# YuhuaXu/ImageMosaicing

Measured on AMD Instinct MI355X. Metric: image-pairs/sec (detect+match+H+warp), 4000x3000 UAV frames, higher is better.
Workload: dtype i16 fixed-point pyramid filtered in f32 (as the reference's OpenCV), f32 (RANSAC / warp coordinates), int8 MFMA with int32 accumulation (descriptor distances, exact), u8 (pixels); 1 GPU; C3: ONE 500-frame 4000x3000 UAV survey, pair window 2 (499 pairs), SIFT(2000,3,0.01,20) + exact BF match + 3x3 grid select + Ransac2D + MosaicImagesRefined warp; frames=500, pairs=499, frames_per_gpu=500, pairs_per_gpu=499

## Files before the change

### imagemosaicing_amd/capi.py

```python
import ctypes as C
import os
import numpy as np

_HERE = os.path.dirname(os.path.abspath(__file__))
_LIB = None

SFPOINT = np.dtype([("x", "<f4"), ("y", "<f4"), ("id", "<i4")])
KEYPOINT = np.dtype([("x", "<f4"), ("y", "<f4"), ("size", "<f4"), ("angle", "<f4"), ("response", "<f4"),
                     ("octave", "<i4"), ("class_id", "<i4")])
DMATCH = np.dtype([("queryIdx", "<i4"), ("trainIdx", "<i4"), ("imgIdx", "<i4"), ("distance", "<f4")])
MATCHPAIR = np.dtype([("ax", "<f4"), ("ay", "<f4"), ("aid", "<i4"), ("ai", "<i4"), ("af", "<i4"),
                      ("bx", "<f4"), ("by", "<f4"), ("bid", "<i4"), ("bi", "<i4"), ("bf", "<i4")])
PAIR_RESULT = np.dtype([("i", "<i4"), ("j", "<i4"), ("n_in", "<i4"), ("n_selected", "<i4"), ("ok", "<i4"),
                        ("accepted", "<i4"), ("H", "<f4", (9,)), ("_pad", "<i4"),
                        ("a", SFPOINT, (400,)), ("b", SFPOINT, (400,))])
CHIPINFO = np.dtype([("x0", "<i4"), ("y0", "<i4"), ("w", "<i4"), ("h", "<i4"), ("img", "<i4"),
                     ("sx", "<f4"), ("sy", "<f4"), ("quad", "<f4", (8,))])
IMAGE_TRANSFORM = np.dtype([("m", "<f4", (9,)), ("fixed", "<i4")])
PAIR_MOMENTS = np.dtype([("i", "<i4"), ("j", "<i4"), ("n_in", "<i4"), ("_pad", "<i4"), ("aa", "<f8", (6,)), ("ab", "<f8", (9,)), ("bb", "<f8", (6,))])
FEATURE_HEADER = np.dtype([("img_id", "<i4"), ("n_kp", "<i4"), ("w", "<i4"), ("h", "<i4")])
FEATURE_RECORD_BYTES = 319488
FEATURE_CHUNK_HEADER = np.dtype([("img_id", "<i4"), ("n_kp", "<i4"), ("w", "<i4"), ("h", "<i4"), ("chunk", "<i4"), ("n_chunks", "<i4"),
                                 ("row0", "<i4"), ("rows", "<i4")])
FEATURE_CHUNK_ROWS = 2048
assert FEATURE_CHUNK_HEADER.itemsize == 32
assert SFPOINT.itemsize == 12 and KEYPOINT.itemsize == 28 and MATCHPAIR.itemsize == 40 and PAIR_RESULT.itemsize == 9664 and PAIR_MOMENTS.itemsize == 184


class Params(C.Structure):
    _fields_ = [("nfeatures", C.c_int32), ("n_octave_layers", C.c_int32), ("contrast_threshold", C.c_float),
                ("edge_threshold", C.c_float), ("sigma", C.c_float), ("max_selected", C.c_int32),
                ("select_fraction", C.c_double), ("grid_x", C.c_int32), ("grid_y", C.c_int32), ("min_inliers", C.c_int32),
                ("ransac_dist", C.c_float), ("sample_times", C.c_int32), ("pair_window", C.c_int32), ("ratio", C.c_float)]


class ScreenParams(C.Structure):
    _fields_ = [("top_k", C.c_int32), ("partners", C.c_int32), ("min_score", C.c_int32), ("ratio_pct", C.c_int32), ("window", C.c_int32)]


class GainParams(C.Structure):
    _fields_ = [("sigma_n", C.c_float), ("sigma_g", C.c_float), ("channels", C.c_int32), ("step", C.c_int32)]


class BlockGainParams(C.Structure):
    _fields_ = [("sigma_n", C.c_float), ("sigma_g", C.c_float), ("channels", C.c_int32), ("step", C.c_int32), ("grid_x", C.c_int32),
                ("grid_y", C.c_int32), ("smooth", C.c_int32), ("reserved", C.c_int32)]


class SharpParams(C.Structure):
    _fields_ = [("prior", C.c_float), ("blur_ratio", C.c_float), ("step", C.c_int32), ("reserved", C.c_int32)]


class CoverParams(C.Structure):
    _fields_ = [("step", C.c_int32), ("min_depth", C.c_int32), ("max_loss", C.c_int64)]


class FeatherParams(C.Structure):
    _fields_ = [("ramp", C.c_int32), ("reserved", C.c_int32 * 3)]


class SeamlineParams(C.Structure):
    _fields_ = [("ramp", C.c_int32), ("reserved", C.c_int32 * 3)]


class MedianParams(C.Structure):
    _fields_ = [("ramp", C.c_int32), ("depth", C.c_int32), ("reserved", C.c_int32 * 2)]


class SeamCutParams(C.Structure):
    _fields_ = [("ramp", C.c_int32), ("level", C.c_int32), ("depth", C.c_int32), ("data_weight", C.c_int32), ("diff_weight", C.c_int32),
                ("seam_penalty", C.c_int32), ("miss_cost", C.c_int32), ("reserved", C.c_int32)]


class SeamReport(C.Structure):
    _fields_ = [("energy_before", C.c_int64), ("energy_after", C.c_int64), ("changed", C.c_int32), ("fallback", C.c_int32)]


SEAM_CELL = np.dtype([("frame", "<u2", 8), ("omega", "u1", 8), ("gray", "u1", 8)])


class Camera(C.Structure):
    _fields_ = [(n, C.c_double) for n in ("fx", "fy", "cx", "cy", "k1", "k2", "p1", "p2", "k3")]


class UndistortParams(C.Structure):
    _fields_ = [("out_fx", C.c_double), ("out_fy", C.c_double), ("out_cx", C.c_double), ("out_cy", C.c_double), ("fill", C.c_int32),
                ("reserved", C.c_int32 * 3)]


class PreviewParams(C.Structure):
    _fields_ = [("render", C.c_int32), ("ramp", C.c_int32), ("level", C.c_int32), ("nodata", C.c_int32), ("reserved", C.c_int32 * 4)]


class LocalWarpParams(C.Structure):
    _fields_ = [("grid_x", C.c_int32), ("grid_y", C.c_int32), ("min_ties", C.c_int32), ("reserved", C.c_int32), ("max_residual", C.c_double),
                ("max_shift", C.c_double), ("smooth", C.c_double), ("prior", C.c_double)]


LOCAL_WARP_REPORT = np.dtype([("n_ties", "<i8"), ("rej_den", "<i8"), ("rej_residual", "<i8"), ("rej_side", "<i8"), ("rms_before", "<f8"),
                              ("rms_after", "<f8"), ("max_shift", "<f8"), ("solved", "<i4"), ("_pad", "<i4")])
assert C.sizeof(LocalWarpParams) == 48 and LOCAL_WARP_REPORT.itemsize == 64

NODATA_NONE, NODATA_ZERO, NODATA_MAP = 0, 1, 2


GAIN_PAIR_STATS = np.dtype([("a", "<i4"), ("b", "<i4"), ("n", "<i8"), ("sum_a", "<i8", (3,)), ("sum_b", "<i8", (3,))])
assert GAIN_PAIR_STATS.itemsize == 64
BLOCK_GAIN_STATS = np.dtype([("pair", "<i4"), ("cell_a", "<i4"), ("cell_b", "<i4"), ("reserved", "<i4"), ("n", "<i8"), ("sum_a", "<i8", (3,)),
                             ("sum_b", "<i8", (3,))])
SHARP_PAIR_STATS = np.dtype([("a", "<i4"), ("b", "<i4"), ("n", "<i8"), ("e_a", "<i8"), ("e_b", "<i8"), ("s_a", "<i8"), ("s_b", "<i8")])
SHARP_FRAME_STATS = np.dtype([("n", "<i8"), ("e", "<i8"), ("s", "<i8")])
SHARP_KEPT, SHARP_DROPPED, SHARP_CUT_VERTEX, SHARP_NO_PAIR = 0, 1, 2, 3
assert SHARP_PAIR_STATS.itemsize == 48 and SHARP_FRAME_STATS.itemsize == 24 and C.sizeof(SharpParams) == 16
COVER_FRAME_STATS = np.dtype([("at_depth", "<i8", (8,))])
COVER_BINS = 9
COVER_NOT_CANDIDATE, COVER_DROPPED, COVER_KEPT_COVERAGE, COVER_CUT_VERTEX, COVER_NOT_EXAMINED = 0, 1, 2, 3, 4
COVER_STATS_FN = C.CFUNCTYPE(C.c_int, C.c_void_p, C.c_void_p, C.c_void_p)
assert COVER_FRAME_STATS.itemsize == 64 and C.sizeof(CoverParams) == 16
PAIR_NORMAL_BLOCK = np.dtype([("i", "<i4"), ("j", "<i4"), ("n_in", "<i4"), ("_pad", "<i4"), ("cost", "<f8"), ("g", "<f8", (16,)), ("N", "<f8", (136,))])


class ProjectiveParams(C.Structure):
    _fields_ = [("max_iters", C.c_int32), ("reserved", C.c_int32), ("prior", C.c_double), ("lambda0", C.c_double), ("lambda_up", C.c_double),
                ("lambda_down", C.c_double), ("min_rel_decrease", C.c_double)]


class ProjectiveReport(C.Structure):
    _fields_ = [("trials", C.c_int32), ("accepted", C.c_int32), ("n_free", C.c_int32), ("n_pairs_used", C.c_int32), ("n_points", C.c_int64),
                ("cost0", C.c_double), ("cost_data", C.c_double), ("cost_prior", C.c_double), ("lambda_", C.c_double)]

    def as_dict(self):
        return {n.rstrip("_"): getattr(self, n) for n, _ in self._fields_}


PAIR_CALIB_BLOCK = np.dtype([("i", "<i4"), ("j", "<i4"), ("n_in", "<i4"), ("n_bad", "<i4"), ("cost", "<f8"), ("g", "<f8", (13,)), ("N", "<f8", (91,))])
CALIB_K1, CALIB_K2, CALIB_P1, CALIB_P2, CALIB_K3 = 1, 2, 4, 8, 16


class CalibParams(C.Structure):
    _fields_ = [("max_iters", C.c_int32), ("mask", C.c_int32), ("min_ties", C.c_int32), ("reserved", C.c_int32), ("lambda0", C.c_double),
                ("lambda_up", C.c_double), ("lambda_down", C.c_double), ("min_rel_decrease", C.c_double)]


class CalibReport(C.Structure):
    _fields_ = [("trials", C.c_int32), ("accepted", C.c_int32), ("n_pairs_used", C.c_int32), ("n_unused_records", C.c_int32), ("n_points", C.c_int64),
                ("cost0", C.c_double), ("cost", C.c_double), ("lambda_", C.c_double)]

    def as_dict(self):
        return {n.rstrip("_"): getattr(self, n) for n, _ in self._fields_}


assert PAIR_CALIB_BLOCK.itemsize == 856 and C.sizeof(CalibParams) == 48 and C.sizeof(CalibReport) == 48


class TieParams(C.Structure):
    _fields_ = [("radius", C.c_int32), ("search", C.c_int32), ("drop_mask", C.c_int32), ("reserved", C.c_int32), ("min_ncc", C.c_float)]


TIE_REPORT = np.dtype([("i", "<i4"), ("j", "<i4"), ("n_in", "<i4"), ("n_out", "<i4"), ("flags", "<i4"), ("count", "<i4", (8,)), ("_pad", "<i4"),
                       ("ncc_q_sum", "<i8")])
TIE_NONE, TIE_REFINED, TIE_EDGE, TIE_FLAT, TIE_LOW, TIE_BORDER = 0, 1, 2, 3, 4, 5
TIE_FLAG_NOT_ACCEPTED, TIE_FLAG_NO_FRAME, TIE_FLAG_BAD_RECORD, TIE_FLAG_DEMOTED = 1, 2, 4, 8
assert TIE_REPORT.itemsize == 64 and C.sizeof(TieParams) == 20
assert PAIR_NORMAL_BLOCK.itemsize == 1240 and C.sizeof(ProjectiveParams) == 48 and C.sizeof(ProjectiveReport) == 56
assert BLOCK_GAIN_STATS.itemsize == 72 and C.sizeof(BlockGainParams) == 32
assert C.sizeof(Camera) == 72 and C.sizeof(UndistortParams) == 48


class VerifyParams(C.Structure):
    _fields_ = [("cycle_tol", C.c_double), ("gate_abs", C.c_double), ("gate_k", C.c_double), ("max_rounds", C.c_int32), ("bridges", C.c_int32)]


PAIR_EDGE = np.dtype([("i", "<i4"), ("j", "<i4"), ("n_in", "<i4"), ("flags", "<i4"), ("box", "<f4", (4,)), ("F", "<f8", (9,)), ("B", "<f8", (9,))])
PAIR_CYCLE = np.dtype([("n_ok", "<i4"), ("n_bad", "<i4"), ("min_e2", "<f8")])
PAIR_RESIDUAL = np.dtype([("i", "<i4"), ("j", "<i4"), ("n_used", "<i4"), ("n_den", "<i4"), ("sum_r2", "<f8"), ("max_r2", "<f8")])
VERIFY_REPORT = np.dtype([("i", "<i4"), ("j", "<i4"), ("n_in", "<i4"), ("verdict", "<i4"), ("n_ok", "<i4"), ("n_bad", "<i4"), ("round", "<i4"),
                          ("flags", "<i4"), ("min_e2", "<f8"), ("rms", "<f8"), ("max_r2", "<f8"), ("reserved", "<f8")])
VERIFY_SUMMARY = np.dtype([("count", "<i4", (8,)), ("rounds", "<i4"), ("n_labelled", "<i4"), ("reserved", "<i4", (2,)), ("s", "<f8"), ("gate", "<f8")])
EDGE_USABLE, EDGE_TESTABLE = 1, 2
VERDICT_NOT_USED, VERDICT_VERIFIED, VERDICT_ADMITTED, VERDICT_BRIDGE, VERDICT_REJECTED, VERDICT_UNDECIDED = 0, 1, 2, 3, 4, 5
VERIFY_SUSPECT = 1
assert PAIR_EDGE.itemsize == 176 and PAIR_CYCLE.itemsize == 16 and PAIR_RESIDUAL.itemsize == 32
assert C.sizeof(VerifyParams) == 32 and VERIFY_REPORT.itemsize == 64 and VERIFY_SUMMARY.itemsize == 64


class GuidedParams(C.Structure):
    _fields_ = [("radius", C.c_float), ("max_dist2", C.c_int32), ("ratio", C.c_float), ("reserved", C.c_int32)]


assert C.sizeof(GuidedParams) == 16


class Mi355Error(RuntimeError):
    def __init__(self, code, msg):
        super().__init__("mi355 error %d: %s" % (code, msg))
        self.code = code


def lib_path():
    return os.environ.get("MI355_LIB") or os.path.join(_HERE, "libmi355mosaic.so")


def load_library():
    global _LIB
    if _LIB is None:
        p = lib_path()
        if not os.path.exists(p):
            raise ImportError("libmi355mosaic.so is not built: run `python -m imagemosaicing_amd.build` "
                              "(there is no CPU fallback for the HIP path)")
        try:
            import torch
        except ImportError:
            pass
        L = C.CDLL(p)
        L.mi355_last_error.restype = C.c_char_p
        L.mi355_last_error.argtypes = [C.c_void_p]
        L.mi355_create.argtypes = [C.POINTER(C.c_void_p), C.c_void_p, C.c_int]
        L.mi355_destroy.argtypes = [C.c_void_p]
        L.mi355_free.argtypes = [C.c_void_p]
        _LIB = L
    return _LIB


def default_params():
    p = Params()
    load_library().mi355_default_params(C.byref(p))
    return p


def _p(a):
    return a.ctypes.data_as(C.c_void_p) if a is not None else None


def _img_geom(img):
    img = np.ascontiguousarray(img, np.uint8)
    h, w = img.shape[:2]
    ch = img.shape[2] if img.ndim == 3 else 1
    return img, w, h, img.strides[0], ch


def _copy_out(ptr, nbytes, dtype):
    if nbytes == 0:
        return np.zeros(0, dtype)
    raw = np.ctypeslib.as_array(C.cast(ptr, C.POINTER(C.c_uint8)), shape=(nbytes,)).copy()
    return raw.view(dtype)


def _view_out(ptr, nbytes, dtype, copy):
    raw = np.ctypeslib.as_array(C.cast(ptr, C.POINTER(C.c_uint8)), shape=(nbytes,))
    return (raw.copy() if copy else raw).view(dtype)


class Context:

    def __init__(self, device=0, params=None):
        self.L = load_library()
        self._h = C.c_void_p()
        rc = self.L.mi355_create(C.byref(self._h), C.byref(params) if params is not None else None, int(device))
        if rc != 0:
            raise Mi355Error(rc, (self.L.mi355_last_error(None) or b"").decode())
        self.params = params if params is not None else default_params()
        self.device = int(device)

    def close(self):
        if self._h:
            self.L.mi355_destroy(self._h)
            self._h = C.c_void_p()

    def __del__(self):
        try:
            self.close()
        except Exception:
            pass

    def _chk(self, rc):
        if rc < 0:
            raise Mi355Error(rc, (self.L.mi355_last_error(self._h) or b"").decode())
        return rc

    def set_stream(self, hip_stream):
        self._chk(self.L.mi355_set_stream(self._h, C.c_void_p(hip_stream or 0)))

    def synchronize(self):
        self._chk(self.L.mi355_synchronize(self._h))

    def set_option(self, name, value):
        self._chk(self.L.mi355_set_option(self._h, name.encode(), int(value)))

    def profile_enable(self, on=True):
        self._chk(self.L.mi355_profile_enable(self._h, int(bool(on))))

    def profile_only(self, cls=None):
        self._chk(self.L.mi355_profile_only(self._h, (cls or "").encode()))

    def profile_reset(self):
        self._chk(self.L.mi355_profile_reset(self._h))

    def profile_get(self, cls):
        ms, n, b = C.c_double(), C.c_int64(), C.c_double()
        self._chk(self.L.mi355_profile_get(self._h, cls.encode(), C.byref(ms), C.byref(n), C.byref(b)))
        return ms.value, n.value, b.value

    def SiftExtract(self, img_id, bgr, max_kp=None):
        img, w, h, ws, ch = _img_geom(bgr)
        assert ch == 3
        max_kp = max_kp or max(int(self.params.nfeatures), 2048)
        kp = np.zeros(max_kp, KEYPOINT)
        desc = np.zeros((max_kp, 128), np.float32)
        n = C.c_int(0)
        self._chk(self.L.mi355_sift_extract(self._h, int(img_id), _p(img), w, h, ws, _p(kp), _p(desc), max_kp, C.byref(n)))
        k = min(n.value, max_kp)
        return kp[:k].copy(), desc[:k].copy()

    def SiftExtractHost(self, img_id, bgr):
        img, w, h, ws, ch = _img_geom(bgr)
        assert ch == 3
        self._chk(self.L.mi355_sift_extract(self._h, int(img_id), _p(img), w, h, ws, None, None, 0, None))

    def SiftExtractDev(self, img_id, d_bgr, w, h, ws, want_count=False):
        if not want_count:
            self._chk(self.L.mi355_sift_extract_dev(self._h, int(img_id), C.c_void_p(int(d_bgr)), int(w), int(h), int(ws), None))
            return None
        n = C.c_int(0)
        self._chk(self.L.mi355_sift_extract_dev(self._h, int(img_id), C.c_void_p(int(d_bgr)), int(w), int(h), int(ws), C.byref(n)))
        return n.value

    def GetFeatures(self, img_id, max_kp=4096):
        kp = np.zeros(max_kp, KEYPOINT)
        desc = np.zeros((max_kp, 128), np.float32)
        n = C.c_int(0)
        self._chk(self.L.mi355_get_features(self._h, int(img_id), _p(kp), _p(desc), max_kp, C.byref(n)))
        return kp[:n.value].copy(), desc[:n.value].copy()

    def SetFeatures(self, img_id, kp, desc, w, h):
        kp = np.ascontiguousarray(kp, KEYPOINT)
        desc = np.ascontiguousarray(desc, np.float32)
        self._chk(self.L.mi355_set_features(self._h, int(img_id), _p(kp), _p(desc), len(kp), int(w), int(h)))

    def DropFeatures(self, img_id=-1):
        self._chk(self.L.mi355_drop_features(self._h, int(img_id)))

    def MatchPairs(self, pairs, ransac_dist=2.5, seed=1):
        pairs = np.ascontiguousarray(pairs, np.int32).reshape(-1, 2)
        out = np.zeros(len(pairs), PAIR_RESULT)
        self._chk(self.L.mi355_match_pairs(self._h, _p(pairs), len(pairs), C.c_float(ransac_dist), C.c_uint32(seed), _p(out)))
        return out

    def MatchPairsDev(self, pairs, d_out, ransac_dist=2.5, seed=1):
        pairs = np.ascontiguousarray(pairs, np.int32).reshape(-1, 2)
        self._chk(self.L.mi355_match_pairs_dev(self._h, _p(pairs), len(pairs), C.c_float(ransac_dist), C.c_uint32(seed), C.c_void_p(int(d_out))))

    def ScreenPairs(self, img_ids, window=0, top_k=256, partners=None, min_score=None, ratio_pct=80, rank=0, world=1, return_scores=False):
        ids = np.ascontiguousarray(img_ids, np.int32).reshape(-1)
        p = screen_params(window=window, top_k=top_k, partners=partners, min_score=min_score, ratio_pct=ratio_pct)
        cap = len(ids) * p.partners if p.partners > 0 else 0
        n = C.c_int(0)
        while True:
            out = np.zeros((max(cap, 1), 2), np.int32)
            sc = np.zeros(max(cap, 1), np.int32)
            rc = self.L.mi355_screen_pairs(self._h, _p(ids), len(ids), C.byref(p), int(rank), int(world), _p(out), _p(sc), cap, C.byref(n))
            if rc == -1 and n.value > cap:
                cap = n.value
                continue
            self._chk(rc)
            break
        pairs = out[:n.value].copy()
        return (pairs, sc[:n.value].copy()) if return_scores else pairs

    def ScreenScoresDev(self, img_ids, d_scores, **params):
        ids = np.ascontiguousarray(img_ids, np.int32).reshape(-1)
        p = screen_params(**params)
        self._chk(self.L.mi355_screen_scores_dev(self._h, _p(ids), len(ids), C.byref(p), C.c_void_p(int(d_scores))))

    def BFMatch(self, img_i, img_j, sorted_=True, max_matches=2048):
        m = np.zeros(max_matches, DMATCH)
        d2 = np.zeros(max_matches, np.int32)
        s2 = np.zeros(max_matches, np.int32)
        n = C.c_int(0)
        self._chk(self.L.mi355_bf_match(self._h, int(img_i), int(img_j), int(bool(sorted_)), _p(m), _p(d2), _p(s2), max_matches, C.byref(n)))
        k = min(n.value, max_matches)
        return m[:k].copy(), d2[:k].copy(), s2[:k].copy()

    def SelectMatchPairs(self, matches, kp1_xy, kp2_xy, nMatch, width, height, gridX=3, gridY=3):
        matches = np.asarray(matches)
        if matches.dtype != DMATCH:
            mm = np.zeros(len(matches), DMATCH)
            mm["queryIdx"] = matches[:, 0]
            mm["trainIdx"] = matches[:, 1]
            matches = mm
        matches = np.ascontiguousarray(matches)
        kp1 = np.ascontiguousarray(kp1_xy, np.float32)
        kp2 = np.ascontiguousarray(kp2_xy, np.float32)
        v1 = np.zeros(400, SFPOINT)
        v2 = np.zeros(400, SFPOINT)
        n = C.c_int(0)
        self._chk(self.L.mi355_select_grid(self._h, _p(matches), len(matches), _p(kp1), len(kp1), _p(kp2), len(kp2), int(nMatch),
                                           int(width), int(height), int(gridX), int(gridY), _p(v1), _p(v2), C.byref(n)))
        return v1[:n.value].copy(), v2[:n.value].copy()

    def Ransac2D(self, p1, p2, fRansacDist=1.0, sampleTimes=1000, seed=1):
        p1 = np.ascontiguousarray(p1, SFPOINT)
        p2 = np.ascontiguousarray(p2, SFPOINT)
        n = len(p1)
        i1 = np.zeros(max(400, n), SFPOINT)
        i2 = np.zeros(max(400, n), SFPOINT)
        nin = C.c_int(0)
        H = np.zeros(9, np.float32)
        ok = self._chk(self.L.mi355_ransac2d(self._h, _p(p1), _p(p2), n, C.c_float(fRansacDist), int(sampleTimes), C.c_uint32(seed),
                                             _p(i1), _p(i2), C.byref(nin), _p(H)))
        return ok, i1[:nin.value].copy(), i2[:nin.value].copy(), H

    def ImageProjectionTransform(self, img, h9):
        img, w, h, ws, ch = _img_geom(img)
        h9 = np.ascontiguousarray(h9, np.float32)
        dst = C.c_void_p()
        dw, dh, dws = C.c_int(), C.c_int(), C.c_int()
        self._chk(self.L.mi355_warp_image(self._h, _p(img), w, h, ws, ch, _p(h9), C.byref(dst), C.byref(dw), C.byref(dh), C.byref(dws)))
        buf = _copy_out(dst, dh.value * dws.value, np.uint8).reshape(dh.value, dws.value)
        self.L.mi355_free(dst)
        return buf, dw.value, dh.value, dws.value

    def MosaicImagesRefined(self, imgs, h9s, want_pixels=True):
        n, imgs, ptrs, w, h, ws = self._host_args(imgs)
        h9s = np.ascontiguousarray(h9s, np.float32)
        canvas = C.c_void_p()
        cw, ch, cws = C.c_int(), C.c_int(), C.c_int()
        self._chk(self.L.mi355_mosaic_refined(self._h, ptrs, _p(w), _p(h), _p(ws), n, _p(h9s), C.byref(canvas), C.byref(cw), C.byref(ch), C.byref(cws)))
        buf = _copy_out(canvas, ch.value * cws.value, np.uint8).reshape(ch.value, cws.value) if want_pixels else None
        self.L.mi355_free(canvas)
        return buf, cw.value, ch.value, cws.value

    def MosaicImagesRefinedDev(self, d_imgs, w, h, ws, h9s, d_canvas, cw, ch, cws, row0=0, rows=-1):
        n = len(d_imgs)
        ptrs = (C.c_void_p * n)(*[int(p) for p in d_imgs])
        w = np.ascontiguousarray(w, np.int32)
        h = np.ascontiguousarray(h, np.int32)
        ws = np.ascontiguousarray(ws, np.int32)
        h9s = np.ascontiguousarray(h9s, np.float32)
        self._chk(self.L.mi355_mosaic_refined_dev(self._h, ptrs, _p(w), _p(h), _p(ws), n, _p(h9s), C.c_void_p(int(d_canvas)),
                                                  int(cw), int(ch), int(cws), int(row0), int(rows if rows >= 0 else ch)))

    def SurfExtract(self, img_id, bgr, hessian=50.0, max_kp=4096):
        img, w, h, ws, ch = _img_geom(bgr)
        assert ch == 3
        kp = np.zeros(max_kp, KEYPOINT)
        desc = np.zeros((max_kp, 128), np.float32)
        n = C.c_int(0)
        self._chk(self.L.mi355_surf_extract(self._h, int(img_id), _p(img), w, h, ws, C.c_float(hessian), int(max_kp), _p(kp), _p(desc), C.byref(n)))
        return kp[:n.value].copy(), desc[:n.value].copy()

    def SurfMatchPairs(self, pairs, ransac_dist=2.5, seed=1, match_dist=0.5, max_features=200, min_inliers=18):
        pairs = np.ascontiguousarray(pairs, np.int32).reshape(-1, 2)
        out = np.zeros(len(pairs), PAIR_RESULT)
        self._chk(self.L.mi355_surf_match_pairs(self._h, _p(pairs), len(pairs), C.c_float(ransac_dist), C.c_uint32(seed), C.c_float(match_dist),
                                                int(max_features), int(min_inliers), _p(out)))
        return out

    def PackFeaturesDev(self, img_ids, d_payload):
        ids = np.ascontiguousarray(img_ids, np.int32)
        hdr = np.zeros(len(ids), FEATURE_HEADER)
        self._chk(self.L.mi355_pack_features_dev(self._h, _p(ids), len(ids), _p(hdr), C.c_void_p(int(d_payload))))
        return hdr

    def InstallFeaturesDev(self, hdr, d_payload):
        hdr = np.ascontiguousarray(hdr, FEATURE_HEADER)
        self._chk(self.L.mi355_install_features_dev(self._h, _p(hdr), C.c_void_p(int(d_payload)), len(hdr)))

    def FeatureChunkCount(self, img_ids):
        ids = np.ascontiguousarray(img_ids, np.int32)
        n = C.c_int(0)
        self._chk(self.L.mi355_feature_chunk_count(self._h, _p(ids), len(ids), C.byref(n)))
        return n.value

    def PackFeatureChunksDev(self, img_ids, d_payload, max_records):
        ids = np.ascontiguousarray(img_ids, np.int32)
        hdr = np.zeros(max(int(max_records), 1), FEATURE_CHUNK_HEADER)
        n = C.c_int(0)
        self._chk(self.L.mi355_pack_feature_chunks_dev(self._h, _p(ids), len(ids), _p(hdr), C.c_void_p(int(d_payload) or None), int(max_records), C.byref(n)))
        return hdr[:n.value].copy()

    def InstallFeatureChunksDev(self, hdr, d_payload):
        hdr = np.ascontiguousarray(hdr, FEATURE_CHUNK_HEADER)
        self._chk(self.L.mi355_install_feature_chunks_dev(self._h, _p(hdr), C.c_void_p(int(d_payload) or None), len(hdr)))

    def CompactAcceptedDev(self, d_in, n, d_out):
        k = C.c_int(0)
        self._chk(self.L.mi355_compact_accepted_dev(self._h, C.c_void_p(int(d_in)), int(n), C.c_void_p(int(d_out)), C.byref(k)))
        return k.value

    def last_sift_counters(self):
        out = (C.c_int32 * 8)()
        self._chk(self.L.mi355_last_sift_counters(self._h, out))
        return list(out)

    def CommInit(self, id128, rank, world):
        buf = (C.c_uint8 * 128).from_buffer_copy(bytes(id128))
        self._chk(self.L.mi355_comm_init(self._h, buf, int(rank), int(world)))

    def CommDestroy(self):
        self._chk(self.L.mi355_comm_destroy(self._h))

    def CommInfo(self):
        r, n = C.c_int(0), C.c_int(0)
        self._chk(self.L.mi355_comm_info(self._h, C.byref(r), C.byref(n)))
        return r.value, n.value

    def AllGatherFeatures(self, img_ids, n_max_per_rank):
        ids = np.ascontiguousarray(img_ids, np.int32)
        self._chk(self.L.mi355_allgather_features(self._h, _p(ids), len(ids), int(n_max_per_rank)))

    def AllGatherFeatureChunks(self, img_ids, install_own=False):
        ids = np.ascontiguousarray(img_ids, np.int32)
        self._chk(self.L.mi355_allgather_feature_chunks(self._h, _p(ids), len(ids), 1 if install_own else 0))

    def AllGatherResults(self, d_local, n_local, accepted_only=True, root=-1, copy=True, wait=True):
        assert wait or (root >= 0 and not copy)
        ptr, n = C.c_void_p(), C.c_int(0)
        flags = (1 if accepted_only else 0) | (0 if wait else 2)
        self._chk(self.L.mi355_allgather_results(self._h, C.c_void_p(int(d_local)), int(n_local), flags, int(root), C.byref(ptr), C.byref(n)))
        if not ptr.value or n.value == 0:
            return np.zeros(0, PAIR_RESULT)
        return _view_out(ptr, n.value * PAIR_RESULT.itemsize, PAIR_RESULT, copy)

    def PairMomentsDev(self, d_results, n, d_out):
        self._chk(self.L.mi355_pair_moments_dev(self._h, C.c_void_p(int(d_results)), int(n), C.c_void_p(int(d_out))))

    def PairNormalBlocksDev(self, d_results, n, h8, part, d_out):
        h8 = np.ascontiguousarray(h8, np.float64).reshape(-1, 8)
        part = np.ascontiguousarray(part, np.uint8)
        assert len(h8) == len(part)
        self._chk(self.L.mi355_pair_normal_blocks_dev(self._h, C.c_void_p(int(d_results)), int(n), _p(h8), _p(part), len(part), C.c_void_p(int(d_out))))

    def GlobalProjectiveRefineDev(self, d_results, n_pairs, w, h, start, fixed=None, label=None, params=None):
        a = _projective_args(w, h, start, fixed, label)
        out, rep = np.zeros(len(a[2]), IMAGE_TRANSFORM), ProjectiveReport()
        self._chk(self.L.mi355_global_projective_refine_dev(self._h, C.c_void_p(int(d_results) or None), int(n_pairs), len(a[2]), _p(a[0]), _p(a[1]), _p(a[3]), _p(a[4]), _p(a[2]),
                                                            C.byref(params) if params is not None else None, _p(out), C.byref(rep)))
        return out, rep.as_dict()

    def PairCalibBlocksDev(self, d_results, n, h8, cam, d_out, min_ties=16):
        h8 = None if h8 is None else np.ascontiguousarray(h8, np.float64).reshape(-1, 8)
        assert h8 is None or len(h8) >= int(n)
        self._chk(self.L.mi355_pair_calib_blocks_dev(self._h, C.c_void_p(int(d_results or 0) or None), int(n), _p(h8), C.byref(cam) if cam is not None else None,
                                                     int(min_ties), C.c_void_p(int(d_out or 0) or None)))

    def CalibrateLensDev(self, d_results, n_pairs, start, params=None, **kw):
        p = params if params is not None else calib_params(**kw)
        out, rep = Camera(), CalibReport()
        self._chk(self.L.mi355_calibrate_lens_dev(self._h, C.c_void_p(int(d_results or 0) or None), int(n_pairs), C.byref(start) if start is not None else None, C.byref(p),
                                                  C.byref(out), C.byref(rep)))
        return out, rep.as_dict()

    def RefineTiesDev(self, d_in, n, d_imgs, w, h, ws, d_out, d_status=0, d_ncc2=0, d_report=0, params=None, **kw):
        n_img, ptrs, w, h, ws = self._frame_args(d_imgs, w, h, ws)
        p = params if params is not None else tie_params(**kw)
        self._chk(self.L.mi355_refine_ties_dev(self._h, C.c_void_p(int(d_in or 0) or None), int(n), ptrs, _p(w), _p(h), _p(ws), n_img, C.byref(p),
                                               C.c_void_p(int(d_out or 0) or None), C.c_void_p(int(d_status or 0) or None),
                                               C.c_void_p(int(d_ncc2 or 0) or None), C.c_void_p(int(d_report or 0) or None)))

    def RefineTies(self, results, imgs, img_ids=None, geom=None, params=None, **kw):
        res = np.ascontiguousarray(results, PAIR_RESULT)
        n = len(res)
        ptrs, ids, w, h, ws, _keep = self._into_args(imgs, img_ids, geom)
        p = params if params is not None else tie_params(**kw)
        out = np.zeros(n, PAIR_RESULT)
        status, ncc2, report = np.zeros((n, 400), np.uint8), np.zeros((n, 400), np.float32), np.zeros(n, TIE_REPORT)
        self._chk(self.L.mi355_refine_ties(self._h, _p(res), n, ptrs, _p(ids), _p(w), _p(h), _p(ws), len(ids), C.byref(p), _p(out), _p(status), _p(ncc2),
                                           _p(report)))
        return out, status, ncc2, report

    def AllGatherMoments(self, d_local, n_local, copy=True):
        ptr, n = C.c_void_p(), C.c_int(0)
        self._chk(self.L.mi355_allgather_moments(self._h, C.c_void_p(int(d_local)), int(n_local), C.byref(ptr), C.byref(n)))
        if not ptr.value or n.value == 0:
            return np.zeros(0, PAIR_MOMENTS)
        return _view_out(ptr, n.value * PAIR_MOMENTS.itemsize, PAIR_MOMENTS, copy)

    def StripeCover(self, w, h, h9s, row0, rows, blended=False, keep=None, band=5, exact=False):
        n = len(w)
        w = np.ascontiguousarray(w, np.int32); h = np.ascontiguousarray(h, np.int32)
        h9s = np.ascontiguousarray(h9s, np.float32)
        keep_a = None if keep is None else np.ascontiguousarray(keep, np.uint8)
        need = np.zeros(n, np.uint8)
        mode = 1 if blended else (2 if exact else 0)
        self._chk(self.L.mi355_mosaic_stripe_cover(self._h, mode, _p(w), _p(h), n, _p(h9s), _p(keep_a), int(band), int(row0), int(rows), _p(need)))
        return need

    def ExchangeFrames(self, d_frames, h, ws, need, owner=None, own_through_rccl=False):
        n = len(d_frames)
        ptrs = (C.c_void_p * max(n, 1))(*[int(p) if p else None for p in d_frames])
# ... 1470 lines not shown
```

### imagemosaicing_amd/csrc/api.hip

```cpp
#include "common.h"
#include "mosaic_frame.h"
#include <memory>
#include <new>

static thread_local std::string g_create_error;

void mi_set_host_error(const std::string& s) { g_create_error = s; }

extern "C" void mi355_default_params(mi355_params* p) {
    if (!p) return;
    p->nfeatures = 2000; p->n_octave_layers = 3; p->contrast_threshold = 0.01f; p->edge_threshold = 20.0f; p->sigma = 1.6f;
    p->max_selected = 400; p->select_fraction = 0.3; p->grid_x = 3; p->grid_y = 3; p->min_inliers = 30;
    p->ransac_dist = 2.5f; p->sample_times = 1000; p->pair_window = 182; p->ratio = 0.0f;
}

void mi355_ctx::prof_begin(const char* cls, double alg_bytes, hipStream_t st) {
    ProfClass& pc = prof[cls];
    if (pc.used == pc.ev.size()) {
        hipEvent_t a, b;
        if (hipEventCreate(&a) != hipSuccess || hipEventCreate(&b) != hipSuccess) return;
        pc.ev.emplace_back(a, b);
    }
    pc.bytes += alg_bytes;
    (void)hipEventRecord(pc.ev[pc.used].first, st);
// ... 67 lines not shown
    if (ctx->heavy_ev) (void)hipEventDestroy(ctx->heavy_ev);
    for (hipEvent_t e : ctx->batch_events) if (e) (void)hipEventDestroy(e);
    if (ctx->own_stream) (void)hipStreamDestroy(ctx->own_stream);
    delete ctx;
}

extern "C" const char* mi355_last_error(mi355_ctx* ctx) { return ctx ? ctx->err.c_str() : g_create_error.c_str(); }

extern "C" int mi355_set_stream(mi355_ctx* ctx, void* hip_stream) {
    LOCKED_PROLOGUE
    { int rc = mi_resolve_features(ctx); if (rc != MI355_OK) return rc; }
    (void)hipStreamSynchronize(ctx->stream);
    if (hip_stream) {
        if (ctx->own_stream) { (void)hipStreamDestroy(ctx->own_stream); ctx->own_stream = nullptr; }
        ctx->stream = (hipStream_t)hip_stream;
    } else {
        if (!ctx->own_stream) MI_HIP(hipStreamCreateWithFlags(&ctx->own_stream, hipStreamNonBlocking));
        ctx->stream = ctx->own_stream;
    }
    return MI355_OK;
}

extern "C" int mi355_synchronize(mi355_ctx* ctx) {
    LOCKED_PROLOGUE
    int rc = mi_resolve_features(ctx);
    if (rc != MI355_OK) return rc;
    MI_HIP(hipStreamSynchronize(ctx->stream));
    return MI355_OK;
}

extern "C" void mi355_free(void* p) { free(p); }

extern "C" int mi355_sift_extract_dev(mi355_ctx* ctx, int img_id, const uint8_t* d_bgr, int w, int h, int width_step, int* n_kp) {
    LOCKED_PROLOGUE
    if (!d_bgr || w < 16 || h < 16 || width_step < 3 * w) { ctx->set_error("sift_extract: bad image geometry"); return MI355_ERR_ARG; }
    return mi_sift_extract_dev(ctx, img_id, d_bgr, w, h, width_step, n_kp);
}

extern "C" int mi355_sift_extract(mi355_ctx* ctx, int img_id, const uint8_t* bgr, int w, int h, int width_step,
                                  mi355_keypoint* kp, float* desc128, int max_kp, int* n_kp) {
    int n = 0;
    const bool deferred = !kp && !desc128 && !n_kp;
    {
        LOCKED_PROLOGUE
        if (!bgr || w < 16 || h < 16 || width_step < 3 * w) { ctx->set_error("sift_extract: bad image geometry"); return MI355_ERR_ARG; }
        const size_t bytes = (size_t)width_step * h;
        if (ctx->keep_frames) {
            uint8_t* dkeep = nullptr;
            int rc = mi_kept_frame_slot(ctx, img_id, w, h, width_step, "sift_extract", &dkeep);
            if (rc != MI355_OK) return rc;
            MI_HIP(hipMemcpyAsync(dkeep, bgr, bytes, hipMemcpyHostToDevice, ctx->stream));
            ctx->pend_event = ctx->kept_frames[img_id].ev;
            rc = mi_sift_extract_dev(ctx, img_id, dkeep, w, h, width_step, deferred ? nullptr : &n);
            ctx->pend_event = nullptr;
            if (rc != MI355_OK || deferred) return rc;
        } else if (deferred) {
            const size_t ring = (size_t)(ctx->sift_nslots + 1) * (size_t)(ctx->sift_batch < 1 ? 1 : ctx->sift_batch);
            if (ctx->host_frames.size() != ring) {
                int rc = mi_resolve_features(ctx);
                if (rc != MI355_OK) return rc;
                for (auto& b : ctx->host_frames) b.release();
                for (hipEvent_t e : ctx->host_frame_ev) if (e) (void)hipEventDestroy(e);
                ctx->host_frames.assign(ring, DevBuf());
                ctx->host_frame_ev.assign(ring, nullptr);
                ctx->host_frame_used.assign(ring, 0);
                ctx->host_frame_next = 0;
            }
            const size_t slot = ctx->host_frame_next;
            ctx->host_frame_next = (ctx->host_frame_next + 1) % ring;
            DevBuf& dimg = ctx->host_frames[slot];
            if (!ctx->host_frame_ev[slot]) MI_HIP(hipEventCreateWithFlags(&ctx->host_frame_ev[slot], hipEventDisableTiming));
            if (ctx->host_frame_used[slot]) {
                int rc = mi_sift_flush_if_parked(ctx, ctx->host_frame_ev[slot]);
                if (rc != MI355_OK) return rc;
                MI_HIP(hipStreamWaitEvent(ctx->stream, ctx->host_frame_ev[slot], 0));
            }
            ctx->host_frame_used[slot] = 1;
            MI_HIP(dimg.reserve(bytes + 16));
            MI_HIP(hipMemcpyAsync(dimg.p, bgr, bytes, hipMemcpyHostToDevice, ctx->stream));
            ctx->pend_event = ctx->host_frame_ev[slot];
            const int rc = mi_sift_extract_dev(ctx, img_id, dimg.as<uint8_t>(), w, h, width_step, nullptr);
            ctx->pend_event = nullptr;
            return rc;
        } else {
            DevBuf& dimg = ctx->buf("sift_host_img");
            MI_HIP(dimg.reserve(bytes + 16));
            MI_HIP(hipMemcpyAsync(dimg.p, bgr, bytes, hipMemcpyHostToDevice, ctx->stream));
            int rc = mi_sift_extract_dev(ctx, img_id, dimg.as<uint8_t>(), w, h, width_step, &n);
            if (rc != MI355_OK) return rc;
        }
    }
    if (n_kp) *n_kp = n;
    if (kp || desc128) return mi355_get_features(ctx, img_id, kp, desc128, max_kp, nullptr);
    return MI355_OK;
}

extern "C" int mi355_set_features(mi355_ctx* ctx, int img_id, const mi355_keypoint* kp, const float* desc128, int n_kp, int w, int h) {
    LOCKED_PROLOGUE
    return mi_set_features(ctx, img_id, kp, desc128, n_kp, w, h);
}

extern "C" int mi355_drop_features(mi355_ctx* ctx, int img_id) {
    LOCKED_PROLOGUE
    (void)mi_resolve_features(ctx);
    MI_HIP(hipStreamSynchronize(ctx->stream));
    if (img_id < 0) { for (auto& kv : ctx->feats) kv.second.release(); ctx->feats.clear(); }
    else { auto it = ctx->feats.find(img_id); if (it != ctx->feats.end()) { it->second.release(); ctx->feats.erase(it); } }
    return MI355_OK;
}

extern "C" int mi355_match_pairs_dev(mi355_ctx* ctx, const int32_t* pairs_ij, int n_pairs, float ransac_dist, uint32_t seed, mi355_pair_result* d_out) {
    LOCKED_PROLOGUE
    if (n_pairs < 0 || (n_pairs > 0 && (!pairs_ij || !d_out))) return MI355_ERR_ARG;
    return mi_match_pairs_dev(ctx, pairs_ij, n_pairs, ransac_dist, seed, d_out);
}

extern "C" int mi355_match_pairs(mi355_ctx* ctx, const int32_t* pairs_ij, int n_pairs, float ransac_dist, uint32_t seed, mi355_pair_result* out) {
    LOCKED_PROLOGUE
    if (n_pairs < 0 || (n_pairs > 0 && (!pairs_ij || !out))) return MI355_ERR_ARG;
    if (n_pairs == 0) return MI355_OK;
    DevBuf& dres = ctx->buf("pair_results");
    MI_HIP(dres.reserve(sizeof(mi355_pair_result) * (size_t)n_pairs));
    int rc = mi_match_pairs_dev(ctx, pairs_ij, n_pairs, ransac_dist, seed, dres.as<mi355_pair_result>());
    if (rc != MI355_OK) return rc;
    MI_HIP(hipMemcpyAsync(out, dres.p, sizeof(mi355_pair_result) * (size_t)n_pairs, hipMemcpyDeviceToHost, ctx->stream));
    MI_HIP(hipStreamSynchronize(ctx->stream));
    return MI355_OK;
}

extern "C" int mi355_bf_match(mi355_ctx* ctx, int img_i, int img_j, int sorted, mi355_dmatch* matches, int32_t* d2, int32_t* second_d2,
                              int max_matches, int* n_matches) {
    LOCKED_PROLOGUE
    return mi_bf_match(ctx, img_i, img_j, sorted, matches, d2, second_d2, max_matches, n_matches);
}

extern "C" int mi355_select_grid(mi355_ctx* ctx, const mi355_dmatch* sorted, int n, const float* kp1_xy, int n_kp1,
                                 const float* kp2_xy, int n_kp2, int nMatch, int width, int height, int gridX, int gridY,
                                 mi355_sfpoint* v1, mi355_sfpoint* v2, int* n_out) {
    LOCKED_PROLOGUE
    if (nMatch < 0 || nMatch > MI355_MAX_SELECTED) { ctx->set_error("select_grid: nMatch must be in [0,400]"); return MI355_ERR_ARG; }
    return mi_select_grid(ctx, sorted, n, kp1_xy, n_kp1, kp2_xy, n_kp2, nMatch, width, height, gridX, gridY, v1, v2, n_out);
}

extern "C" int mi355_ransac2d(mi355_ctx* ctx, const mi355_sfpoint* p1, const mi355_sfpoint* p2, int n, float dist, int sample_times,
                              uint32_t seed, mi355_sfpoint* in1, mi355_sfpoint* in2, int* n_in, float H[9]) {
    LOCKED_PROLOGUE
    if (!n_in || !H) return MI355_ERR_ARG;
    *n_in = 0;
    for (int i = 0; i < 9; i++) H[i] = 0.0f;
    if (n <= 0 || !p1 || !p2) return 0;
    if (n > MI355_RANSAC_BIG_MAX) { ctx->set_error("ransac2d: at most 65535 correspondences"); return MI355_ERR_ARG; }
    if (n > MI355_MAX_SELECTED) {
        int ok = 0;
        const int rc = mi_ransac_big(ctx, p1, p2, n, dist, sample_times, seed, in1, in2, n_in, H, &ok);
        return rc != MI355_OK ? rc : ok;
    }
    DevBuf& d1 = ctx->buf("r1_p1"); DevBuf& d2 = ctx->buf("r1_p2"); DevBuf& dn = ctx->buf("r1_n"); DevBuf& dres = ctx->buf("pair_results");
    MI_HIP(d1.reserve(sizeof(mi355_sfpoint) * MI355_MAX_SELECTED)); MI_HIP(d2.reserve(sizeof(mi355_sfpoint) * MI355_MAX_SELECTED));
    MI_HIP(dn.reserve(sizeof(int))); MI_HIP(dres.reserve(sizeof(mi355_pair_result)));
    MI_HIP(hipMemcpyAsync(d1.p, p1, sizeof(mi355_sfpoint) * n, hipMemcpyHostToDevice, ctx->stream));
    MI_HIP(hipMemcpyAsync(d2.p, p2, sizeof(mi355_sfpoint) * n, hipMemcpyHostToDevice, ctx->stream));
    MI_HIP(hipMemcpyAsync(dn.p, &n, sizeof(int), hipMemcpyHostToDevice, ctx->stream));
    int rc = mi_ransac_batch(ctx, d1.as<mi355_sfpoint>(), d2.as<mi355_sfpoint>(), dn.as<int>(), &n, 1, MI355_MAX_SELECTED, dist, sample_times, seed,
                             dres.as<mi355_pair_result>());
    if (rc != MI355_OK) return rc;
    const std::unique_ptr<mi355_pair_result> r(new (std::nothrow) mi355_pair_result);
    if (!r) return MI355_ERR_NOMEM;
    hipError_t e = hipMemcpyAsync(r.get(), dres.p, sizeof(mi355_pair_result), hipMemcpyDeviceToHost, ctx->stream);
    if (e == hipSuccess) e = hipStreamSynchronize(ctx->stream);
    if (e != hipSuccess) { ctx->set_error(hipGetErrorString(e)); return MI355_ERR_DEVICE; }
    *n_in = r->n_in;
    if (in1) memcpy(in1, r->a, sizeof(mi355_sfpoint) * r->n_in);
    if (in2) memcpy(in2, r->b, sizeof(mi355_sfpoint) * r->n_in);
    memcpy(H, r->H, sizeof(float) * 9);
    return r->ok;
}

extern "C" int mi355_warp_image(mi355_ctx* ctx, const uint8_t* src, int w, int h, int ws, int ch, const float h9[9],
                                uint8_t** dst, int* dw, int* dh, int* dws) {
    LOCKED_PROLOGUE
    if (!dst || !dw || !dh || !dws) return MI355_ERR_ARG;
    return mi_warp_image(ctx, src, w, h, ws, ch, h9, dst, dw, dh, dws);
}

extern "C" int mi355_mosaic_refined_dev(mi355_ctx* ctx, const uint8_t* const* d_imgs, const int* w, const int* h, const int* ws, int n,
                                        const float* h9s, uint8_t* d_canvas, int cw, int ch, int cws, int row0, int rows) {
    LOCKED_PROLOGUE
    if (!d_imgs || !w || !h || !ws || !h9s || !d_canvas || n <= 0) return MI355_ERR_ARG;
    return mi_mosaic_refined_dev(ctx, d_imgs, w, h, ws, n, h9s, d_canvas, cw, ch, cws, row0, rows);
}

extern "C" int mi355_mosaic_refined(mi355_ctx* ctx, const uint8_t* const* imgs, const int* w, const int* h, const int* ws, int n,
                                    const float* h9s, uint8_t** canvas, int* cw, int* ch, int* cws) {
    LOCKED_PROLOGUE
    if (!imgs || !w || !h || !ws || !h9s || !canvas || !cw || !ch || !cws) return MI355_ERR_ARG;
    int lw, lh, lws;
    std::vector<const uint8_t*> d_imgs;
    uint8_t* d_canvas;
    int rc = mi_render_host_begin(ctx, "mosaic_refined", imgs, w, h, ws, n, h9s, &lw, &lh, &lws, d_imgs, &d_canvas);
    if (rc == MI355_OK) rc = mi_mosaic_refined_dev(ctx, d_imgs.data(), w, h, ws, n, h9s, d_canvas, lw, lh, lws, 0, lh);
    if (rc != MI355_OK) return rc;
    return mi_render_host_end(ctx, lw, lh, lws, canvas, cw, ch, cws);
}

extern "C" int mi355_chips_and_masks(mi355_ctx* ctx, const uint8_t* const* imgs, const int* w, const int* h, const int* ws, int n,
                                     const float* h9s, const uint8_t* keep, int find_masks,
                                     int* n_chips, mi355_chip_info** chips, uint8_t*** chip_imgs, uint8_t*** masks, int* canvas_w, int* canvas_h) {
    LOCKED_PROLOGUE
    return mi_chips_and_masks(ctx, imgs, w, h, ws, n, h9s, keep, find_masks, n_chips, chips, chip_imgs, masks, canvas_w, canvas_h);
}

extern "C" int mi355_multiband_blend(mi355_ctx* ctx, const uint8_t* const* chips, const uint8_t* const* masks, const mi355_chip_info* info, int n,
                                     int canvas_w, int canvas_h, int band, uint8_t** out, int* out_w, int* out_h, int* out_ws) {
    LOCKED_PROLOGUE
    return mi_multiband_blend(ctx, chips, masks, info, n, canvas_w, canvas_h, band, out, out_w, out_h, out_ws);
}

extern "C" int mi355_mosaic_blended(mi355_ctx* ctx, const uint8_t* const* imgs, const int* w, const int* h, const int* ws, int n, const float* h9s,
                                    const uint8_t* keep, int band, uint8_t** out, int* out_w, int* out_h, int* out_ws) {
    LOCKED_PROLOGUE
    return mi_mosaic_blended(ctx, imgs, w, h, ws, n, h9s, keep, band, out, out_w, out_h, out_ws);
}

extern "C" int mi355_mosaic_blended_dev(mi355_ctx* ctx, const uint8_t* const* d_imgs, const int* w, const int* h, const int* ws, int n, const float* h9s,
                                        const uint8_t* keep, int band, uint8_t* d_canvas, int cw, int ch, int cws) {
    LOCKED_PROLOGUE
    return mi_mosaic_blended_dev(ctx, d_imgs, w, h, ws, n, h9s, keep, band, d_canvas, cw, ch, cws);
}

extern "C" int mi355_mosaic_blended_rows_dev(mi355_ctx* ctx, const uint8_t* const* d_imgs, const int* w, const int* h, const int* ws, int n, const float* h9s,
                                             const uint8_t* keep, int band, uint8_t* d_rows, int cw, int ch, int cws, int row0, int rows) {
    LOCKED_PROLOGUE
    if (rows < 1) { ctx->set_error("mosaic_blended_rows_dev: bad stripe"); return MI355_ERR_ARG; }
    return mi_mosaic_blended_dev(ctx, d_imgs, w, h, ws, n, h9s, keep, band, d_rows, cw, ch, cws, row0, rows);
}

extern "C" int mi355_mosaic_stripe_cover(mi355_ctx* ctx, int mode, const int* w, const int* h, int n, const float* h9s, const uint8_t* keep, int band,
                                         int row0, int rows, uint8_t* need) {
    LOCKED_PROLOGUE
    if (!w || !h || !h9s || !need || n <= 0 || mode < 0 || mode > 2) { ctx->set_error("mosaic_stripe_cover: bad arguments"); return MI355_ERR_ARG; }
    memset(need, 0, (size_t)n);
    std::vector<const uint8_t*> none((size_t)n, nullptr);
    std::vector<int> ws((size_t)n);
    for (int k = 0; k < n; k++) ws[k] = (3 * w[k] + 3) & ~3;
    if (mode != MI355_COVER_BLENDED) {
        int cw = 0, ch = 0, cws = 0;
        const int rc = mi355_mosaic_layout(w, h, n, h9s, &cw, &ch, &cws, nullptr);
        if (rc != MI355_OK) { ctx->set_error("mosaic_stripe_cover: no image with h[8] != 0 / empty canvas"); return rc; }
        return mi_mosaic_refined_dev(ctx, none.data(), w, h, ws.data(), n, h9s, nullptr, cw, ch, cws, row0, rows, need, mode == MI355_COVER_REFINED_EXACT ? 1 : 0);
    }
    int cw = 0, ch = 0;
    { const int rc = mi_blend_layout(w, h, n, h9s, keep, &cw, &ch); if (rc != MI355_OK) return rc; }
    return mi_mosaic_blended_dev(ctx, none.data(), w, h, ws.data(), n, h9s, keep, band, nullptr, cw, ch, (cw * 3 + 3) & ~3, row0, rows, need);
}

extern "C" int mi355_blend_layout(const int* w, const int* h, int n, const float* h9s, const uint8_t* keep, int* cw, int* ch, int* cws) {
    if (!cw || !ch) return MI355_ERR_ARG;
    const int rc = mi_blend_layout(w, h, n, h9s, keep, cw, ch);
    if (rc == MI355_OK && cws) *cws = (*cw * 3 + 3) & ~3;
    return rc;
}

extern "C" int mi355_profile_enable(mi355_ctx* ctx, int on) {
    LOCKED_PROLOGUE
    ctx->profiling = on != 0;
    return MI355_OK;
}
extern "C" int mi355_last_sift_counters(mi355_ctx* ctx, int32_t out8[8]) {
    LOCKED_PROLOGUE
    if (!out8) return MI355_ERR_ARG;
    for (int i = 0; i < 8; i++) out8[i] = ctx->last_counts[i];
    return MI355_OK;
}
extern "C" int mi355_set_option(mi355_ctx* ctx, const char* name, int value) {
    LOCKED_PROLOGUE
    if (!name) return MI355_ERR_ARG;
    if (std::string(name) == "sift_slots") {
        int rc = mi_resolve_features(ctx);
        if (rc != MI355_OK) return rc;
        ctx->sift_nslots = value < 1 ? 1 : (value > 4 ? 4 : value);
        return MI355_OK;
    }
    if (std::string(name) == "sift_batch") {
        int rc = mi_resolve_features(ctx);
        if (rc != MI355_OK) return rc;
        ctx->sift_batch = value < 1 ? 1 : (value > 32 ? 32 : value);
        return MI355_OK;
    }
    if (std::string(name) == "keepall_max") {
        if (value < MI355_SIFT_KEEPALL_MAX || value > MI355_SIFT_KEEPALL_LIMIT || value % 2048 != 0) {
            ctx->set_error("set_option: keepall_max must be a multiple of 2048 in [" + std::to_string(MI355_SIFT_KEEPALL_MAX) + ", " + std::to_string(MI355_SIFT_KEEPALL_LIMIT) + "]");
            return MI355_ERR_ARG;
        }
        int rc = mi_resolve_features(ctx);
        if (rc != MI355_OK) return rc;
        for (const auto& kv : ctx->feats)
            if (kv.second.n > value) {
                ctx->set_error("set_option: keepall_max=" + std::to_string(value) + " is below the " + std::to_string(kv.second.n) + " keypoints of image " + std::to_string(kv.first));
                return MI355_ERR_ARG;
            }
        ctx->keepall_max = value;
        return MI355_OK;
    }
    if (std::string(name) == "big_subpairs_max") { ctx->big_sub_max = value < 1 ? 1 : value; return MI355_OK; }
    {
        struct { const char* n; int* p; } knobs[] = {{"ransac_split", &ctx->ransac_split}, {"strict_frames", &ctx->strict_frames}};
        for (auto& k : knobs) if (std::string(name) == k.n) { *k.p = value; return MI355_OK; }
    }
    if (std::string(name) == "keep_frames") { ctx->keep_frames = value ? 1 : 0; return MI355_OK; }
    if (std::string(name) == "download_chunk_mb") {
        if (value < 1) { ctx->set_error("set_option: download_chunk_mb must be >= 1"); return MI355_ERR_ARG; }
        ctx->download_chunk = (size_t)value << 20;
        return MI355_OK;
    }
    if (std::string(name) == "download_threads") { ctx->download_threads = value < 1 ? 1 : (value > 16 ? 16 : value); return MI355_OK; }
    if (std::string(name) == "preview_stripe_rows") {
        if (value < 0) { ctx->set_error("set_option: preview_stripe_rows must be >= 0"); return MI355_ERR_ARG; }
        ctx->preview_stripe_rows = value;
        return MI355_OK;
    }
    if (std::string(name) == "download_mode") { ctx->download_mode = value < 0 || value > 2 ? 0 : value; return MI355_OK; }
    if (std::string(name) == "sift_flush") return mi_sift_flush(ctx);
    if (std::string(name) == "blur_stream") { ctx->blur_stream = value ? 1 : 0; return MI355_OK; }
    if (std::string(name) == "sift_cascade" || std::string(name) == "keepall_order") return MI355_OK;
    if (std::string(name) == "serial_heavy") {
        int rc = mi_resolve_features(ctx);
        if (rc != MI355_OK) return rc;
        ctx->serial_heavy = value ? 1 : 0; ctx->heavy_ev_valid = false;
        return MI355_OK;
    }
    if (std::string(name).rfind("profile_every:", 0) == 0) { ctx->prof[std::string(name).substr(14)].every = value < 1 ? 1 : value; return MI355_OK; }
    if (std::string(name) == "xstream_min_w") { ctx->xstream_min_w = value < 256 ? 256 : value; return MI355_OK; }
    if (std::string(name) == "xstream_min_frames") { ctx->xstream_min_frames = value < 1 ? 1 : value; return MI355_OK; }
    ctx->set_error(std::string("set_option: unknown option ") + name);
    return MI355_ERR_ARG;
}
extern "C" int mi355_profile_only(mi355_ctx* ctx, const char* kernel_class) {
    LOCKED_PROLOGUE
    ctx->prof_only = kernel_class ? kernel_class : "";
    return MI355_OK;
}
extern "C" int mi355_profile_reset(mi355_ctx* ctx) {
    LOCKED_PROLOGUE
    (void)mi_resolve_features(ctx);
    MI_HIP(hipStreamSynchronize(ctx->stream));
    for (auto& kv : ctx->prof) { kv.second.used = 0; kv.second.bytes = 0.0; kv.second.seen = 0; }
    return MI355_OK;
}
extern "C" int mi355_profile_get(mi355_ctx* ctx, const char* kernel_class, double* total_ms, int64_t* launches, double* alg_bytes) {
    LOCKED_PROLOGUE
    if (!kernel_class) return MI355_ERR_ARG;
    (void)mi_resolve_features(ctx);
    MI_HIP(hipStreamSynchronize(ctx->stream));
    double ms = 0.0; int64_t cnt = 0; double bytes = 0.0;
    auto it = ctx->prof.find(kernel_class);
    if (it != ctx->prof.end()) {
        for (size_t i = 0; i < it->second.used; i++) {
            float t = 0.0f;
            if (hipEventElapsedTime(&t, it->second.ev[i].first, it->second.ev[i].second) == hipSuccess) ms += t;
        }
        cnt = (int64_t)it->second.used; bytes = it->second.bytes;
    }
    if (total_ms) *total_ms = ms;
    if (launches) *launches = cnt;
    if (alg_bytes) *alg_bytes = bytes;
    return MI355_OK;
}

extern "C" int mi355_pair_schedule(int n_images, int window, int rank, int world, int32_t* pairs_ij, int max_pairs, int* n_pairs) {
    if (n_images < 0 || window < 2 || world < 1 || rank < 0 || rank >= world || !n_pairs) return MI355_ERR_ARG;
    int cnt = 0;
    for (int i = rank; i < n_images; i += world) {
        const int jEnd = n_images < i + window ? n_images : i + window;
        for (int j = i + 1; j < jEnd; j++) {
            if (pairs_ij && cnt < max_pairs) { pairs_ij[2 * cnt] = i; pairs_ij[2 * cnt + 1] = j; }
            cnt++;
        }
    }
    *n_pairs = cnt;
    return (pairs_ij && cnt > max_pairs) ? MI355_ERR_ARG : MI355_OK;
}
```

### imagemosaicing_amd/csrc/common.h

```cpp
#pragma once
#include <hip/hip_runtime.h>
#include <cstdint>
#include <cstdio>
#include <cstring>
#include <cstdlib>
#include <map>
#include <mutex>
#include <string>
#include <unordered_map>
#include <vector>
#include "../../include/mi355_mosaic.h"

#define MI_HIP(call)                                                                       \
    do {                                                                                   \
        hipError_t e_ = (call);                                                            \
        if (e_ != hipSuccess) {                                                            \
            ctx->set_error(std::string(#call) + ": " + hipGetErrorString(e_));             \
            return MI355_ERR_DEVICE;                                                       \
        }                                                                                  \
    } while (0)

#define LOCKED_PROLOGUE                                  \
    if (!ctx) return MI355_ERR_ARG;                      \
    std::lock_guard<std::mutex> lk(ctx->mu);             \
    if (hipSetDevice(ctx->device) != hipSuccess) { ctx->set_error("hipSetDevice failed"); return MI355_ERR_DEVICE; }

constexpr int MI355_SIFT_BATCH_MAX = 32;
constexpr int MI355_SIFT_KEEPALL_MAX = 32768;

constexpr int MI355_SIFT_KEEPALL_LIMIT = 262144;

struct DevBuf {
    void*  p = nullptr;
    size_t cap = 0;
    hipError_t reserve(size_t bytes) {
        if (bytes <= cap) return hipSuccess;
        if (p) { hipError_t e = hipFree(p); if (e != hipSuccess) return e; p = nullptr; cap = 0; }
        size_t slack = bytes / 4;
        if (slack > ((size_t)256 << 20)) slack = (size_t)256 << 20;
        size_t want = bytes + slack + 256;
        hipError_t e = hipMalloc(&p, want);
        if (e == hipSuccess) cap = want;
        return e;
    }
    void release() { if (p) (void)hipFree(p); p = nullptr; cap = 0; }
    template <class T> T* as() const { return reinterpret_cast<T*>(p); }
};

struct HostBuf {
    void*  p = nullptr;
    size_t cap = 0;
    hipError_t reserve(size_t bytes) {
        if (bytes <= cap) return hipSuccess;
        if (p) { hipError_t e = hipHostFree(p); if (e != hipSuccess) return e; p = nullptr; cap = 0; }
        const size_t want = bytes + bytes / 8 + 4096;
        hipError_t e = hipHostMalloc(&p, want, hipHostMallocDefault);
        if (e == hipSuccess) cap = want;
        return e;
    }
    void release() { if (p) (void)hipHostFree(p); p = nullptr; cap = 0; }
    template <class T> T* as() const { return reinterpret_cast<T*>(p); }
};

struct Features {
    int n = 0;
    int npad = 0;
    int w = 0, h = 0;
    DevBuf kp;
    DevBuf xy;
    DevBuf d8;
    DevBuf s8;
    DevBuf n8;
    bool pending = false;
    volatile int* h_cnt = nullptr;
    hipEvent_t ready = nullptr;
    unsigned caps[3] = {0, 0, 0};
    int kp_limit = 0;
    void release() { kp.release(); xy.release(); d8.release(); s8.release(); n8.release(); }
};

struct KeptFrame {
    void*  p = nullptr;
    size_t cap = 0;
    int w = 0, h = 0, ws = 0;
    hipEvent_t ev = nullptr;
};

struct ProfClass {
    std::vector<std::pair<hipEvent_t, hipEvent_t>> ev;
    size_t used = 0;
    double bytes = 0.0;
    size_t seen = 0;
    int every = 1;
};

struct SiftWork;
struct mi355_comm;
struct SurfState;

struct mi355_ctx {
    int device = 0;
    hipStream_t stream = nullptr;
    hipStream_t own_stream = nullptr;
    std::mutex mu;
    mi355_params p;
    std::string err;
    std::unordered_map<int, Features> feats;
    std::map<std::string, DevBuf> ws;
    std::map<std::string, HostBuf> hws;
    struct DrawTables { uint32_t seed = 0; bool valid = false; DevBuf buf, raw; hipEvent_t ready = nullptr; unsigned long long used = 0; };
    DrawTables draw_tables[4];
    unsigned long long draw_clock = 0;
    hipStream_t aux_stream = nullptr;
    hipEvent_t aux_ev = nullptr;
    int* draw_flags = nullptr;
    bool profiling = false;
    std::string prof_only;
    std::map<std::string, ProfClass> prof;
    std::vector<SiftWork*> sift_slots;
    int sift_next = 0;
    std::vector<hipEvent_t> batch_events; size_t batch_events_used = 0;
    hipEvent_t heavy_ev = nullptr; bool heavy_ev_valid = false;
    int serial_heavy = 0;
    std::vector<DevBuf> host_frames;
    std::vector<hipEvent_t> host_frame_ev;
    std::vector<char> host_frame_used;
    size_t host_frame_next = 0;
    hipEvent_t pend_event = nullptr;
    int keep_frames = 0;
    std::unordered_map<int, KeptFrame> kept_frames;
    size_t download_chunk = (size_t)64 << 20;
    int download_threads = 4;
    int preview_stripe_rows = 1024;
    int download_mode = 0;
    hipStream_t dl_stream = nullptr;
    hipEvent_t dl_ev[3] = {nullptr, nullptr, nullptr};
    int blur_stream = 1;
    int sift_nslots = 3;
    int xstream_min_w = 1500, xstream_min_frames = 4;
    int sift_batch = 16;
    int strict_frames = 0;
    int ransac_split = -1;
    hipEvent_t sift_in_ev = nullptr;
    std::vector<int*> pinned_chunks;
    size_t pinned_used = 0;
    int num_cu = 256;
    mi355_comm* comm = nullptr;
    SurfState* surf = nullptr;
    int keepall_max = MI355_SIFT_KEEPALL_MAX;
    int big_sub_max = 65536;
    int last_counts[8] = {0};

    void set_error(const std::string& s) { err = s; }
    DevBuf& buf(const std::string& name) { return ws[name]; }
    HostBuf& hbuf(const std::string& name) { return hws[name]; }
    void prof_begin(const char* cls, double alg_bytes, hipStream_t st);
    void prof_end(const char* cls, hipStream_t st);
};

struct ProfScope {
    mi355_ctx* c; const char* cls; hipStream_t st;
    bool on;
    ProfScope(mi355_ctx* c_, const char* cls_, double bytes, hipStream_t st_ = nullptr) : c(c_), cls(cls_), st(st_ ? st_ : c_->stream) {
        on = c->profiling && (c->prof_only.empty() || ("," + c->prof_only + ",").find(std::string(",") + cls + ",") != std::string::npos);
        if (on) { ProfClass& pc = c->prof[cls]; if (pc.every > 1) on = (pc.seen++ % (size_t)pc.every) == 0; }
        if (on) c->prof_begin(cls, bytes, st);
    }
    ~ProfScope() { if (on) c->prof_end(cls, st); }
};

int mi_warp_image(mi355_ctx*, const uint8_t* src, int w, int h, int ws, int ch, const float* h9,
                  uint8_t** dst, int* dw, int* dh, int* dws);
int mi_mosaic_refined_dev(mi355_ctx*, const uint8_t* const* d_imgs, const int* w, const int* h, const int* ws, int n,
                          const float* h9s, uint8_t* d_canvas, int cw, int ch, int cws, int row0, int rows, uint8_t* cover_only = nullptr, int cover_exact = 0);
int mi_mosaic_feathered_dev(mi355_ctx*, const uint8_t* const* d_imgs, const int* w, const int* h, const int* ws, int n, const float* h9s,
                            const mi355_feather_params* params, uint8_t* d_canvas, int cw, int ch, int cws, int row0, int rows);
int mi_mosaic_seamline_dev(mi355_ctx*, const uint8_t* const* d_imgs, const int* w, const int* h, const int* ws, int n, const float* h9s,
                           const mi355_seamline_params* params, uint8_t* d_canvas, int cw, int ch, int cws, uint16_t* d_owner, uint16_t* d_count,
                           int row0, int rows, uint8_t* cover_only);
int mi_mosaic_median_dev(mi355_ctx*, const uint8_t* const* d_imgs, const int* w, const int* h, const int* ws, int n, const float* h9s,
                         const mi355_median_params* params, uint8_t* d_canvas, int cw, int ch, int cws, uint8_t* d_spread, uint16_t* d_count,
                         int row0, int rows, uint8_t* cover_only);
int mi_mosaic_seamcut_dev(mi355_ctx*, const uint8_t* const* d_imgs, const int* w, const int* h, const int* ws, int n, const float* h9s,
                          const mi355_seamcut_params* params, const uint16_t* d_cells, uint8_t* d_canvas, int cw, int ch, int cws, uint16_t* d_owner,
                          uint16_t* d_count, int row0, int rows, uint8_t* cover_only);
int mi_seam_labels_dev(mi355_ctx*, const mi355_seam_cell* d_cand, int gw, int gh, const mi355_seamcut_params* params, uint16_t* d_cells,
                       mi355_seam_report* report);
int mi_seamcut_params_check(mi355_ctx*, const char* who, const mi355_seamcut_params* params);
int mi_mosaic_blended_seam_dev(mi355_ctx*, const uint8_t* const* d_imgs, const int* w, const int* h, const int* ws, int n, const float* h9s,
                               const uint8_t* keep, int band, const mi355_seamcut_params* params, const uint16_t* d_cells, int gw, int gh,
                               uint8_t* d_canvas, int cw, int ch, int cws);
int mi_mosaic_overview_dev(mi355_ctx*, const uint8_t* d_rows, int cw, int ch, int cws, const uint16_t* d_valid_rows, int nodata, int levels,
                           uint8_t* const* d_levels, uint16_t* const* d_covers, int row0, int rows, int only_level = 0);
int mi_sift_flush(mi355_ctx*);
int mi_sift_flush_if_parked(mi355_ctx*, hipEvent_t ev);
int mi_mosaic_blended(mi355_ctx*, const uint8_t* const* imgs, const int* w, const int* h, const int* ws, int n, const float* h9s,
                      const uint8_t* keep, int band, uint8_t** out, int* ow, int* oh, int* ows);
int mi_mosaic_blended_dev(mi355_ctx*, const uint8_t* const* d_imgs, const int* w, const int* h, const int* ws, int n, const float* h9s,
                          const uint8_t* keep, int band, uint8_t* d_canvas, int cw, int ch, int cws, int row0 = 0, int rows = -1, uint8_t* cover_only = nullptr);
int mi_blend_layout(const int* w, const int* h, int n, const float* h9s, const uint8_t* keep, int* cw, int* ch);
int mi_multiband_blend(mi355_ctx*, const uint8_t* const* chips, const uint8_t* const* masks, const mi355_chip_info* info, int n,
                       int W, int H, int band, uint8_t** out, int* ow, int* oh, int* ows);
int mi_chips_and_masks(mi355_ctx*, const uint8_t* const* imgs, const int* w, const int* h, const int* ws, int n,
                       const float* h9s, const uint8_t* keep, int find_masks, int* n_chips, mi355_chip_info** chips,
                       uint8_t*** chip_imgs, uint8_t*** masks, int* cw, int* ch);
int mi_ransac_tables(mi355_ctx*, uint32_t seed, const uint16_t** d_tables);
int mi_ransac_batch(mi355_ctx*, const mi355_sfpoint* d_p1, const mi355_sfpoint* d_p2, const int* d_n, const int* h_n,
                    int n_pairs, int stride, float dist, int sample_times, uint32_t seed, mi355_pair_result* d_out, int min_keep = -1);
int mi_ransac_big(mi355_ctx*, const mi355_sfpoint* p1, const mi355_sfpoint* p2, int n, float dist, int sample_times, uint32_t seed,
                  mi355_sfpoint* in1, mi355_sfpoint* in2, int* n_in, float* H, int* ok);
int mi_match_pairs_dev(mi355_ctx*, const int32_t* pairs, int n_pairs, float dist, uint32_t seed, mi355_pair_result* d_out);
int mi_finalize_pairs(mi355_ctx*, const int32_t* pairs_ij , int n_pairs, const int* d_nsel, mi355_pair_result* d_out);
int mi_bf_match(mi355_ctx*, int img_i, int img_j, int sorted, mi355_dmatch* matches, int32_t* d2, int32_t* second, int maxm, int* nm);
int mi_select_grid(mi355_ctx*, const mi355_dmatch* sorted, int n, const float* kp1, int nk1, const float* kp2, int nk2,
                   int nMatch, int width, int height, int gx, int gy, mi355_sfpoint* v1, mi355_sfpoint* v2, int* n_out);
int mi_set_features(mi355_ctx*, int img_id, const mi355_keypoint* kp, const float* desc, int n, int w, int h);
int mi_finish_features(mi355_ctx*, Features& f);
int mi_finish_features_batch(mi355_ctx*, Features* const* fs, int nf, const int* d_n, int n_stride, hipStream_t st, int max_rows = 2048);
int mi_resolve_features(mi355_ctx*);
int mi_resolve_features_of(mi355_ctx*, const int* ids, int n);
int mi_sift_extract_dev(mi355_ctx*, int img_id, const uint8_t* d_bgr, int w, int h, int ws, int* n_kp);
void mi_sift_release(mi355_ctx*);
void mi_comm_release(mi355_ctx*);
void mi_surf_release(mi355_ctx*);
int  mi_kept_frame_slot(mi355_ctx*, int img_id, int w, int h, int ws, const char* who, uint8_t** d_frame);
void mi_frames_release(mi355_ctx*);
int mi_compact_accepted(mi355_ctx* ctx, const mi355_pair_result* d_in, int n, mi355_pair_result* d_out, int* d_n_out);
int mi_pair_moments(mi355_ctx* ctx, const mi355_pair_result* d_results, int n, mi355_pair_moments* d_out);

#include "host_error.h"
int  mi_inverse_matrix_host(const float* src, int order, float* dst, float eps);
void mi_glibc_draw_table(uint32_t seed, int n, int max_draws, uint16_t* out4);
```

### imagemosaicing_amd/csrc/sift.hip

```cpp
#include "common.h"
#include "sift_plan.h"
#include <memory>
#include "detmath.h"
#include <cmath>
#include <type_traits>

namespace {

using namespace sift_plan;
constexpr int MAX_INTERP = 5, ORI_BINS = 36;
constexpr int FIXPT_SCALE = 48;
constexpr float DOG_THRESHOLD_P1 = 21.0f;
constexpr float HIST_Q = 1024.0f;
constexpr int SIFT_BATCH_MAX = MI355_SIFT_BATCH_MAX;
static_assert(SIFT_BATCH_MAX == BATCH_MAX, "sift_plan.h: BATCH_MAX");
typedef int16_t lvl_t;

__host__ __device__ __forceinline__ int reflect101(int p, int n) {
    if (n == 1) return 0;
    while (p < 0 || p >= n) { if (p < 0) p = -p; else p = 2 * n - 2 - p; }
    return p;
}

typedef float v2f __attribute__((ext_vector_type(2)));
struct __attribute__((aligned(4))) uint2_a4 { unsigned x, y; };
typedef float v4f __attribute__((ext_vector_type(4)));

__device__ __forceinline__ v4f ld4(const lvl_t* p) {
    const uint2 q = *reinterpret_cast<const uint2*>(p);
    v4f o;
    o.x = (float)(int)(short)(q.x & 0xffffu); o.y = (float)((int)q.x >> 16);
    o.z = (float)(int)(short)(q.y & 0xffffu); o.w = (float)((int)q.y >> 16);
    return o;
}
__device__ __forceinline__ float ld1(const lvl_t* p) { return (float)(int)*p; }
__device__ __forceinline__ int sat16(float v) {
    int q = (int)rintf(v);
    q = q < -32768 ? -32768 : (q > 32767 ? 32767 : q);
    return q;
}
__device__ __forceinline__ float gray48(const uint8_t* p) {
    return (float)(((1868 * (int)p[0] + 9617 * (int)p[1] + 4899 * (int)p[2] + 8192) >> 14) * FIXPT_SCALE);
}

__device__ __forceinline__ int xcd_remap(int bid, int nb) {
    const int q = nb >> 3, r = nb & 7, xcd = bid & 7, local = bid >> 3;
    const int base = xcd < r ? xcd * (q + 1) : r * (q + 1) + (xcd - r) * q;
    return base + local;
}

template <int J, int NPP, class F> __device__ __forceinline__ bool static_rows(F& f) {
    if constexpr (J < NPP) { if (!f(std::integral_constant<int, J>{})) return false; return static_rows<J + 1, NPP>(f); }
    else return true;
}

struct Blur16Args {
    const lvl_t* src;
    const uint8_t* bgr[SIFT_BATCH_MAX];
    int bgr_ws[SIFT_BATCH_MAX];
    lvl_t* dst;
    lvl_t* ds;
    int w, h;
    int tiles_x, tiles_y;
    float k[2 * MAX_R + 1];
    float kp[2 * (MAX_R + 1)];
    size_t fstride;
    int nb;
};

template <int R, bool BGR>
__global__ __launch_bounds__(256) void blur16_tile(Blur16Args a) {
    constexpr int ROWS = T16H + 2 * R, COLS = T16W + 2 * R, PIN = COLS | 1, PMID = T16W + 4;
    __shared__ float s_in[ROWS * PIN];
    __shared__ __attribute__((aligned(16))) float s_mid[ROWS * PMID];
    const int tid = threadIdx.x, fr = blockIdx.y;
    const int tile = xcd_remap(blockIdx.x, a.tiles_x * a.tiles_y);
    const int ty = tile / a.tiles_x, tx = tile - ty * a.tiles_x;
    const int x0 = tx * T16W, y0 = ty * T16H;
    const lvl_t* src = BGR ? nullptr : a.src + (size_t)fr * a.fstride;
    const uint8_t* bgr = a.bgr[0]; int bws = a.bgr_ws[0];
    if (BGR) {
#pragma unroll
        for (int q = 1; q < SIFT_BATCH_MAX; q++) if (fr == q) { bgr = a.bgr[q]; bws = a.bgr_ws[q]; }
    }
    lvl_t* dst = a.dst + (size_t)fr * a.fstride;
    for (int idx = tid; idx < ROWS * COLS; idx += 256) {
        const int ry = idx / COLS, rx = idx - ry * COLS;
        const int gy = reflect101(y0 - R + ry, a.h), gx = reflect101(x0 - R + rx, a.w);
        s_in[ry * PIN + rx] = BGR ? gray48(bgr + (size_t)gy * bws + 3 * gx) : ld1(src + (size_t)gy * a.w + gx);
    }
    __syncthreads();
    for (int item = tid; item < ROWS * (T16W / 4); item += 256) {
        const int xg = item / ROWS, row = item - xg * ROWS;
        const float* in = s_in + row * PIN + 4 * xg;
        float e[2 * R + 4];
#pragma unroll
        for (int m = 0; m < 2 * R + 4; m++) e[m] = in[m];
        float acc[4];
#pragma unroll
        for (int q = 0; q < 4; q++) acc[q] = a.k[0] * e[q];
#pragma unroll
        for (int i = 1; i <= 2 * R; i++) {
#pragma unroll
            for (int q = 0; q < 4; q++) { const float p = a.k[i] * e[q + i]; acc[q] = acc[q] + p; }
        }
        *reinterpret_cast<v4f*>(s_mid + row * PMID + 4 * xg) = (v4f){acc[0], acc[1], acc[2], acc[3]};
    }
    __syncthreads();
    for (int item = tid; item < T16H * (T16W / 4); item += 256) {
        const int yy = item / (T16W / 4), xg = item - yy * (T16W / 4);
        const float* mid = s_mid + (yy + R) * PMID + 4 * xg;
        v4f acc = *reinterpret_cast<const v4f*>(mid) * a.k[R];
#pragma unroll
        for (int j = 1; j <= R; j++) {
            const v4f sm = *reinterpret_cast<const v4f*>(mid + j * PMID) + *reinterpret_cast<const v4f*>(mid - j * PMID);
            const v4f p = sm * a.k[R + j];
            acc = acc + p;
        }
        const int gx = x0 + 4 * xg, gy = y0 + yy;
        if (gy >= a.h) continue;
        const int o0 = sat16(acc.x), o1 = sat16(acc.y), o2 = sat16(acc.z), o3 = sat16(acc.w);
        lvl_t* d = dst + (size_t)gy * a.w + gx;
        if (gx + 3 < a.w && (a.w & 3) == 0) {
            *reinterpret_cast<uint2*>(d) = make_uint2((unsigned)(o0 & 0xffff) | ((unsigned)o1 << 16), (unsigned)(o2 & 0xffff) | ((unsigned)o3 << 16));
        } else {
            if (gx < a.w) d[0] = (lvl_t)o0;
            if (gx + 1 < a.w) d[1] = (lvl_t)o1;
            if (gx + 2 < a.w) d[2] = (lvl_t)o2;
            if (gx + 3 < a.w) d[3] = (lvl_t)o3;
        }
        if (a.ds && !(gy & 1) && (gy >> 1) < (a.h >> 1)) {
            lvl_t* q = a.ds + (size_t)fr * a.fstride + (size_t)(gy >> 1) * (a.w >> 1);
            if ((gx >> 1) < (a.w >> 1)) q[gx >> 1] = (lvl_t)o0;
            if (((gx + 2) >> 1) < (a.w >> 1)) q[(gx + 2) >> 1] = (lvl_t)o2;
        }
    }
}

#include "build/blur16_asm.inc"
template <int R, bool BGR, bool DS>
__device__ __forceinline__ void blur16_stream_body(const Blur16Args& a, int L, int nstrip, int nseg) {
    constexpr int RA = (R + 3) / 4 * 4, SW = 256, BW = SW + 2 * RA;
    constexpr int BUF = (BW + 8 + 63) & ~63;
    static_assert(2 * RA + R <= 64, "halo lanes");
    __shared__ __attribute__((aligned(16))) float s_buf[4][2][BUF];
    const int lane = threadIdx.x & 63, wave = threadIdx.x >> 6;
    int unit = __builtin_amdgcn_readfirstlane(xcd_remap(blockIdx.x, gridDim.x) * 4 + wave);
    const int per = nstrip * nseg, fr = unit / per;
    if (fr >= a.nb) return;
    unit -= fr * per;
    const int seg = unit / nstrip, strip = unit - seg * nstrip;
    if (seg >= nseg) return;
    const int x0 = strip * SW, y0 = seg * L;
    const int lact = (a.h - y0 < L) ? a.h - y0 : L;
    const int wv = a.w - x0;
    const int xm = x0 + 4 * lane;
    const int xl = xm < a.w - 4 ? xm : a.w - 4;
    int hcol, hpos;
    if (lane < RA) { hcol = x0 - RA + lane; hpos = lane; }
    else if (lane < 2 * RA) { hcol = x0 + SW + (lane - RA); hpos = SW + lane; }
    else if (wv < SW && lane < 2 * RA + R) { hcol = x0 + wv + (lane - 2 * RA); hpos = RA + wv + (lane - 2 * RA); }
    else { hcol = x0; hpos = BW + (lane & 7); }
    hcol = reflect101(hcol, a.w);
    const size_t fro = (size_t)fr * a.fstride;
    const uint8_t* bgr = a.bgr[0]; int bws = a.bgr_ws[0];
    if (BGR) {
#pragma unroll
        for (int q = 1; q < SIFT_BATCH_MAX; q++) if (fr == q) { bgr = a.bgr[q]; bws = a.bgr_ws[q]; }
    }
    const int rowb = BGR ? bws : 2 * a.w;
    int gy = y0 - R, dir = 1;
    if (gy < 0) { gy = -gy; dir = -1; }
    const unsigned long long rp = (unsigned long long)(BGR ? reinterpret_cast<uintptr_t>(bgr) : reinterpret_cast<uintptr_t>(a.src + fro)) + (unsigned long long)gy * (unsigned)rowb;
    const unsigned moff = BGR ? 3u * xl : 2u * xl;
    unsigned hoff, hsh = 0;
    if (BGR) {
        const int b0 = 3 * hcol; int st = b0 & ~3; if (st + 8 > bws) st = bws - 8;
        hoff = (unsigned)st; hsh = 8u * (unsigned)(b0 - st);
    } else hoff = 2u * hcol;
    const unsigned lds0 = (unsigned)reinterpret_cast<uintptr_t>(&s_buf[wave][0][0]);
    const unsigned lds_win = lds0 + 16u * lane, lds_main = lds0 + 4u * (RA + 4 * lane), lds_halo = lds0 + 4u * hpos;
    const unsigned long long dp = (unsigned long long)reinterpret_cast<uintptr_t>(a.dst + fro) + 2ull * (unsigned long long)y0 * a.w;
    const unsigned long long dsp = DS ? (unsigned long long)reinterpret_cast<uintptr_t>(a.ds + fro) + 2ull * (unsigned long long)(y0 >> 1) * (a.w >> 1) : 0ull;
    const unsigned doff = 2u * xm, dsoff = 2u * (xm >> 1);
    const unsigned long long smask = __ballot(xm < a.w);
    const unsigned long long kp = (unsigned long long)reinterpret_cast<uintptr_t>(__builtin_amdgcn_kernarg_segment_ptr()) + offsetof(Blur16Args, kp);
    const int n = lact + 2 * R + 1;
    const int hm1 = a.h - 1, dstr = 2 * a.w;
    (void)hsh;
#define BLUR_ASM_CALL(NAME) NAME(lds_win, lds_main, lds_halo, moff, hoff, doff, dsoff, rp, dp, dsp, kp, smask, rowb, gy, dir, hm1, dstr, n)
    if constexpr (BGR) { static_assert(R == 6, "base level"); blur16_asm_r6_bgr(lds_win, lds_main, lds_halo, moff, hoff, doff, dsoff, hsh, rp, dp, dsp, kp, smask, rowb, gy, dir, hm1, dstr, n); }
    else if constexpr (R == 5) BLUR_ASM_CALL(blur16_asm_r5);
    else if constexpr (R == 6) BLUR_ASM_CALL(blur16_asm_r6);
    else if constexpr (R == 8 && DS) BLUR_ASM_CALL(blur16_asm_r8_ds);
    else if constexpr (R == 8) BLUR_ASM_CALL(blur16_asm_r8);
    else if constexpr (R == 10) BLUR_ASM_CALL(blur16_asm_r10);
    else if constexpr (R == 13) BLUR_ASM_CALL(blur16_asm_r13);
#undef BLUR_ASM_CALL
}
template <int R, bool BGR, bool DS, int W>
__global__ __launch_bounds__(256) __attribute__((amdgpu_waves_per_eu(W, W))) void blur16_stream(Blur16Args a, int L, int nstrip, int nseg) {
    blur16_stream_body<R, BGR, DS>(a, L, nstrip, nseg);
}

__global__ __launch_bounds__(256) void downsample16(const lvl_t* src, int sw, lvl_t* dst, int dw, int dh, size_t fstride) {
    src += (size_t)blockIdx.z * fstride; dst += (size_t)blockIdx.z * fstride;
    const int x = blockIdx.x * 64 + (threadIdx.x & 63), y = blockIdx.y * 4 + (threadIdx.x >> 6);
    if (x < dw && y < dh) dst[(size_t)y * dw + x] = src[(size_t)(2 * y) * sw + 2 * x];
}

struct OctaveDev { lvl_t* lv[N_LEVELS]; int w, h; };

constexpr int ECAP = 128;
constexpr int REG_STRIDE = 32;
struct BatchStride { size_t pyr, claimed, cand, refined, kps, cube, sel, mins; };
struct FrameOuts { mi355_keypoint* kp[SIFT_BATCH_MAX]; uint8_t* d8[SIFT_BATCH_MAX]; };

struct Refined { int o, layer, r, c; float xi, xr, xc, contr, scl; unsigned start; };

struct PyrDev { OctaveDev oc[MAX_OCT]; unsigned* claimed[MAX_OCT]; unsigned* mins[MAX_OCT]; int n_oct; };

__device__ __forceinline__ float dogv(const OctaveDev& oc, size_t foff, int lvl, int r, int c) {
    const size_t o = foff + (size_t)r * oc.w + c;
    return (float)((int)oc.lv[lvl + 1][o] - (int)oc.lv[lvl][o]);
}

__device__ __forceinline__ void solve3(const float a[3][3], const float b[3], float x[3]) {
    const float det = (a[0][0] * (a[1][1] * a[2][2] - a[2][1] * a[1][2]) - a[0][1] * (a[1][0] * a[2][2] - a[2][0] * a[1][2])) + a[0][2] * (a[1][0] * a[2][1] - a[2][0] * a[1][1]);
    if (det == 0.0f) { x[0] = x[1] = x[2] = 0.0f; return; }
    const float d = 1.0f / det;
    x[0] = d * ((b[0] * (a[1][1] * a[2][2] - a[1][2] * a[2][1]) - a[0][1] * (b[1] * a[2][2] - a[1][2] * b[2])) + a[0][2] * (b[1] * a[2][1] - a[1][1] * b[2]));
    x[1] = d * ((a[0][0] * (b[1] * a[2][2] - a[1][2] * b[2]) - b[0] * (a[1][0] * a[2][2] - a[1][2] * a[2][0])) + a[0][2] * (a[1][0] * b[2] - b[1] * a[2][0]));
    x[2] = d * ((a[0][0] * (a[1][1] * b[2] - b[1] * a[2][1]) - a[0][1] * (a[1][0] * b[2] - b[1] * a[2][0])) + b[0] * (a[1][0] * a[2][1] - a[1][1] * a[2][0]));
}

struct FitOff { float xi, xr, xc; };
template <class DV>
__device__ __forceinline__ FitOff fit_step(DV dv, int L, int R, int C) {
    const float img_scale = 1.0f / (float)(255 * FIXPT_SCALE);
    const float deriv_scale = img_scale * 0.5f, second_scale = img_scale, cross_scale = img_scale * 0.25f;
    float dD[3];
    dD[0] = (dv(L, R, C + 1) - dv(L, R, C - 1)) * deriv_scale;
    dD[1] = (dv(L, R + 1, C) - dv(L, R - 1, C)) * deriv_scale;
    dD[2] = (dv(L + 1, R, C) - dv(L - 1, R, C)) * deriv_scale;
    const float v2 = dv(L, R, C) * 2.0f;
    const float dxx = (dv(L, R, C + 1) + dv(L, R, C - 1) - v2) * second_scale;
    const float dyy = (dv(L, R + 1, C) + dv(L, R - 1, C) - v2) * second_scale;
    const float dss = (dv(L + 1, R, C) + dv(L - 1, R, C) - v2) * second_scale;
    const float dxy = (dv(L, R + 1, C + 1) - dv(L, R + 1, C - 1) - dv(L, R - 1, C + 1) + dv(L, R - 1, C - 1)) * cross_scale;
    const float dxs = (dv(L + 1, R, C + 1) - dv(L + 1, R, C - 1) - dv(L - 1, R, C + 1) + dv(L - 1, R, C - 1)) * cross_scale;
    const float dys = (dv(L + 1, R + 1, C) - dv(L + 1, R - 1, C) - dv(L - 1, R + 1, C) + dv(L - 1, R - 1, C)) * cross_scale;
    const float A[3][3] = {{dxx, dxy, dxs}, {dxy, dyy, dys}, {dxs, dys, dss}};
    float X[3];
    solve3(A, dD, X);
    FitOff f; f.xi = -X[2]; f.xr = -X[1]; f.xc = -X[0];
    return f;
}
template <class DV>
__device__ __forceinline__ bool fit_accept(DV dv, int L, int R, int C, FitOff f, float contrast_thr, float edge_thr, float& contr) {
    const float img_scale = 1.0f / (float)(255 * FIXPT_SCALE);
    const float deriv_scale = img_scale * 0.5f, second_scale = img_scale, cross_scale = img_scale * 0.25f;
    float dD0 = (dv(L, R, C + 1) - dv(L, R, C - 1)) * deriv_scale;
    float dD1 = (dv(L, R + 1, C) - dv(L, R - 1, C)) * deriv_scale;
    float dD2 = (dv(L + 1, R, C) - dv(L - 1, R, C)) * deriv_scale;
    const float t = ((0.0f + dD0 * f.xc) + dD1 * f.xr) + dD2 * f.xi;
    contr = dv(L, R, C) * img_scale + t * 0.5f;
    if (fabsf(contr) * (float)N_LAYERS < contrast_thr) return false;
    const float v2 = dv(L, R, C) * 2.0f;
    const float dxx = (dv(L, R, C + 1) + dv(L, R, C - 1) - v2) * second_scale;
    const float dyy = (dv(L, R + 1, C) + dv(L, R - 1, C) - v2) * second_scale;
    const float dxy = (dv(L, R + 1, C + 1) - dv(L, R + 1, C - 1) - dv(L, R - 1, C + 1) + dv(L, R - 1, C - 1)) * cross_scale;
    const float tr = dxx + dyy, det = dxx * dyy - dxy * dxy;
    if (det <= 0.0f || (tr * tr) * edge_thr >= ((edge_thr + 1.0f) * (edge_thr + 1.0f)) * det) return false;
    return true;
}
__device__ __forceinline__ int fit_state(FitOff f) {
    if (fabsf(f.xi) < 0.5f && fabsf(f.xr) < 0.5f && fabsf(f.xc) < 0.5f) return 0;
    if (fabsf(f.xi) > 7.0e8f || fabsf(f.xr) > 7.0e8f || fabsf(f.xc) > 7.0e8f) return 1;
    if (!(f.xi == f.xi) || !(f.xr == f.xr) || !(f.xc == f.xc)) return 1;
    return 2;
}

__global__ __launch_bounds__(256) void extrema_kernel(OctaveDev oc, int octave, unsigned long long* cand, unsigned* count, unsigned cap, unsigned* overflow, BatchStride bs,
                                                      float* cube, unsigned cube_cap) {
    {
        const size_t f = blockIdx.y;
#pragma unroll
        for (int l = 0; l < N_LEVELS; l++) oc.lv[l] += f * bs.pyr;
        cand += f * bs.cand; count += f * CCNT_STRIDE; overflow += f * CNT_STRIDE; cube += f * bs.cube;
    }
    constexpr int PC = EW + 8;
    constexpr int P4 = PC / 4;
    constexpr int RW = EH + 2;
    __shared__ v4f s_d4[5][RW * P4];
    __shared__ unsigned long long s_list[ECAP];
    __shared__ unsigned s_n, s_base;
    const int tid = threadIdx.x;
    const int tiles_x = (oc.w + EW - 1) / EW, tiles_y = (oc.h + EH - 1) / EH;
    const int tile = xcd_remap(blockIdx.x, tiles_x * tiles_y);
    const int tyy = tile / tiles_x, txx = tile - tyy * tiles_x;
    const int x0 = txx * EW, y0 = tyy * EH;
    if (tid == 0) s_n = 0;
    const bool vec = ((oc.w & 3) == 0) && (x0 - 4 >= 0) && (x0 + EW + 4 <= oc.w) && ((reinterpret_cast<uintptr_t>(oc.lv[0]) & 7) == 0);
    if (vec) {
        for (int idx = tid; idx < RW * (EW / 4); idx += 256) {
            const int ry = idx / (EW / 4), c4 = idx - ry * (EW / 4);
            int gy = y0 - 1 + ry;
            gy = gy < 0 ? 0 : (gy > oc.h - 1 ? oc.h - 1 : gy);
            const size_t o = (size_t)gy * oc.w + (x0 + 4 * c4);
            v4f g[N_LEVELS];
#pragma unroll
            for (int l = 0; l < N_LEVELS; l++) g[l] = ld4(oc.lv[l] + o);
#pragma unroll
            for (int l = 0; l < 5; l++) s_d4[l][ry * P4 + 1 + c4] = g[l + 1] - g[l];
        }
        if (tid < 2 * RW) {
            const int ry = tid >> 1, side = tid & 1;
            int gy = y0 - 1 + ry;
            gy = gy < 0 ? 0 : (gy > oc.h - 1 ? oc.h - 1 : gy);
            const size_t o = (size_t)gy * oc.w + (side ? x0 + EW : x0 - 1);
            float g[N_LEVELS];
#pragma unroll
            for (int l = 0; l < N_LEVELS; l++) g[l] = ld1(oc.lv[l] + o);
#pragma unroll
            for (int l = 0; l < 5; l++) reinterpret_cast<float*>(s_d4[l])[ry * PC + (side ? 4 + EW : 3)] = g[l + 1] - g[l];
        }
    } else {
        for (int idx = tid; idx < RW * PC; idx += 256) {
            const int ry = idx / PC, rx = idx - ry * PC;
            int gy = y0 - 1 + ry, gx = x0 - 4 + rx;
            gy = gy < 0 ? 0 : (gy > oc.h - 1 ? oc.h - 1 : gy);
            gx = gx < 0 ? 0 : (gx > oc.w - 1 ? oc.w - 1 : gx);
            const size_t o = (size_t)gy * oc.w + gx;
            float g[N_LEVELS];
#pragma unroll
            for (int l = 0; l < N_LEVELS; l++) g[l] = ld1(oc.lv[l] + o);
#pragma unroll
            for (int l = 0; l < 5; l++) reinterpret_cast<float*>(s_d4[l])[idx] = g[l + 1] - g[l];
        }
    }
    __syncthreads();
    for (int item = tid; item < EH * (EW / 4); item += 256) {
        const int ly = item / (EW / 4), xg = item - ly * (EW / 4);
        const int r = y0 + ly;
        float cm[5][6], cn[5][6], mid[5][6], top[5][6], bot[5][6];
#pragma unroll
        for (int pl = 0; pl < 5; pl++) {
            const float* base = reinterpret_cast<const float*>(s_d4[pl]) + (ly + 1) * PC + 4 * xg + 4;
#pragma unroll
            for (int rr = -1; rr <= 1; rr++) {
                const float* q = base + rr * PC;
                const v4f c4 = *reinterpret_cast<const v4f*>(q);
                float v[6] = {q[-1], c4.x, c4.y, c4.z, c4.w, q[4]};
#pragma unroll
                for (int j = 0; j < 6; j++) { if (rr == -1) top[pl][j] = v[j]; else if (rr == 0) mid[pl][j] = v[j]; else bot[pl][j] = v[j]; }
            }
#pragma unroll
            for (int j = 0; j < 6; j++) {
                cm[pl][j] = fmaxf(fmaxf(top[pl][j], mid[pl][j]), bot[pl][j]);
                cn[pl][j] = fminf(fminf(top[pl][j], mid[pl][j]), bot[pl][j]);
            }
        }
        unsigned hit = 0;
#pragma unroll
        for (int k = 0; k < 4; k++) {
            const int j = k + 1;
#pragma unroll
            for (int layer = 1; layer <= N_LAYERS; layer++) {
                const float val = mid[layer][j];
                float mx = fmaxf(fmaxf(cm[layer - 1][j - 1], cm[layer - 1][j]), cm[layer - 1][j + 1]);
                mx = fmaxf(mx, fmaxf(fmaxf(cm[layer + 1][j - 1], cm[layer + 1][j]), cm[layer + 1][j + 1]));
                mx = fmaxf(mx, fmaxf(fmaxf(cm[layer][j - 1], cm[layer][j + 1]), fmaxf(top[layer][j], bot[layer][j])));
                float mn = fminf(fminf(cn[layer - 1][j - 1], cn[layer - 1][j]), cn[layer - 1][j + 1]);
                mn = fminf(mn, fminf(fminf(cn[layer + 1][j - 1], cn[layer + 1][j]), cn[layer + 1][j + 1]));
                mn = fminf(mn, fminf(fminf(cn[layer][j - 1], cn[layer][j + 1]), fminf(top[layer][j], bot[layer][j])));
                const float q = val > 0.0f ? mx : -mn;
                hit |= fabsf(val) >= fmaxf(q, DOG_THRESHOLD_P1) ? (1u << ((layer - 1) * 4 + k)) : 0u;
            }
        }
        unsigned cmask = 0;
#pragma unroll
        for (int k = 0; k < 4; k++) { const int c = x0 + 4 * xg + k; cmask |= (c >= IMG_BORDER && c < oc.w - IMG_BORDER) ? (0x111u << k) : 0u; }
        hit = (r >= IMG_BORDER && r < oc.h - IMG_BORDER) ? (hit & cmask) : 0u;
        while (hit) {
            const int bb = __builtin_ctz(hit); hit &= hit - 1;
            const int layer = bb / 4 + 1, c = x0 + 4 * xg + (bb & 3);
            const unsigned long long rec = ((unsigned long long)octave << 48) | ((unsigned long long)layer << 40) | ((unsigned long long)r << 20) | (unsigned long long)c;
            const unsigned slot = atomicAdd(&s_n, 1u);
            if (slot < ECAP) s_list[slot] = rec;
            else {
                const unsigned reg = ((unsigned)tile >> REG_SHIFT) & (NREG - 1);
                const unsigned g = atomicAdd(&count[reg * REG_STRIDE], 1u);
                if (g < cap) cand[(size_t)reg * cap + g] = rec; else *overflow = 1;
            }
        }
    }
    __syncthreads();
    const unsigned nloc = s_n < ECAP ? s_n : ECAP;
    const unsigned reg = ((unsigned)tile >> REG_SHIFT) & (NREG - 1);
    if (tid == 0 && nloc) s_base = atomicAdd(&count[reg * REG_STRIDE], nloc);
    __syncthreads();
    for (unsigned i = tid; i < nloc; i += 256) {
        const unsigned g = s_base + i;
        if (g < cap) cand[(size_t)reg * cap + g] = s_list[i] | (g < cube_cap ? (1ull << 63) : 0ull); else *overflow = 1;
    }
    for (unsigned idx = tid; idx < nloc * 27; idx += 256) {
        const unsigned ci = idx / 27, e = idx - ci * 27;
        const unsigned g = s_base + ci;
        if (g >= cube_cap) continue;
        const unsigned long long rec = s_list[ci];
        const int L0 = (int)((rec >> 40) & 0xff), R0 = (int)((rec >> 20) & 0xfffff), C0 = (int)(rec & 0xfffff);
        const int dl = (int)(e / 9) - 1, dr = (int)((e / 3) % 3) - 1, dc = (int)(e % 3) - 1;
        cube[((size_t)reg * 32 + e) * cube_cap + g] = reinterpret_cast<const float*>(s_d4[L0 + dl])[(R0 + dr - y0 + 1) * PC + (C0 + dc - x0) + 4];
    }
}

constexpr int XCAP = 144;
constexpr int XNB_CAP = 64;
constexpr int XRING_DW = 5 * 3 * 128;
constexpr int XNB_DW = 18;
constexpr int XLDS_BYTES = 4 * (XRING_DW * 4 + XCAP * 8 + XNB_CAP * XNB_DW * 4);
static_assert(XWAVES * XLDS_BYTES <= 160 * 1024 && XLDS_BYTES <= 53 * 1024, "extrema_stream: ring + list must leave room for XWAVES workgroups per CU");
typedef short s2 __attribute__((ext_vector_type(2)));
struct XRow { uint2 m[N_LEVELS]; };
struct XDog { s2 m[5][2]; };
__device__ __forceinline__ s2 as_s2(unsigned v) { return __builtin_bit_cast(s2, v); }
__device__ __forceinline__ unsigned as_u(s2 v) { return __builtin_bit_cast(unsigned, v); }
__device__ __forceinline__ s2 pmax(s2 a, s2 b) { return __builtin_elementwise_max(a, b); }
__device__ __forceinline__ s2 pmin(s2 a, s2 b) { return __builtin_elementwise_min(a, b); }
__device__ __forceinline__ unsigned dpp_lower(unsigned v) { return (unsigned)__builtin_amdgcn_update_dpp(0, (int)v, 0x138 , 0xf, 0xf, true); }
__device__ __forceinline__ unsigned dpp_upper(unsigned v) { return (unsigned)__builtin_amdgcn_update_dpp(0, (int)v, 0x130 , 0xf, 0xf, true); }

__device__ __forceinline__ unsigned xtest_row(const XDog& A, const XDog& B, const XDog& C, int xm, int clo, int chi, bool row_ok) {
    s2 hx[5][2], hn[5][2];
#pragma unroll
    for (int p = 0; p < 5; p++) {
        auto h3 = [](s2 c01, s2 c23, bool mx, s2& o01, s2& o23) {
            const unsigned u01 = as_u(c01), u23 = as_u(c23);
            const unsigned l23 = dpp_lower(u23), r01 = dpp_upper(u01);
            const s2 s_m0 = as_s2(__builtin_amdgcn_alignbit(u01, l23, 16));
            const s2 s_12 = as_s2(__builtin_amdgcn_alignbit(u23, u01, 16));
            const s2 s_34 = as_s2(__builtin_amdgcn_alignbit(r01, u23, 16));
            if (mx) { o01 = pmax(pmax(s_m0, c01), s_12); o23 = pmax(pmax(s_12, c23), s_34); }
            else    { o01 = pmin(pmin(s_m0, c01), s_12); o23 = pmin(pmin(s_12, c23), s_34); }
        };
        h3(pmax(pmax(A.m[p][0], B.m[p][0]), C.m[p][0]), pmax(pmax(A.m[p][1], B.m[p][1]), C.m[p][1]), true, hx[p][0], hx[p][1]);
        h3(pmin(pmin(A.m[p][0], B.m[p][0]), C.m[p][0]), pmin(pmin(A.m[p][1], B.m[p][1]), C.m[p][1]), false, hn[p][0], hn[p][1]);
    }
    unsigned hit = 0;
    const s2 t21 = {21, 21}, tm21 = {-21, -21};
#pragma unroll
    for (int layer = 1; layer <= N_LAYERS; layer++) {
#pragma unroll
        for (int r = 0; r < 2; r++) {
            const s2 val = B.m[layer][r];
            const s2 mx = pmax(pmax(pmax(hx[layer - 1][r], hx[layer][r]), hx[layer + 1][r]), t21);
            const s2 mn = pmin(pmin(pmin(hn[layer - 1][r], hn[layer][r]), hn[layer + 1][r]), tm21);
            const bool h0 = (val.x == mx.x) | (val.x == mn.x), h1 = (val.y == mx.y) | (val.y == mn.y);
            hit = (hit << 2) | (h0 ? 2u : 0u) | (h1 ? 1u : 0u);
        }
    }
    if (!row_ok || hit == 0) return 0u;
    unsigned out = 0;
#pragma unroll
    for (int b = 0; b < 12; b++) out |= ((hit >> (11 - b)) & 1u) << b;
    unsigned cmask = 0;
#pragma unroll
    for (int k = 0; k < 4; k++) cmask |= (xm + k >= clo && xm + k < chi) ? (0x111u << k) : 0u;
    return out & cmask;
}

struct XH { s2 hx[5][2], hn[5][2]; };
struct XCen { s2 v[3][2]; };
__device__ __forceinline__ void xrow_extremes(const XDog& d, XH& h, XCen& c) {
#pragma unroll
    for (int p = 0; p < 5; p++) {
        const unsigned u01 = as_u(d.m[p][0]), u23 = as_u(d.m[p][1]);
        const unsigned l23 = dpp_lower(u23), r01 = dpp_upper(u01);
        const s2 s_m0 = as_s2(__builtin_amdgcn_alignbit(u01, l23, 16));
        const s2 s_12 = as_s2(__builtin_amdgcn_alignbit(u23, u01, 16));
        const s2 s_34 = as_s2(__builtin_amdgcn_alignbit(r01, u23, 16));
        h.hx[p][0] = pmax(pmax(s_m0, d.m[p][0]), s_12); h.hx[p][1] = pmax(pmax(s_12, d.m[p][1]), s_34);
        h.hn[p][0] = pmin(pmin(s_m0, d.m[p][0]), s_12); h.hn[p][1] = pmin(pmin(s_12, d.m[p][1]), s_34);
    }
#pragma unroll
    for (int l = 0; l < 3; l++) { c.v[l][0] = d.m[l + 1][0]; c.v[l][1] = d.m[l + 1][1]; }
}
__device__ __forceinline__ unsigned xtest_rows(const XH& A, const XH& B, const XH& C, const XCen& cen, int xm, int clo, int chi, bool row_ok) {
    s2 hx[5][2], hn[5][2];
#pragma unroll
    for (int p = 0; p < 5; p++)
#pragma unroll
        for (int r = 0; r < 2; r++) { hx[p][r] = pmax(pmax(A.hx[p][r], B.hx[p][r]), C.hx[p][r]); hn[p][r] = pmin(pmin(A.hn[p][r], B.hn[p][r]), C.hn[p][r]); }
    unsigned hit = 0;
    const s2 t21 = {21, 21}, tm21 = {-21, -21};
#pragma unroll
    for (int layer = 1; layer <= N_LAYERS; layer++) {
#pragma unroll
        for (int r = 0; r < 2; r++) {
            const s2 val = cen.v[layer - 1][r];
            const s2 mx = pmax(pmax(pmax(hx[layer - 1][r], hx[layer][r]), hx[layer + 1][r]), t21);
            const s2 mn = pmin(pmin(pmin(hn[layer - 1][r], hn[layer][r]), hn[layer + 1][r]), tm21);
            const bool h0 = (val.x == mx.x) | (val.x == mn.x), h1 = (val.y == mx.y) | (val.y == mn.y);
            hit = (hit << 2) | (h0 ? 2u : 0u) | (h1 ? 1u : 0u);
        }
    }
    if (!row_ok || hit == 0) return 0u;
    unsigned out = 0;
#pragma unroll
    for (int b = 0; b < 12; b++) out |= ((hit >> (11 - b)) & 1u) << b;
    unsigned cmask = 0;
#pragma unroll
    for (int k = 0; k < 4; k++) cmask |= (xm + k >= clo && xm + k < chi) ? (0x111u << k) : 0u;
    return out & cmask;
}

__global__ __launch_bounds__(256) __attribute__((amdgpu_waves_per_eu(XWAVES, XWAVES)))
void extrema_stream(OctaveDev oc, int octave, unsigned long long* cand, unsigned* count, unsigned cap, unsigned* overflow, BatchStride bs,
                    float* cube, unsigned cube_cap, int L, int nstrip, int nseg, int nb, int xsw ) {
    const int lane = threadIdx.x & 63, wave = threadIdx.x >> 6;
    int unit = __builtin_amdgcn_readfirstlane(xcd_remap(blockIdx.x, gridDim.x) * 4 + wave);
    const int per = nstrip * nseg, fr = unit / per;
    if (fr >= nb) return;
    unit -= fr * per;
    {
        const size_t f = (size_t)fr;
#pragma unroll
        for (int l = 0; l < N_LEVELS; l++) oc.lv[l] += f * bs.pyr;
        cand += f * bs.cand; count += f * CCNT_STRIDE; overflow += f * CNT_STRIDE; cube += f * bs.cube;
    }
    const int seg = unit / nstrip, strip = unit - seg * nstrip;
    const int xs = strip * xsw, y0 = seg * L;
    const int lact = (oc.h - y0 < L) ? oc.h - y0 : L;
    const unsigned reg = (unsigned)unit & (NREG - 1);
    const int xm = xs - 4 + 4 * lane;
    const int xl = xm < 0 ? 0 : (xm < oc.w - 4 ? xm : oc.w - 4);
    int clo = xs > IMG_BORDER ? xs : IMG_BORDER, chi = xs + xsw < oc.w - IMG_BORDER ? xs + xsw : oc.w - IMG_BORDER;
    if (lane == 0 || lane == 63) { clo = 0; chi = 0; }
    const int hm1 = oc.h - 1;
    auto load_row = [&](int r, XRow& q) {
        r = r < 0 ? 0 : (r > hm1 ? hm1 : r);
        const size_t o = (size_t)r * oc.w + xl;
#pragma unroll
        for (int l = 0; l < N_LEVELS; l++) q.m[l] = *reinterpret_cast<const uint2*>(oc.lv[l] + o);
    };
    auto to_dog = [&](const XRow& q, XDog& d) {
#pragma unroll
        for (int p = 0; p < 5; p++) { d.m[p][0] = as_s2(q.m[p + 1].x) - as_s2(q.m[p].x); d.m[p][1] = as_s2(q.m[p + 1].y) - as_s2(q.m[p].y); }
    };
    __shared__ unsigned s_ring[4][XRING_DW];
    __shared__ unsigned long long s_rec[4][XCAP];
    __shared__ uint2 s_nb[4][XNB_CAP][XNB_DW / 2];
    static_assert(sizeof(s_ring) + sizeof(s_rec) + sizeof(s_nb) == XLDS_BYTES, "XLDS_BYTES");
    auto ring_put = [&](const XDog& d, int slot) {
        unsigned* q = &s_ring[wave][lane * 30 + slot];
#pragma unroll
        for (int p = 0; p < 5; p++) { q[p * 3] = as_u(d.m[p][0]); q[p * 3 + 15] = as_u(d.m[p][1]); }
    };
    int nq = 0;
    auto wave_sync = [&]() { __builtin_amdgcn_fence(__ATOMIC_ACQ_REL, "wavefront"); __builtin_amdgcn_wave_barrier(); };
    auto flush = [&](auto cubes) {
        constexpr bool CUBES = decltype(cubes)::value;
        if (nq == 0) return;
        wave_sync();
        unsigned base = 0;
        if (lane == 0) base = atomicAdd(&count[reg * REG_STRIDE], (unsigned)nq);
        base = __shfl(base, 0);
        for (int idx = lane; idx < nq; idx += 64) {
            const unsigned g = base + (unsigned)idx;
            if (g >= cap) { *overflow = 1; continue; }
            const unsigned long long rec = s_rec[wave][idx];
            const bool has = CUBES && idx < XNB_CAP && g < cube_cap;
            cand[(size_t)reg * cap + g] = rec | (has ? (1ull << 63) : 0ull);
            if (has) {
                const int sh = (rec & 1ull) ? 0 : 16;
                float* cb = cube + (size_t)reg * 32 * cube_cap + g;
#pragma nounroll
                for (int i = 0; i < XNB_DW / 2; i++, cb += (size_t)3 * cube_cap) {
                    const uint2 wv = s_nb[wave][idx][i];
                    const unsigned long long ww = (((unsigned long long)wv.y << 32) | wv.x) >> sh;
                    cb[0] = (float)(int)(short)(ww & 0xffffu);
                    cb[cube_cap] = (float)(int)(short)((ww >> 16) & 0xffffu);
                    cb[(size_t)2 * cube_cap] = (float)(int)(short)((ww >> 32) & 0xffffu);
                }
            }
        }
        wave_sync();
        nq = 0;
    };
    auto emit = [&](unsigned hit, int rc, auto sbc) -> bool {
        constexpr int SB = decltype(sbc)::value;
        constexpr bool IN_LOOP = SB >= 0;
        const int nq0 = nq;
        while (__builtin_amdgcn_ballot_w64(hit != 0)) {
            const bool mine = hit != 0;
            const int bb = mine ? __builtin_ctz(hit) : 0;
            hit &= hit - 1;
            const unsigned long long m = __builtin_amdgcn_ballot_w64(mine);
            const int add = __builtin_popcountll(m);
            if (nq + add > XCAP) {
                if constexpr (IN_LOOP) { nq = nq0; return false; }
                else flush(std::false_type{});
            }
            if constexpr (IN_LOOP) wave_sync();
            if (mine) {
                const int layer = bb / 4 + 1, k = bb & 3, c = xm + k;
                const int slot = nq + __builtin_popcountll(m & ((1ull << lane) - 1ull));
                s_rec[wave][slot] = ((unsigned long long)octave << 48) | ((unsigned long long)layer << 40) | ((unsigned long long)rc << 20) | (unsigned long long)c;
                if (IN_LOOP && slot < XNB_CAP) {
                    const unsigned* q = &s_ring[wave][(2 * lane + ((k + 1) >> 1) - 1) * 15 + (layer - 1) * 3];
                    uint2* nbp = s_nb[wave][slot];
                    uint2 v[XNB_DW / 2];
#pragma unroll
                    for (int pl = 0; pl < 3; pl++)
#pragma unroll
                        for (int dr = 0; dr < 3; dr++) {
                            const int o = pl * 3 + (SB + dr + 2) % 3;
                            v[pl * 3 + dr] = make_uint2(q[o], q[o + 15]);
                        }
#pragma unroll
                    for (int i = 0; i < XNB_DW / 2; i++) nbp[i] = v[i];
                }
            }
            nq += add;
        }
        return true;
    };
    XH win[3];
    XCen cen[3];
    XRow nxt[XD];
    auto prime = [&](int t) {
        XRow q; XDog dq;
        load_row(y0 + t - 1, q); to_dog(q, dq); ring_put(dq, 0); xrow_extremes(dq, win[0], cen[0]);
        load_row(y0 + t, q); to_dog(q, dq); ring_put(dq, 1); xrow_extremes(dq, win[1], cen[1]);
#pragma unroll
        for (int d = 0; d < XD; d++) load_row(y0 + t + 1 + d, nxt[d]);
    };
    prime(0);
    int tb = 0, t_slow = -1;
    for (bool done = false; !done;) {
        for (;;) {
            if (tb >= lact) { done = true; break; }
            if (nq > XNB_CAP / 2) break;
            auto step = [&](auto jc) -> bool {
                constexpr int j = decltype(jc)::value;
                const int tt = tb + j;
                if (tt >= lact) return false;
                const int rc = y0 + tt;
                XH& A = win[j % 3]; XH& B = win[(j + 1) % 3]; XH& Cc = win[(j + 2) % 3];
                { XDog dq; to_dog(nxt[j % XD], dq); ring_put(dq, (j + 2) % 3); xrow_extremes(dq, Cc, cen[(j + 2) % 3]); }
                load_row(rc + 1 + XD, nxt[j % XD]);
                const unsigned hit = xtest_rows(A, B, Cc, cen[(j + 1) % 3], xm, clo, chi, rc >= IMG_BORDER && rc < oc.h - IMG_BORDER);
                if (!emit(hit, rc, std::integral_constant<int, (j + 1) % 3>{})) { t_slow = tt; return false; }
                return true;
            };
            if (!static_rows<0, 3 * XD>(step)) { done = true; break; }
            tb += 3 * XD;
        }
        flush(std::true_type{});
    }
    if (t_slow >= 0) {
        for (int tt = t_slow; tt < lact; tt++) {
            const int rc = y0 + tt;
            XRow q; XDog A, B, Cc;
            load_row(rc - 1, q); to_dog(q, A);
            load_row(rc, q); to_dog(q, B);
            load_row(rc + 1, q); to_dog(q, Cc);
            emit(xtest_row(A, B, Cc, xm, clo, chi, rc >= IMG_BORDER && rc < oc.h - IMG_BORDER), rc, std::integral_constant<int, -1>{});
        }
        flush(std::false_type{});
    }
}

__global__ __launch_bounds__(256) void refine_kernel(PyrDev P, const unsigned long long* cand_all, const unsigned* cand_counts, unsigned cand_cap, unsigned* cand_total,
                                                     float contrast_thr, float edge_thr, float sigma,
                                                     Refined* out, unsigned* out_count, unsigned out_cap, unsigned* out_resp, BatchStride bs,
                                                     const float* cube_all, unsigned cube_cap) {
    const size_t fr = blockIdx.z, foff = fr * bs.pyr;
    cube_all += fr * bs.cube;
    cand_all += fr * bs.cand; cand_counts += fr * CCNT_STRIDE; cand_total += fr * CNT_STRIDE;
    out += fr * bs.refined; out_count += fr * CNT_STRIDE; out_resp += fr * bs.refined;
    const unsigned reg = blockIdx.y;
    unsigned n = cand_counts[reg * REG_STRIDE];
    if (n > cand_cap) n = cand_cap;
    const unsigned long long* cand = cand_all + (size_t)reg * cand_cap;
    if (blockIdx.x == 0 && blockIdx.y == 0 && threadIdx.x < 64) {
        unsigned tot = cand_counts[threadIdx.x * REG_STRIDE];
        for (int off = 32; off > 0; off >>= 1) tot += __shfl_xor(tot, off);
        if (threadIdx.x == 0) cand_total[0] = tot;
    }
    for (unsigned i = blockIdx.x * blockDim.x + threadIdx.x; i < n; i += gridDim.x * blockDim.x) {
        const unsigned long long pk = cand[i];
        const int o = (int)((pk >> 48) & 0xff);
        int L = (int)((pk >> 40) & 0xff), R = (int)((pk >> 20) & 0xfffff), C = (int)(pk & 0xfffff);
        const unsigned start = ((unsigned)L << 28) | ((unsigned)R << 14) | (unsigned)C;
        const OctaveDev& oc = P.oc[o];
        auto dv = [&](int l, int r, int c) { return dogv(oc, foff, l, r, c); };
        FitOff f = {0.0f, 0.0f, 0.0f};
        int it = 0;
        bool alive = true, accepted = false;
        float contr = 0.0f;
        const bool from_cube = (pk >> 63) != 0;
        const bool can_gather = (oc.w & 1) == 0 && (foff & 1) == 0;
        float cv[27];
        auto gather = [&](int l, int r, int c) {
            const int a0 = (c - 1) & ~1, sh = ((c - 1) & 1) * 16;
            int v[4][9];
#pragma unroll
            for (int q = 0; q < 4; q++) {
                const lvl_t* lp = oc.lv[l - 1 + q] + foff;
#pragma unroll
                for (int dr = 0; dr < 3; dr++) {
                    const uint2_a4 wv = *reinterpret_cast<const uint2_a4*>(lp + (size_t)(r - 1 + dr) * oc.w + a0);
                    const unsigned long long ww = (((unsigned long long)wv.y << 32) | wv.x) >> sh;
                    v[q][dr * 3 + 0] = (int)(short)(ww & 0xffffu); v[q][dr * 3 + 1] = (int)(short)((ww >> 16) & 0xffffu); v[q][dr * 3 + 2] = (int)(short)((ww >> 32) & 0xffffu);
                }
            }
#pragma unroll
            for (int dl = 0; dl < 3; dl++)
#pragma unroll
                for (int e = 0; e < 9; e++) cv[dl * 9 + e] = (float)(v[dl + 1][e] - v[dl][e]);
        };
        if (from_cube || can_gather) {
            for (; it < MAX_INTERP; it++) {
                if (it == 0 && from_cube) {
                    const float* cb = cube_all + (size_t)reg * 32 * cube_cap + i;
#pragma unroll
                    for (int e = 0; e < 27; e++) cv[e] = cb[(size_t)e * cube_cap];
                } else if (can_gather) gather(L, R, C);
                else break;
                const int L0 = L, R0 = R, C0 = C;
                auto dvc = [&](int l, int r, int c) { return cv[(l - L0 + 1) * 9 + (r - R0 + 1) * 3 + (c - C0 + 1)]; };
                f = fit_step(dvc, L, R, C);
                const int stt = fit_state(f);
                if (stt == 1) { alive = false; break; }
                if (stt == 0) { accepted = fit_accept(dvc, L, R, C, f, contrast_thr, edge_thr, contr); alive = accepted; break; }
                C += (int)rintf(f.xc); R += (int)rintf(f.xr); L += (int)rintf(f.xi);
                if (L < 1 || L > N_LAYERS || C < IMG_BORDER || C >= oc.w - IMG_BORDER || R < IMG_BORDER || R >= oc.h - IMG_BORDER) { alive = false; break; }
            }
            if (!alive || (can_gather && !accepted)) continue;
        }
        if (!accepted) {
            for (; it < MAX_INTERP; it++) {
                f = fit_step(dv, L, R, C);
                const int stt = fit_state(f);
                if (stt == 0) break;
                if (stt == 1) { alive = false; break; }
                C += (int)rintf(f.xc); R += (int)rintf(f.xr); L += (int)rintf(f.xi);
                if (L < 1 || L > N_LAYERS || C < IMG_BORDER || C >= oc.w - IMG_BORDER || R < IMG_BORDER || R >= oc.h - IMG_BORDER) { alive = false; break; }
            }
            if (!alive || it >= MAX_INTERP) continue;
            if (!fit_accept(dv, L, R, C, f, contrast_thr, edge_thr, contr)) continue;
        }
        const size_t bit = ((size_t)R * oc.w + C) * 4 + (size_t)L;
        const unsigned mask = 1u << (bit & 31);
        if (!P.mins[o]) {
            const unsigned old = atomicOr(&P.claimed[o][fr * bs.claimed + (bit >> 5)], mask);
            if (old & mask) continue;
        }
        const unsigned long long act = __ballot(1);
        const int leader = __builtin_ctzll(act), lane_id = (int)(threadIdx.x & 63);
        unsigned slot = 0;
        if (lane_id == leader) slot = atomicAdd(out_count, (unsigned)__builtin_popcountll(act));
        slot = __shfl(slot, leader) + (unsigned)__builtin_popcountll(act & ((1ull << lane_id) - 1ull));
        if (slot < out_cap) {
            Refined rr;
            rr.o = o; rr.layer = L; rr.r = R; rr.c = C; rr.xi = f.xi; rr.xr = f.xr; rr.xc = f.xc; rr.contr = contr;
            rr.scl = sigma * det_exp2f(((float)L + f.xi) / (float)N_LAYERS);
            rr.start = start;
            out[slot] = rr;
            out_resp[slot] = __float_as_uint(fabsf(contr));
            if (P.mins[o]) atomicMin(&P.mins[o][fr * bs.mins + bit], start);
        } else if (!P.mins[o]) atomicAnd(&P.claimed[o][fr * bs.claimed + (bit >> 5)], ~mask);
    }
}

__device__ __forceinline__ void unclaim_body(const PyrDev& P, const Refined* ref, const unsigned* ref_count, unsigned ref_cap, const BatchStride& bs, size_t fr, unsigned first, unsigned step) {
    ref += fr * bs.refined; ref_count += fr * CNT_STRIDE;
    unsigned n = *ref_count;
    if (n > ref_cap) n = ref_cap;
    for (unsigned i = first; i < n; i += step) {
        const Refined rr = ref[i];
        const size_t bit = ((size_t)rr.r * P.oc[rr.o].w + rr.c) * 4 + (size_t)rr.layer;
        atomicAnd(&P.claimed[rr.o][fr * bs.claimed + (bit >> 5)], ~(1u << (bit & 31)));
    }
}

__global__ __launch_bounds__(256) void keepall_live_kernel(PyrDev P, const Refined* ref, const unsigned* ref_count, unsigned ref_cap, unsigned* ctrl, unsigned* list, BatchStride bs) {
    const size_t fr = blockIdx.y;
    ref += fr * bs.refined; ref_count += fr * CNT_STRIDE; ctrl += fr * CNT_STRIDE; list += fr * bs.refined;
    unsigned n = *ref_count;
    if (n > ref_cap) n = ref_cap;
    const int lane = threadIdx.x & 63;
    for (unsigned i0 = blockIdx.x * blockDim.x; i0 < n; i0 += gridDim.x * blockDim.x) {
        const unsigned i = i0 + threadIdx.x;
        bool take = false;
        if (i < n) {
            const Refined rr = ref[i];
            const size_t bit = ((size_t)rr.r * P.oc[rr.o].w + rr.c) * 4 + (size_t)rr.layer;
            take = P.mins[rr.o][fr * bs.mins + bit] == rr.start;
        }
        const unsigned long long m = __builtin_amdgcn_ballot_w64(take);
        if (m) {
            const int first = __builtin_ctzll(m);
            unsigned base = 0;
            if (lane == first) base = atomicAdd(&ctrl[2], (unsigned)__builtin_popcountll(m));
            base = __shfl(base, first);
            if (take) list[base + (unsigned)__builtin_popcountll(m & ((1ull << lane) - 1ull))] = i;
        }
    }
}
__global__ __launch_bounds__(256) void keepall_reset_kernel(PyrDev P, const Refined* ref, const unsigned* ref_count, unsigned ref_cap, BatchStride bs) {
    const size_t fr = blockIdx.y;
    ref += fr * bs.refined; ref_count += fr * CNT_STRIDE;
    unsigned n = *ref_count;
    if (n > ref_cap) n = ref_cap;
    for (unsigned i = blockIdx.x * blockDim.x + threadIdx.x; i < n; i += gridDim.x * blockDim.x) {
        const Refined rr = ref[i];
        P.mins[rr.o][fr * bs.mins + ((size_t)rr.r * P.oc[rr.o].w + rr.c) * 4 + (size_t)rr.layer] = 0xffffffffu;
    }
}

struct KpRec {
    unsigned resp_bits; int o, layer, r, c, bin;
    float ptx, pty, scl, angle, xi;
    unsigned start;
};

constexpr int UNCLAIM_WGS = 32;
__global__ __launch_bounds__(1024) void select_unclaim_kernel(PyrDev P, const Refined* ref, BatchStride bs,
                                                              const unsigned* resp , const unsigned* ref_count, unsigned ref_cap,
                                                              unsigned want, unsigned* ctrl , size_t resp_stride,
                                                              unsigned* list ) {
    if (blockIdx.x > 0) { unclaim_body(P, ref, ref_count, ref_cap, bs, blockIdx.y, (blockIdx.x - 1) * 1024 + threadIdx.x, (gridDim.x - 1) * 1024); return; }
    resp += (size_t)blockIdx.y * resp_stride; ref_count += (size_t)blockIdx.y * CNT_STRIDE; ctrl += (size_t)blockIdx.y * CNT_STRIDE;
    list += (size_t)blockIdx.y * resp_stride;
    __shared__ unsigned s_h[16][256];
    __shared__ unsigned s_sel[2], s_cnt;
    const int tid = threadIdx.x, wv = tid >> 6;
    unsigned n = *ref_count;
    if (n > ref_cap) n = ref_cap;
    if (n <= want) {
        if (tid == 0) { ctrl[0] = 0; ctrl[1] = 0; ctrl[2] = n; }
        for (unsigned i = tid; i < n; i += 1024) list[i] = i;
        return;
    }
    const unsigned nr = (n + 1023u) & ~1023u;
    unsigned above = 0, hi_sel = 0;
    for (int pass = 0; pass < 2; pass++) {
        for (int i = tid; i < 16 * 256; i += 1024) (&s_h[0][0])[i] = 0;
        __syncthreads();
        for (unsigned i0 = tid; i0 < nr; i0 += 8 * 1024) {
            unsigned vv[8];
#pragma unroll
            for (int u = 0; u < 8; u++) { const unsigned i = i0 + 1024u * u; vv[u] = i < n ? resp[i] : 0u; }
#pragma unroll
            for (int u = 0; u < 8; u++) {
                if (i0 + 1024u * u >= n) continue;
                const unsigned key = (vv[u] >> 15) & 0xffffu;
                if (pass == 0) atomicAdd(&s_h[wv][key >> 8], 1u);
                else if ((key >> 8) == hi_sel) atomicAdd(&s_h[wv][key & 255u], 1u);
            }
        }
        __syncthreads();
        if (tid < 256) { unsigned t = 0; for (int w = 0; w < 16; w++) t += s_h[w][tid]; s_h[0][tid] = t; }
        __syncthreads();
        if (tid == 0) {
            unsigned cum = above; int b = 255;
            for (; b >= 0; b--) { if (cum + s_h[0][b] >= want) break; cum += s_h[0][b]; }
            if (b < 0) b = 0;
            s_sel[0] = (unsigned)b; s_sel[1] = cum;
        }
        __syncthreads();
        if (pass == 0) { hi_sel = s_sel[0]; above = s_sel[1]; }
        else if (tid == 0) { ctrl[0] = ((hi_sel << 8) | s_sel[0]) << 15; ctrl[1] = 0; s_cnt = 0; }
        __syncthreads();
    }
    const unsigned T = ((hi_sel << 8) | s_sel[0]) << 15;
    const int lane = tid & 63;
    for (unsigned i0 = tid; i0 < nr; i0 += 8 * 1024) {
        unsigned vv[8];
#pragma unroll
        for (int u = 0; u < 8; u++) { const unsigned i = i0 + 1024u * u; vv[u] = i < n ? resp[i] : 0u; }
#pragma unroll
        for (int u = 0; u < 8; u++) {
            const unsigned i = i0 + 1024u * u;
            const bool take = i < n && vv[u] >= T;
            const unsigned long long m = __builtin_amdgcn_ballot_w64(take);
            if (m) {
                const int first = __builtin_ctzll(m);
                unsigned base = 0;
                if (lane == first) base = atomicAdd(&s_cnt, (unsigned)__builtin_popcountll(m));
                base = __shfl(base, first);
                if (take) list[base + (unsigned)__builtin_popcountll(m & ((1ull << lane) - 1ull))] = i;
            }
        }
    }
    __syncthreads();
    if (tid == 0) ctrl[2] = s_cnt;
}

static_assert(sizeof(lvl_t) == 2, "level_taps forms byte offsets of 2-byte samples in 32 bits");
struct LevelTaps { lvl_t e, w, n, s; };
__device__ __forceinline__ LevelTaps level_taps(const lvl_t* lvl, int cols, int r, int c) {
    const char* b = (const char*)lvl;
    const unsigned row = 2u * (unsigned)cols, o = 2u * ((unsigned)r * (unsigned)cols + (unsigned)c);
    LevelTaps t;
    t.e = *(const lvl_t*)(b + o + 2); t.w = *(const lvl_t*)(b + o - 2);
    t.n = *(const lvl_t*)(b + (o - row)); t.s = *(const lvl_t*)(b + (o + row));
    return t;
}
__device__ __forceinline__ void level_grad(const LevelTaps& t, float& dx, float& dy) {
    dx = (float)((int)t.e - (int)t.w); dy = (float)((int)t.n - (int)t.s);
}

constexpr int OCAP = 256;
__global__ __launch_bounds__(256) void orient_kernel(PyrDev P, const Refined* ref, const unsigned* ref_count, unsigned ref_cap,
                                                     KpRec* out, unsigned* out_resp, unsigned* out_count, unsigned out_cap,
                                                     const unsigned* ctrl, int pass, BatchStride bs, const unsigned* list) {
    const size_t fr = blockIdx.y, foff = fr * bs.pyr;
    ref += fr * bs.refined; ref_count += fr * CNT_STRIDE; out += fr * bs.kps; out_resp += fr * bs.kps; out_count += fr * CNT_STRIDE; ctrl += fr * CNT_STRIDE;
    list += fr * bs.refined;
    __shared__ unsigned long long s_hq[4][ORI_BINS];
    const unsigned Tbits = ctrl[0];
    if (pass == 1 && (ctrl[1] == 0 || Tbits == 0)) return;
    __shared__ float s_hist[4][ORI_BINS + 4];
    __shared__ KpRec s_out[OCAP];
    __shared__ unsigned s_on, s_obase;
    const int tid = threadIdx.x, lane = tid & 63, wv = tid >> 6;
    unsigned n = *ref_count;
    if (n > ref_cap) n = ref_cap;
    if (pass == 0) n = ctrl[2] < n ? ctrl[2] : n;
    if (tid == 0) s_on = 0;
    __syncthreads();
    for (unsigned base = blockIdx.x * 4; base < n; base += gridDim.x * 4) {
        unsigned k = base + wv;
        bool take = false;
        if (k < n) {
            if (pass == 0) { k = list[k]; take = true; }
            else take = __float_as_uint(fabsf(ref[k].contr)) < Tbits;
        }
        if (take) {
            const Refined rr = ref[k];
            const OctaveDev& oc = P.oc[__builtin_amdgcn_readfirstlane(rr.o)];
            const lvl_t* img = oc.lv[__builtin_amdgcn_readfirstlane(rr.layer)] + foff;
            const int radius = (int)rintf(4.5f * rr.scl);
            const float osig = 1.5f * rr.scl;
            const float expf_scale = -1.0f / (2.0f * osig * osig);
            const int side = 2 * radius + 1, S = side * side;
            if (lane < ORI_BINS) s_hq[wv][lane] = 0ull;
            __builtin_amdgcn_fence(__ATOMIC_ACQ_REL, "workgroup");
            __builtin_amdgcn_wave_barrier();
            const int per = (S + 63) / 64;
            int sc = lane * per, ic = sc / side, jc = sc - ic * side;
            for (int k0 = 0; k0 < per; k0 += 4) {
                LevelTaps tv[4]; int d2v[4]; bool okv[4];
#pragma unroll
                for (int u = 0; u < 4; u++) {
                    const int s = k0 + u < per ? sc : S;
                    const int i = ic - radius, j = jc - radius;
                    sc++; jc++;
                    if (jc == side) { jc = 0; ic++; }
                    const int y = rr.r + i, x = rr.c + j;
                    okv[u] = (s < S) && !(y <= 0 || y >= oc.h - 1 || x <= 0 || x >= oc.w - 1);
                    d2v[u] = i * i + j * j;
                    tv[u] = LevelTaps{0, 0, 0, 0};
                    if (okv[u]) tv[u] = level_taps(img, oc.w, y, x);
                }
#pragma unroll
                for (int u = 0; u < 4; u++) {
                    if (!okv[u]) continue;
                    float dx, dy;
                    level_grad(tv[u], dx, dy);
                    const float wgt = det_expf((float)d2v[u] * expf_scale);
                    const float ang = det_atan2deg(dy, dx);
                    const float mag = sqrtf(dx * dx + dy * dy);
                    int b = (int)rintf(((float)ORI_BINS / 360.0f) * ang);
                    if (b >= ORI_BINS) b -= ORI_BINS;
                    if (b < 0) b += ORI_BINS;
                    const float t = wgt * mag;
                    atomicAdd(&s_hq[wv][b], (unsigned long long)(unsigned)(int)rintf(t * HIST_Q));
                }
            }
            __builtin_amdgcn_fence(__ATOMIC_ACQ_REL, "workgroup");
            __builtin_amdgcn_wave_barrier();
            if (lane < ORI_BINS) s_hist[wv][lane] = (float)(long long)s_hq[wv][lane] * (1.0f / HIST_Q);
            __builtin_amdgcn_fence(__ATOMIC_ACQ_REL, "workgroup");
            __builtin_amdgcn_wave_barrier();
            float hs = 0.0f;
            if (lane < ORI_BINS) {
                const float m2 = s_hist[wv][(lane + ORI_BINS - 2) % ORI_BINS], m1 = s_hist[wv][(lane + ORI_BINS - 1) % ORI_BINS];
                const float p1 = s_hist[wv][(lane + 1) % ORI_BINS], p2 = s_hist[wv][(lane + 2) % ORI_BINS];
                hs = ((m2 + p2) * (1.0f / 16.0f) + (m1 + p1) * (4.0f / 16.0f)) + s_hist[wv][lane] * (6.0f / 16.0f);
            }
            float omax = hs;
            for (int off = 32; off > 0; off >>= 1) { const float o2 = __shfl_xor(omax, off); omax = o2 > omax ? o2 : omax; }
            const float hl = __shfl(hs, lane > 0 ? lane - 1 : ORI_BINS - 1);
            const float hr = __shfl(hs, lane < ORI_BINS - 1 ? lane + 1 : 0);
            const float mag_thr = omax * 0.8f;
            if (lane < ORI_BINS && hs > hl && hs > hr && hs >= mag_thr) {
                float bf = (float)lane + (0.5f * (hl - hr)) / ((hl - 2.0f * hs) + hr);
                bf = bf < 0.0f ? (float)ORI_BINS + bf : (bf >= (float)ORI_BINS ? bf - (float)ORI_BINS : bf);
                KpRec kr;
                kr.resp_bits = __float_as_uint(fabsf(rr.contr));
                kr.o = rr.o; kr.layer = rr.layer; kr.r = rr.r; kr.c = rr.c; kr.bin = lane;
                kr.ptx = (float)rr.c + rr.xc; kr.pty = (float)rr.r + rr.xr; kr.scl = rr.scl; kr.xi = rr.xi; kr.start = rr.start;
                kr.angle = (360.0f / (float)ORI_BINS) * bf;
                const unsigned slot = atomicAdd(&s_on, 1u);
                if (slot < OCAP) s_out[slot] = kr;
            }
        }
        __syncthreads();
        const bool last = base + gridDim.x * 4 >= n;
        if (s_on > OCAP - 72 || last) {
            const unsigned cntl = s_on < OCAP ? s_on : OCAP;
            if (tid == 0 && cntl) s_obase = atomicAdd(out_count, cntl);
            __syncthreads();
            for (unsigned i = tid; i < cntl; i += 256) {
                const unsigned g = s_obase + i;
                if (g < out_cap) { out[g] = s_out[i]; out_resp[g] = s_out[i].resp_bits; }
            }
            __syncthreads();
            if (tid == 0) s_on = 0;
            __syncthreads();
        }
    }
}

constexpr int TOPK_CAP = 4096;

struct SelRec { float ptx, pty, scl, angle; int o, layer; };

__device__ __forceinline__ unsigned long long tie_key(const KpRec& k) {
    return ((unsigned long long)k.o << 52) | ((unsigned long long)k.layer << 48) | ((unsigned long long)k.r << 28) | ((unsigned long long)k.c << 8) | (unsigned long long)k.bin;
}

__global__ __launch_bounds__(1024) void topk_kernel(const KpRec* kps, const unsigned* resp, const unsigned* kp_count, unsigned kp_cap, int nfeatures,
                                                    FrameOuts outs, SelRec* out_sel, int* out_n, int* overflow, unsigned* ctrl, int pass, BatchStride bs) {
    const size_t fr = blockIdx.x;
    kps += fr * bs.kps; resp += fr * bs.kps; kp_count += fr * CNT_STRIDE; out_sel += fr * bs.sel; out_n += fr * CNT_STRIDE; overflow += fr * CNT_STRIDE; ctrl += fr * CNT_STRIDE;
    mi355_keypoint* out_kp = outs.kp[0];
#pragma unroll
    for (int q = 1; q < SIFT_BATCH_MAX; q++) if ((int)fr == q) out_kp = outs.kp[q];
    __shared__ unsigned s_hist[256];
    if (pass == 1 && (ctrl[1] == 0 || ctrl[0] == 0)) return;
    __shared__ unsigned s_misc[8];
    __shared__ unsigned long long s_k0[TOPK_CAP];
    __shared__ unsigned long long s_k1[TOPK_CAP];
    __shared__ unsigned s_idx[TOPK_CAP];
    const int tid = threadIdx.x, lane = tid & 63;
    unsigned N = *kp_count;
    if (N > kp_cap) { N = kp_cap; if (tid == 0) *overflow = 1; }
    const unsigned K = (unsigned)nfeatures;
    unsigned thresh = 0;
    if (N > K) {
        unsigned prefix = 0, want = K;
        const unsigned Nr = (N + 1023u) & ~1023u;
        for (int pass = 0; pass < 4; pass++) {
            const int shift = 24 - 8 * pass;
            for (int i = tid; i < 256; i += 1024) s_hist[i] = 0;
            __syncthreads();
            const unsigned himask = pass == 0 ? 0u : (0xffffffffu << (shift + 8));
            for (unsigned i0 = tid; i0 < Nr; i0 += 8 * 1024) {
                unsigned vv[8];
#pragma unroll
                for (int u = 0; u < 8; u++) { const unsigned i = i0 + 1024u * u; vv[u] = i < N ? resp[i] : 0u; }
#pragma unroll
                for (int u = 0; u < 8; u++) {
                    const unsigned i = i0 + 1024u * u;
                    if (i0 + 1024u * u - tid >= Nr) break;
                    const unsigned v = vv[u];
                    const bool valid = (i < N) && ((v & himask) == prefix);
                    const unsigned d = (v >> shift) & 255u;
                    unsigned long long peers = __ballot(valid);
#pragma unroll
                    for (int b = 0; b < 8; b++) {
                        const unsigned long long m = __ballot(valid && ((d >> b) & 1u));
                        peers &= ((d >> b) & 1u) ? m : ~m;
                    }
                    if (valid && (peers & ((1ull << lane) - 1ull)) == 0ull) atomicAdd(&s_hist[d], (unsigned)__popcll(peers));
                }
            }
            __syncthreads();
            if (tid == 0) {
                unsigned cum = 0; int b = 255;
                for (; b >= 0; b--) { if (cum + s_hist[b] >= want) break; cum += s_hist[b]; }
                if (b < 0) b = 0;
                s_misc[0] = (unsigned)b; s_misc[1] = want - cum;
            }
            __syncthreads();
            prefix |= s_misc[0] << shift; want = s_misc[1];
            __syncthreads();
        }
        thresh = prefix;
    }
    if (tid == 0) s_misc[2] = 0;
    for (int i = tid; i < TOPK_CAP; i += 1024) { s_k0[i] = ~0ull; s_k1[i] = ~0ull; s_idx[i] = 0xffffffffu; }
    __syncthreads();
    for (unsigned i0 = tid; i0 < N; i0 += 8 * 1024) {
        unsigned vv[8];
#pragma unroll
        for (int u = 0; u < 8; u++) { const unsigned i = i0 + 1024u * u; vv[u] = i < N ? resp[i] : 0u; }
#pragma unroll
        for (int u = 0; u < 8; u++) {
            const unsigned i = i0 + 1024u * u;
            if (i < N && vv[u] >= thresh) {
                const KpRec k = kps[i];
                const unsigned slot = atomicAdd(&s_misc[2], 1u);
                if (slot < TOPK_CAP) { s_k0[slot] = (unsigned long long)(~k.resp_bits); s_k1[slot] = tie_key(k); s_idx[slot] = i; }
            }
        }
    }
    __syncthreads();
    unsigned M = s_misc[2];
    if (M > TOPK_CAP) { M = TOPK_CAP; if (tid == 0) *overflow = 1; }
    if (N > K && M > (unsigned)SEL_STRIDE && tid == 0) *overflow = 1;
    int SN = 64;
    while ((unsigned)SN < M) SN <<= 1;
    for (int k = 2; k <= SN; k <<= 1) {
        for (int j = k >> 1; j > 0; j >>= 1) {
            for (int i = tid; i < SN; i += 1024) {
                const int ixj = i ^ j;
                if (ixj > i) {
                    const unsigned long long a0 = s_k0[i], a1 = s_k1[i], b0 = s_k0[ixj], b1 = s_k1[ixj];
                    const bool gt = (a0 > b0) || (a0 == b0 && a1 > b1);
                    const bool up = (i & k) == 0;
                    if (gt == up) {
                        s_k0[i] = b0; s_k1[i] = b1; s_k0[ixj] = a0; s_k1[ixj] = a1;
                        const unsigned t = s_idx[i]; s_idx[i] = s_idx[ixj]; s_idx[ixj] = t;
                    }
                }
            }
            __syncthreads();
        }
    }
    const unsigned keep = N > K ? (M < (unsigned)SEL_STRIDE ? M : (unsigned)SEL_STRIDE) : M;
    for (unsigned i = tid; i < keep; i += 1024) {
        const KpRec k = kps[s_idx[i]];
        const float s2 = (float)(1 << k.o);
        mi355_keypoint kp;
        kp.x = k.ptx * s2; kp.y = k.pty * s2; kp.size = (k.scl * s2) * 2.0f; kp.angle = k.angle;
        kp.response = __uint_as_float(k.resp_bits);
        kp.octave = (k.o & 255) | (k.layer << 8) | (((int)rintf((k.xi + 0.5f) * 255.0f)) << 16);
        kp.class_id = -1;
        out_kp[i] = kp;
        SelRec sr; sr.ptx = k.ptx; sr.pty = k.pty; sr.scl = k.scl; sr.angle = k.angle; sr.o = k.o; sr.layer = k.layer;
        out_sel[i] = sr;
    }
    if (tid == 0) {
        *out_n = (int)keep;
        if (pass == 0 && ctrl[0] != 0 && keep < K) ctrl[1] = 1;
    }
}

__device__ __forceinline__ unsigned long long keepall_key(const KpRec& k) {
    return ((unsigned long long)k.o << 40) | ((unsigned long long)k.start << 6) | (unsigned long long)k.bin;
}

__device__ __forceinline__ void keepall_emit(const KpRec& k, mi355_keypoint* out_kp, SelRec* out_sel, unsigned pos) {
    const float s2 = (float)(1 << k.o);
    mi355_keypoint kp;
    kp.x = k.ptx * s2; kp.y = k.pty * s2; kp.size = (k.scl * s2) * 2.0f; kp.angle = k.angle;
    kp.response = __uint_as_float(k.resp_bits);
    kp.octave = (k.o & 255) | (k.layer << 8) | (((int)rintf((k.xi + 0.5f) * 255.0f)) << 16);
    kp.class_id = -1;
    out_kp[pos] = kp;
    SelRec sr; sr.ptx = k.ptx; sr.pty = k.pty; sr.scl = k.scl; sr.angle = k.angle; sr.o = k.o; sr.layer = k.layer;
    out_sel[pos] = sr;
}

__device__ __forceinline__ bool keepall_fits(unsigned N, unsigned kp_cap, unsigned kmax, int* out_n, int* overflow, bool writer) {
    if (N <= kp_cap && N <= kmax) return true;
    if (writer) { if (N > kp_cap) *overflow = 1; *out_n = 0; }
    return false;
}


__global__ __launch_bounds__(1024) void keepall_sort_tiles_kernel(const KpRec* kps, const unsigned* kp_count, unsigned kp_cap, unsigned kmax, unsigned long long* sorted,
                                                                  size_t sorted_stride, FrameOuts outs, SelRec* out_sel, BatchStride bs) {
    const size_t fr = blockIdx.y;
    kps += fr * bs.kps; kp_count += fr * CNT_STRIDE; sorted += fr * sorted_stride; out_sel += fr * bs.sel;
    const unsigned N = *kp_count;
    if (N > kp_cap || N > kmax) return;
    const unsigned t0 = blockIdx.x * KA_TILE;
    if (t0 >= N) return;
    __shared__ unsigned long long s[KA_TILE];
    const int tid = threadIdx.x;
    for (int q = tid; q < KA_TILE; q += 1024) s[q] = t0 + q < N ? (keepall_key(kps[t0 + q]) << 18) | (unsigned long long)(t0 + q) : ~0ull;
    __syncthreads();
    const int lane = tid & 63, p0 = (tid >> 6) * 128 + lane;
    for (int k = 2; k <= KA_TILE; k <<= 1) {
        for (int j = k >> 1; j > 0; j >>= 1) {
#pragma unroll
            for (int h = 0; h < 2; h++) {
                const int p = p0 + 64 * h, i = 2 * p - (p & (j - 1)), ixj = i + j;
                const unsigned long long a = s[i], b = s[ixj];
                if ((a > b) == ((i & k) == 0)) { s[i] = b; s[ixj] = a; }
            }
            if (j >= 256 || (j == 1 && k >= 256)) __syncthreads();
            else { __builtin_amdgcn_fence(__ATOMIC_ACQ_REL, "workgroup"); __builtin_amdgcn_wave_barrier(); }
        }
    }
    if (N <= (unsigned)KA_TILE) {
        mi355_keypoint* out_kp = outs.kp[0];
#pragma unroll
        for (int q = 1; q < SIFT_BATCH_MAX; q++) if ((int)fr == q) out_kp = outs.kp[q];
        for (unsigned q = tid; q < N; q += 1024) keepall_emit(kps[(unsigned)(s[q] & 0x3ffffu)], out_kp, out_sel, q);
        return;
    }
    for (int q = tid; q < KA_TILE; q += 1024) sorted[t0 + q] = s[q];
}

__global__ __launch_bounds__(256) void keepall_place_kernel(const KpRec* kps, const unsigned* kp_count, unsigned kp_cap, unsigned kmax, const unsigned long long* sorted,
                                                            size_t sorted_stride, FrameOuts outs, SelRec* out_sel, int* out_n, int* overflow, BatchStride bs) {
    const size_t fr = blockIdx.y;
    kps += fr * bs.kps; kp_count += fr * CNT_STRIDE; sorted += fr * sorted_stride; out_sel += fr * bs.sel; out_n += fr * CNT_STRIDE; overflow += fr * CNT_STRIDE;
    const unsigned N = *kp_count;
    if (!keepall_fits(N, kp_cap, kmax, out_n, overflow, blockIdx.x == 0 && threadIdx.x == 0)) return;
    if (blockIdx.x == 0 && threadIdx.x == 0) *out_n = (int)N;
    if (N <= (unsigned)KA_TILE) return;
    const unsigned i = blockIdx.x * 256 + threadIdx.x;
    if (i >= N) return;
    mi355_keypoint* out_kp = outs.kp[0];
#pragma unroll
    for (int q = 1; q < SIFT_BATCH_MAX; q++) if ((int)fr == q) out_kp = outs.kp[q];
    const KpRec k = kps[i];
    const unsigned long long key = keepall_key(k) << 18;
    const unsigned nt = (N + KA_TILE - 1) / KA_TILE;
    unsigned rank = 0, t = 0;
    for (; t + 4 <= nt; t += 4) {
        unsigned pos[4] = {0u, 0u, 0u, 0u};
        const unsigned long long* a = sorted + (size_t)t * KA_TILE;
        for (unsigned step = KA_TILE / 2; step > 0; step >>= 1) {
#pragma unroll
            for (int u = 0; u < 4; u++) if (a[(size_t)u * KA_TILE + pos[u] + step - 1] < key) pos[u] += step;
        }
#pragma unroll
        for (int u = 0; u < 4; u++) rank += pos[u] + (a[(size_t)u * KA_TILE + pos[u]] < key ? 1u : 0u);
    }
    for (; t < nt; t++) {
        const unsigned long long* a = sorted + (size_t)t * KA_TILE;
        unsigned pos = 0;
        for (unsigned step = KA_TILE / 2; step > 0; step >>= 1) if (a[pos + step - 1] < key) pos += step;
        rank += pos + (a[pos] < key ? 1u : 0u);
    }
    keepall_emit(k, out_kp, out_sel, rank);
}

__global__ __launch_bounds__(256) void describe_kernel(PyrDev P, const SelRec* sel, const int* n_sel, FrameOuts outs, BatchStride bs) {
    const size_t fr = blockIdx.y, foff = fr * bs.pyr;
    sel += fr * bs.sel; n_sel += fr * CNT_STRIDE;
    uint8_t* desc = outs.d8[0];
#pragma unroll
    for (int q = 1; q < SIFT_BATCH_MAX; q++) if ((int)fr == q) desc = outs.d8[q];
    constexpr int d = 4, n = 8, HB = (d + 2) * (d + 2) * (n + 2);
    __shared__ unsigned long long s_hq4[4][HB];
    __shared__ float s_dst4[4][128];
    const int lane = threadIdx.x & 63, wv = threadIdx.x >> 6;
    const int kidx = blockIdx.x * 4 + wv;
    if (kidx >= *n_sel) return;
    unsigned long long* s_hq = s_hq4[wv];
    float* s_dst = s_dst4[wv];
    auto wave_sync = [&]() { __builtin_amdgcn_fence(__ATOMIC_ACQ_REL, "workgroup"); __builtin_amdgcn_wave_barrier(); };
    const SelRec k = sel[kidx];
    const OctaveDev& oc = P.oc[__builtin_amdgcn_readfirstlane(k.o)];
    const lvl_t* img = oc.lv[__builtin_amdgcn_readfirstlane(k.layer)] + foff;
    const int rows = oc.h, cols = oc.w;
    for (int i = lane; i < HB; i += 64) s_hq[i] = 0ull;
    wave_sync();
    const int px = (int)rintf(k.ptx), py = (int)rintf(k.pty);
    float sin_t, cos_t;
    det_sincosdeg(k.angle, sin_t, cos_t);
    const float bins_per_deg = (float)n / 360.0f;
    const float exp_scale = -1.0f / ((float)(d * d) * 0.5f);
    const float hist_width = 3.0f * k.scl;
    const int radius = (int)rintf(hist_width * 1.4142135623730951f * (float)(d + 1) * 0.5f);
    cos_t = cos_t / hist_width; sin_t = sin_t / hist_width;
    const int side = 2 * radius + 1, S = side * side;
    __shared__ int s_q4[4][64 * 5];
    int* s_q = s_q4[wv];
    int qn = 0;
    bool pending = false;
    int p_word = 0;
    LevelTaps p_taps = {0, 0, 0, 0};
    auto fetch = [&](int packed) {
        const int i = (int)((unsigned)packed >> 16) - 32768, j = (int)((unsigned)packed & 0xffffu) - 32768;
        return level_taps(img, cols, py + i, px + j);
    };
    auto heavy = [&](int packed, const LevelTaps& taps) {
        const int i = (int)((unsigned)packed >> 16) - 32768, j = (int)((unsigned)packed & 0xffffu) - 32768;
        const float c_rot = (float)j * cos_t - (float)i * sin_t;
        const float r_rot = (float)j * sin_t + (float)i * cos_t;
        float rbin = r_rot + (float)(d / 2) - 0.5f;
        float cbin = c_rot + (float)(d / 2) - 0.5f;
        float dx, dy;
        level_grad(taps, dx, dy);
        const float ori = det_atan2deg(dy, dx);
        const float mag = sqrtf(dx * dx + dy * dy) * det_expf((c_rot * c_rot + r_rot * r_rot) * exp_scale);
        float obin = (ori - k.angle) * bins_per_deg;
        const float r0f = floorf(rbin), c0f = floorf(cbin), o0f = floorf(obin);
        rbin -= r0f; cbin -= c0f; obin -= o0f;
        const int r0 = (int)r0f, c0 = (int)c0f;
        int o0 = (int)o0f;
        if (o0 < 0) o0 += n;
        if (o0 >= n) o0 -= n;
        const float v_r1 = mag * rbin, v_r0 = mag - v_r1;
        const float v_rc11 = v_r1 * cbin, v_rc10 = v_r1 - v_rc11;
        const float v_rc01 = v_r0 * cbin, v_rc00 = v_r0 - v_rc01;
        const float v_rco111 = v_rc11 * obin, v_rco110 = v_rc11 - v_rco111;
        const float v_rco101 = v_rc10 * obin, v_rco100 = v_rc10 - v_rco101;
        const float v_rco011 = v_rc01 * obin, v_rco010 = v_rc01 - v_rco011;
        const float v_rco001 = v_rc00 * obin, v_rco000 = v_rc00 - v_rco001;
        const int idx = ((r0 + 1) * (d + 2) + c0 + 1) * (n + 2) + o0;
#define FIXQ(v) ((unsigned long long)(unsigned)(int)rintf((v) * HIST_Q))
        atomicAdd(&s_hq[idx], FIXQ(v_rco000)); atomicAdd(&s_hq[idx + 1], FIXQ(v_rco001));
        atomicAdd(&s_hq[idx + (n + 2)], FIXQ(v_rco010)); atomicAdd(&s_hq[idx + (n + 3)], FIXQ(v_rco011));
        atomicAdd(&s_hq[idx + (d + 2) * (n + 2)], FIXQ(v_rco100)); atomicAdd(&s_hq[idx + (d + 2) * (n + 2) + 1], FIXQ(v_rco101));
        atomicAdd(&s_hq[idx + (d + 3) * (n + 2)], FIXQ(v_rco110)); atomicAdd(&s_hq[idx + (d + 3) * (n + 2) + 1], FIXQ(v_rco111));
#undef FIXQ
    };
    const int per = (S + 63) / 64;
    int sc = lane * per, ic = sc / side, jc = sc - ic * side;
    for (int k0 = 0; k0 < per; k0 += 4) {
#pragma unroll
        for (int u = 0; u < 4; u++) {
            const int kk = k0 + u;
            const int i = ic - radius, j = jc - radius;
            const float c_rot = (float)j * cos_t - (float)i * sin_t;
            const float r_rot = (float)j * sin_t + (float)i * cos_t;
            const float rbin = r_rot + (float)(d / 2) - 0.5f;
            const float cbin = c_rot + (float)(d / 2) - 0.5f;
            const int r = py + i, c = px + j;
            const bool ok = kk < per && sc < S && (rbin > -1.0f && rbin < (float)d && cbin > -1.0f && cbin < (float)d && r > 0 && r < rows - 1 && c > 0 && c < cols - 1);
            const unsigned long long m = __builtin_amdgcn_ballot_w64(ok);
            if (ok) s_q[qn + __builtin_popcountll(m & ((1ull << lane) - 1ull))] = (int)(((unsigned)(i + 32768) << 16) | (unsigned)(j + 32768));
            qn += __builtin_popcountll(m);
            sc++; jc++;
            if (jc == side) { jc = 0; ic++; }
        }
        wave_sync();
        while (qn >= 64) {
            qn -= 64;
            const int word = s_q[qn + lane];
            const LevelTaps taps = fetch(word);
            if (pending) heavy(p_word, p_taps);
            p_word = word; p_taps = taps; pending = true;
        }
        wave_sync();
    }
    const bool tail = lane < qn;
    int t_word = 0;
    LevelTaps t_taps = {0, 0, 0, 0};
    if (tail) { t_word = s_q[lane]; t_taps = fetch(t_word); }
    if (pending) heavy(p_word, p_taps);
    if (tail) heavy(t_word, t_taps);
    wave_sync();
#pragma unroll
    for (int half = 0; half < 2; half++) {
        const int t = lane + 64 * half;
        const int cell = t >> 3, q = t & 7, i = cell >> 2, j = cell & 3;
        const int idx = ((i + 1) * (d + 2) + (j + 1)) * (n + 2);
        float v = (float)(long long)s_hq[idx + q] * (1.0f / HIST_Q);
        if (q < 2) v = v + (float)(long long)s_hq[idx + n + q] * (1.0f / HIST_Q);
        s_dst[t] = v;
    }
    wave_sync();
    float a = s_dst[lane], b = s_dst[lane + 64];
    auto seq_sum = [&](float va, float vb) {
        const float sa = va * va, sb = vb * vb;
        float acc = 0.0f;
#pragma unroll
        for (int q = 0; q < 64; q++) acc = acc + __int_as_float(__builtin_amdgcn_readlane(__float_as_int(sa), q));
#pragma unroll
        for (int q = 0; q < 64; q++) acc = acc + __int_as_float(__builtin_amdgcn_readlane(__float_as_int(sb), q));
        return acc;
    };
    const float thr = sqrtf(seq_sum(a, b)) * 0.2f;
    a = a < thr ? a : thr; b = b < thr ? b : thr;
    const float nn = sqrtf(seq_sum(a, b));
    const float fac = 512.0f / (nn > 1.1920929e-7f ? nn : 1.1920929e-7f);
    const float va = rintf(a * fac), vb = rintf(b * fac);
    desc[(size_t)kidx * 128 + lane] = (uint8_t)(va < 0.0f ? 0 : (va > 255.0f ? 255 : (int)va));
    desc[(size_t)kidx * 128 + lane + 64] = (uint8_t)(vb < 0.0f ? 0 : (vb > 255.0f ? 255 : (int)vb));
}

struct BlurFn { void (*stream)(Blur16Args, int, int, int); void (*tile)(Blur16Args); };
template <bool BGR>
BlurFn blur_kernel(const Launch& L) {
    const bool w4 = L.waves == 4;
    if (L.kind == BLUR_STREAM) {
        if constexpr (BGR) return {w4 ? blur16_stream<6, true, false, 4> : blur16_stream<6, true, false, 3>, nullptr};
        else switch (L.radius) {
            case 5: return {w4 ? blur16_stream<5, false, false, 4> : blur16_stream<5, false, false, 3>, nullptr};
            case 6: return {w4 ? blur16_stream<6, false, false, 4> : blur16_stream<6, false, false, 3>, nullptr};
            case 8: if (L.ds) return {w4 ? blur16_stream<8, false, true, 4> : blur16_stream<8, false, true, 3>, nullptr};
                    return {w4 ? blur16_stream<8, false, false, 4> : blur16_stream<8, false, false, 3>, nullptr};
            case 10: return {blur16_stream<10, false, false, 3>, nullptr};
            case 13: return {blur16_stream<13, false, false, 3>, nullptr};
        }
    }
    switch (L.radius) {
#define CASE(RR) case RR: return {nullptr, blur16_tile<RR, BGR>};
        CASE(2) CASE(3) CASE(4) CASE(5) CASE(6) CASE(7) CASE(8) CASE(9) CASE(10) CASE(11) CASE(12) CASE(13) CASE(14) CASE(15) CASE(16)
#undef CASE
    }
    return {nullptr, nullptr};
}

struct SiftBufs {
    DevBuf pyr;
    DevBuf claimed;
    DevBuf cand, refined, kps, kresp, sel, counters, rhist, ccnt;
    DevBuf olist;
    DevBuf mins;
    DevBuf ksort;
    DevBuf cube;
    hipError_t reserve(const Layout& l, int nb, hipStream_t st) {
        const Strides& bs = l.bs;
        const struct { DevBuf* b; size_t bytes; } want[] = {
            {&pyr, bs.pyr * sizeof(lvl_t)}, {&claimed, bs.claimed * sizeof(unsigned)}, {&cand, bs.cand * sizeof(unsigned long long)},
            {&refined, bs.refined * sizeof(Refined)}, {&kps, bs.kps * sizeof(KpRec)}, {&kresp, bs.kps * sizeof(unsigned)}, {&sel, bs.sel * sizeof(SelRec)},
            {&mins, bs.mins * sizeof(unsigned)}, {&ksort, l.ksort_stride * sizeof(unsigned long long)}, {&counters, CNT_STRIDE * sizeof(unsigned)},
            {&rhist, bs.refined * sizeof(unsigned)}, {&olist, bs.refined * sizeof(unsigned)}, {&ccnt, CCNT_STRIDE * sizeof(unsigned)}, {&cube, bs.cube * sizeof(float)}};
        for (const auto& w : want) {
            if (!w.bytes) { w.b->release(); continue; }
            if (const hipError_t e = w.b->reserve((size_t)nb * w.bytes); e != hipSuccess) return e;
        }
        if (const hipError_t e = hipMemsetAsync(claimed.p, 0, (size_t)nb * bs.claimed * sizeof(unsigned), st); e != hipSuccess) return e;
        return l.keepall ? hipMemsetAsync(mins.p, 0xff, (size_t)nb * bs.mins * sizeof(unsigned), st) : hipSuccess;
    }
    void release() { for (DevBuf* b : {&pyr, &claimed, &cand, &refined, &kps, &kresp, &sel, &counters, &rhist, &ccnt, &olist, &mins, &ksort, &cube}) b->release(); }
};

}

struct SiftWork {
    Layout lay;
    int nb = 0;
    hipStream_t stream = nullptr;
    hipEvent_t done = nullptr;
    SiftBufs b;
    PyrDev P;
    BatchStride bs;
    struct Pend { int img_id; const uint8_t* d_bgr; int ws; hipEvent_t ev; };
    std::vector<Pend> pend;
};

constexpr int SIFT_SLOTS_MAX = 4;
#define SIFT_SLOTS (ctx->sift_nslots)

void mi_sift_release(mi355_ctx* ctx) {
    for (SiftWork* s : ctx->sift_slots) {
        if (!s) continue;
        if (s->stream) { (void)hipStreamSynchronize(s->stream); (void)hipStreamDestroy(s->stream); }
        if (s->done) (void)hipEventDestroy(s->done);
        s->b.release();
        delete s;
    }
    ctx->sift_slots.clear();
    if (ctx->sift_in_ev) { (void)hipEventDestroy(ctx->sift_in_ev); ctx->sift_in_ev = nullptr; }
    for (int* p : ctx->pinned_chunks) (void)hipHostFree(p);
    ctx->pinned_chunks.clear();
    ctx->pinned_used = 0;
}

static int sift_run_batch(mi355_ctx* ctx, SiftWork* s);

int mi_sift_flush(mi355_ctx* ctx) {
    int rc = MI355_OK;
    for (SiftWork* s : ctx->sift_slots) if (s && !s->pend.empty()) { const int r = sift_run_batch(ctx, s); if (r != MI355_OK) rc = r; }
    return rc;
}

static int adopt_counts(mi355_ctx* ctx, int img_id, Features& f) {
    f.pending = false;
    if (!f.h_cnt) { f.n = 0; return MI355_OK; }
    const volatile int* c = f.h_cnt;
    for (int i = 0; i < 8; i++) ctx->last_counts[i] = c[i];
    if ((unsigned)c[0] > f.caps[0] || (unsigned)c[1] > f.caps[1] || (unsigned)c[2] > f.caps[2] || c[4]) {
        ctx->set_error("sift: candidate buffer overflow (image " + std::to_string(img_id) + " has more extrema than the buffers assume)");
        f.n = 0;
        return MI355_ERR_FAILED;
    }
    if (f.kp_limit > 0 && c[2] > f.kp_limit) {
        ctx->set_error("sift: keep-all frame (image " + std::to_string(img_id) + ") has " + std::to_string(c[2]) + " keypoints, more than keepall_max=" +
                       std::to_string(f.kp_limit));
        f.n = 0;
        return MI355_ERR_FAILED;
    }
    f.n = c[3];
    return MI355_OK;
}

int mi_resolve_features(mi355_ctx* ctx) {
    int rc = mi_sift_flush(ctx);
    bool any = false;
    for (auto& kv : ctx->feats) if (kv.second.pending) { any = true; break; }
    if (!any) { ctx->batch_events_used = 0; return rc; }
    for (SiftWork* s : ctx->sift_slots) if (s && s->stream) MI_HIP(hipStreamSynchronize(s->stream));
    for (auto& kv : ctx->feats) {
        if (!kv.second.pending) continue;
        const int r = adopt_counts(ctx, kv.first, kv.second);
        if (r != MI355_OK) rc = r;
    }
    ctx->batch_events_used = 0;
    return rc;
}

int mi_resolve_features_of(mi355_ctx* ctx, const int* ids, int n) {
    int rc = MI355_OK;
    bool parked = false;
    for (int k = 0; k < n && !parked; k++) {
        auto it = ctx->feats.find(ids[k]);
        if (it != ctx->feats.end() && it->second.pending && !it->second.h_cnt && !it->second.ready) parked = true;
    }
    if (parked) rc = mi_sift_flush(ctx);
    for (int k = 0; k < n; k++) {
        auto it = ctx->feats.find(ids[k]);
        if (it == ctx->feats.end() || !it->second.pending) continue;
        Features& f = it->second;
        if (f.ready) MI_HIP(hipEventSynchronize(f.ready));
        else { const int r = mi_resolve_features(ctx); if (r != MI355_OK) rc = r; continue; }
        const int r = adopt_counts(ctx, it->first, f);
        if (r != MI355_OK) rc = r;
    }
    return rc;
}

static constexpr size_t PINNED_CHUNK = 4096;

static int* pinned_slot(mi355_ctx* ctx) {
    const size_t chunk = ctx->pinned_used / PINNED_CHUNK, off = ctx->pinned_used % PINNED_CHUNK;
    if (chunk >= ctx->pinned_chunks.size()) {
        int* p = nullptr;
        if (hipHostMalloc((void**)&p, PINNED_CHUNK * 8 * sizeof(int), hipHostMallocDefault) != hipSuccess) return nullptr;
        ctx->pinned_chunks.push_back(p);
    }
    ctx->pinned_used++;
    return ctx->pinned_chunks[chunk] + off * 8;
}

static int sift_prepare(mi355_ctx* ctx, SiftWork* s, const Layout& lay, int nb) {
    if (s->lay.same_key(lay) && s->nb == nb) return MI355_OK;
    MI_HIP(hipStreamSynchronize(s->stream));
    MI_HIP(s->b.reserve(lay, nb, s->stream));
    if ((((uintptr_t)s->b.pyr.p) | ((uintptr_t)s->b.claimed.p)) & 127) { ctx->set_error("sift: work area is not 128-byte aligned"); return MI355_ERR_FAILED; }
    memset(&s->P, 0, sizeof(s->P));
    for (int o = 0; o < lay.n_oct; o++) {
        const Octave& oc = lay.oc[o];
        s->P.oc[o].w = oc.w; s->P.oc[o].h = oc.h;
        for (int i = 0; i < N_LEVELS; i++) s->P.oc[o].lv[i] = s->b.pyr.as<lvl_t>() + oc.lv[i];
        s->P.claimed[o] = s->b.claimed.as<unsigned>() + oc.claimed;
        s->P.mins[o] = lay.keepall ? s->b.mins.as<unsigned>() + oc.mins : nullptr;
    }
    s->P.n_oct = lay.n_oct;
    s->bs = BatchStride{lay.bs.pyr, lay.bs.claimed, lay.bs.cand, lay.bs.refined, lay.bs.kps, lay.bs.cube, lay.bs.sel, lay.bs.mins};
    s->lay = lay; s->nb = nb;
    return MI355_OK;
}

int mi_sift_extract_dev(mi355_ctx* ctx, int img_id, const uint8_t* d_bgr, int w, int h, int ws, int* n_kp) {
    if (ctx->p.n_octave_layers != N_LAYERS || ctx->p.sigma != 1.6f) { ctx->set_error("sift: this build implements nOctaveLayers=3, sigma=1.6 (the reference's SIFT(2000,3,0.01,20))"); return MI355_ERR_ARG; }
    if (ctx->p.nfeatures > 2048) { ctx->set_error("sift: nfeatures must be in [1,2048], or <= 0 for cv::SIFT's keep-all (up to keepall_max=" + std::to_string(ctx->keepall_max) + " keypoints per frame)"); return MI355_ERR_ARG; }
    const bool keepall = ctx->p.nfeatures <= 0;
    const int kmax = keepall ? ctx->keepall_max : 0;
    if (keepall && (w > 16384 || h > 16384)) { ctx->set_error("sift: keep-all frames are at most 16384 x 16384"); return MI355_ERR_ARG; }
    std::string refused;
    const Layout lay = make_layout(w, h, keepall, kmax, refused);
    if (!refused.empty()) { ctx->set_error(refused); return MI355_ERR_ARG; }
    if (ctx->sift_slots.empty()) {
        ctx->sift_slots.resize(SIFT_SLOTS_MAX, nullptr);
        MI_HIP(hipEventCreateWithFlags(&ctx->sift_in_ev, hipEventDisableTiming));
    }
    if (ctx->sift_next >= SIFT_SLOTS) ctx->sift_next = 0;
    const int slot = ctx->sift_next;
    if (!ctx->sift_slots[slot]) {
        ctx->sift_slots[slot] = new SiftWork();
        MI_HIP(hipStreamCreateWithFlags(&ctx->sift_slots[slot]->stream, hipStreamNonBlocking));
        MI_HIP(hipEventCreateWithFlags(&ctx->sift_slots[slot]->done, hipEventDisableTiming));
    }
    SiftWork* s = ctx->sift_slots[slot];
    int rc = MI355_OK;
    static const size_t total_mem = [] { size_t fr = 0, tot = 0; return hipMemGetInfo(&fr, &tot) == hipSuccess ? tot : (size_t)0; }();
    const int nb = batch_frames(w, h, keepall, ctx->sift_batch, SIFT_SLOTS, total_mem);
    if (!s->pend.empty() && !(s->lay.same_key(lay) && s->nb == nb)) { rc = sift_run_batch(ctx, s); if (rc != MI355_OK) return rc; }
    rc = sift_prepare(ctx, s, lay, nb);
    if (rc != MI355_OK) return rc;
    auto fit = ctx->feats.find(img_id);
    if (fit != ctx->feats.end() && fit->second.pending) { rc = mi_resolve_features(ctx); if (rc != MI355_OK) return rc; }
    Features& f = ctx->feats[img_id];
    f.w = w; f.h = h;
    MI_HIP(f.kp.reserve(sizeof(mi355_keypoint) * (size_t)(keepall ? kmax : 2048)));
    MI_HIP(f.d8.reserve((size_t)128 * (size_t)(keepall ? kmax : 2048)));
    f.pending = true; f.h_cnt = nullptr; f.ready = nullptr; f.n = 0;
    s->pend.push_back({img_id, d_bgr, ws, ctx->pend_event});
    if ((int)s->pend.size() >= nb) {
        rc = sift_run_batch(ctx, s);
        if (rc != MI355_OK) return rc;
    }
    if (ctx->pinned_used >= PINNED_CHUNK * 64) {
        rc = mi_resolve_features(ctx);
        if (rc != MI355_OK) return rc;
        ctx->pinned_used = 0;
    }
    if (n_kp) {
        rc = mi_resolve_features(ctx);
        if (rc != MI355_OK) return rc;
        *n_kp = f.n;
    }
    return MI355_OK;
}

struct BatchRun {
    mi355_ctx* ctx; SiftWork* s; hipStream_t st;
    std::vector<SiftWork::Pend> pend;
    std::vector<Features*> fs;
    int n;
    unsigned* cnt;
    FrameOuts outs;
    int enqueue_pyramid();
    void enqueue_keypoints();
    int publish_batch();
};

int BatchRun::enqueue_pyramid() {
    const PyramidTaps& taps = pyramid_taps();
    Routes routes = {ctx->blur_stream, ctx->xstream_min_w, ctx->xstream_min_frames, true};
    for (const SiftWork::Pend& p : pend) routes.base_frames_aligned = routes.base_frames_aligned && ((uintptr_t)p.d_bgr & 3) == 0 && (p.ws & 3) == 0 && p.ws >= 3 * s->lay.w;
    for (const Launch& L : pyramid_launches(s->lay, n, routes)) {
        const OctaveDev& oc = s->P.oc[L.octave];
        const dim3 grid(L.gx, L.gy, L.gz), block(256);
        switch (L.kind) {
            case BLUR_STREAM: case BLUR_TILE: {
                const bool base = L.level == 0;
                const Taps& t = base ? taps.base : taps.lv[L.level];
                Blur16Args a; memset(&a, 0, sizeof(a));
                a.w = oc.w; a.h = oc.h; a.tiles_x = (oc.w + T16W - 1) / T16W; a.tiles_y = (oc.h + T16H - 1) / T16H;
                a.fstride = s->bs.pyr; a.nb = n;
                if (base) for (int k = 0; k < n; k++) { a.bgr[k] = pend[k].d_bgr; a.bgr_ws[k] = pend[k].ws; }
                else a.src = oc.lv[L.level - 1];
                a.dst = oc.lv[L.level];
                if (L.ds) a.ds = s->P.oc[L.octave + 1].lv[0];
                memcpy(a.k, t.k, sizeof(float) * (2 * t.r + 1));
                const BlurFn k = base ? blur_kernel<true>(L) : blur_kernel<false>(L);
                if (!k.stream && !k.tile) { ctx->set_error("sift: unsupported kernel radius"); return MI355_ERR_FAILED; }
                ProfScope ps(ctx, k.stream ? "gauss_stream" : "gauss", L.bytes, st);
                if (k.stream) {
                    for (int i = 0; i <= t.r; i++) { a.kp[2 * i] = a.k[i]; a.kp[2 * i + 1] = i ? a.k[i - 1] : 0.0f; }
                    hipLaunchKernelGGL(k.stream, grid, block, 0, st, a, L.L, L.nstrip, L.nseg);
                } else hipLaunchKernelGGL(k.tile, grid, block, 0, st, a);
                break;
            }
            case DOWNSAMPLE: {
                const OctaveDev& pv = s->P.oc[L.octave - 1];
                ProfScope ps(ctx, "downsample", L.bytes, st);
                hipLaunchKernelGGL(downsample16, grid, block, 0, st, pv.lv[N_LAYERS], pv.w, oc.lv[0], oc.w, oc.h, s->bs.pyr);
                break;
            }
            case EXTREMA_STREAM: case EXTREMA_TILE: {
                ProfScope ps(ctx, "extrema", L.bytes, st);
                const SiftBufs& d = s->b;
                if (L.kind == EXTREMA_STREAM) hipLaunchKernelGGL(extrema_stream, grid, block, 0, st, oc, L.octave, d.cand.as<unsigned long long>(), d.ccnt.as<unsigned>(), s->lay.cand_cap, cnt + 4, s->bs,
                                                                 d.cube.as<float>(), s->lay.cube_cap, L.L, L.nstrip, L.nseg, n, L.xsw);
                else hipLaunchKernelGGL(extrema_kernel, grid, block, 0, st, oc, L.octave, d.cand.as<unsigned long long>(), d.ccnt.as<unsigned>(), s->lay.cand_cap, cnt + 4, s->bs, d.cube.as<float>(), s->lay.cube_cap);
                break;
            }
        }
    }
    return MI355_OK;
}

void BatchRun::enqueue_keypoints() {
    const SiftBufs& d = s->b;
    const Layout& lay = s->lay;
    const BatchStride bs = s->bs;
    const unsigned kmax = (unsigned)lay.kmax;
    {
        ProfScope ps(ctx, "refine", 0.0, st);
        hipLaunchKernelGGL(refine_kernel, dim3(REFINE_GX, NREG, n), dim3(256), 0, st, s->P, d.cand.as<unsigned long long>(), d.ccnt.as<unsigned>(), lay.cand_cap, cnt + 0,
                           ctx->p.contrast_threshold, ctx->p.edge_threshold, 1.6f, d.refined.as<Refined>(), cnt + 1, lay.ref_cap, d.rhist.as<unsigned>(), bs, d.cube.as<float>(), lay.cube_cap);
    }
    {
        ProfScope ps(ctx, "kp_select", 0.0, st);
        if (lay.keepall) {
            hipLaunchKernelGGL(keepall_live_kernel, dim3(256, n), dim3(256), 0, st, s->P, d.refined.as<Refined>(), cnt + 1, lay.ref_cap, cnt + 8, d.olist.as<unsigned>(), bs);
            hipLaunchKernelGGL(keepall_reset_kernel, dim3(256, n), dim3(256), 0, st, s->P, d.refined.as<Refined>(), cnt + 1, lay.ref_cap, bs);
        } else {
            hipLaunchKernelGGL(select_unclaim_kernel, dim3(1 + UNCLAIM_WGS, n), dim3(1024), 0, st, s->P, d.refined.as<Refined>(), bs, d.rhist.as<unsigned>(), cnt + 1, lay.ref_cap,
                               (unsigned)ctx->p.nfeatures + 256u, cnt + 8, bs.refined, d.olist.as<unsigned>());
        }
    }
    for (int pass = 0; pass < (lay.keepall ? 1 : 2); pass++) {
        {
            ProfScope ps(ctx, "orient", 0.0, st);
            hipLaunchKernelGGL(orient_kernel, dim3(ctx->num_cu * 4, n), dim3(256), 0, st, s->P, d.refined.as<Refined>(), cnt + 1, lay.ref_cap,
                               d.kps.as<KpRec>(), d.kresp.as<unsigned>(), cnt + 2, lay.kp_cap, cnt + 8, pass, bs, d.olist.as<unsigned>());
        }
        ProfScope ps(ctx, "topk", 0.0, st);
        if (lay.keepall) {
            hipLaunchKernelGGL(keepall_sort_tiles_kernel, dim3((kmax + KA_TILE - 1) / KA_TILE, n), dim3(1024), 0, st, d.kps.as<KpRec>(), cnt + 2, lay.kp_cap, kmax,
                               d.ksort.as<unsigned long long>(), lay.ksort_stride, outs, d.sel.as<SelRec>(), bs);
            hipLaunchKernelGGL(keepall_place_kernel, dim3((kmax + 255) / 256, n), dim3(256), 0, st, d.kps.as<KpRec>(), cnt + 2, lay.kp_cap, kmax,
                               d.ksort.as<const unsigned long long>(), lay.ksort_stride, outs, d.sel.as<SelRec>(), reinterpret_cast<int*>(cnt + 3), reinterpret_cast<int*>(cnt + 4), bs);
        } else {
            hipLaunchKernelGGL(topk_kernel, dim3(n), dim3(1024), 0, st, d.kps.as<KpRec>(), d.kresp.as<unsigned>(), cnt + 2, lay.kp_cap, ctx->p.nfeatures,
                               outs, d.sel.as<SelRec>(), reinterpret_cast<int*>(cnt + 3), reinterpret_cast<int*>(cnt + 4), cnt + 8, pass, bs);
        }
    }
    ProfScope ps(ctx, "describe", 0.0, st);
    hipLaunchKernelGGL(describe_kernel, dim3(((int)bs.sel + 3) / 4, n), dim3(256), 0, st, s->P, d.sel.as<SelRec>(), reinterpret_cast<const int*>(cnt + 3), outs, bs);
}

int BatchRun::publish_batch() {
    const Layout& lay = s->lay;
    { int rc = mi_finish_features_batch(ctx, fs.data(), n, reinterpret_cast<const int*>(cnt + 3), (int)CNT_STRIDE, st, lay.keepall ? lay.kmax : 2048); if (rc != MI355_OK) return rc; }
    if (ctx->pinned_used % PINNED_CHUNK + (size_t)n > PINNED_CHUNK) ctx->pinned_used += PINNED_CHUNK - ctx->pinned_used % PINNED_CHUNK;
    int* h0 = nullptr;
    for (int k = 0; k < n; k++) {
        int* hc = pinned_slot(ctx);
        if (!hc) { ctx->set_error("sift: pinned alloc failed"); return MI355_ERR_NOMEM; }
        if (k == 0) h0 = hc;
        Features& f = *fs[k];
        f.h_cnt = hc; f.pending = true; f.n = 0;
        f.caps[0] = 0xffffffffu; f.caps[1] = lay.ref_cap; f.caps[2] = lay.kp_cap;
        f.kp_limit = lay.keepall ? lay.kmax : 0;
    }
    MI_HIP(hipMemcpy2DAsync(h0, 8 * sizeof(int), cnt, CNT_STRIDE * sizeof(unsigned), 8 * sizeof(unsigned), (size_t)n, hipMemcpyDeviceToHost, st));
    MI_HIP(hipEventRecord(s->done, st));
    if (ctx->batch_events_used >= ctx->batch_events.size()) {
        hipEvent_t e = nullptr;
        MI_HIP(hipEventCreateWithFlags(&e, hipEventDisableTiming));
        ctx->batch_events.push_back(e);
    }
    hipEvent_t e = ctx->batch_events[ctx->batch_events_used++];
    MI_HIP(hipEventRecord(e, st));
    for (int k = 0; k < n; k++) fs[k]->ready = e;
    for (int k = 0; k < n; k++) if (pend[k].ev) MI_HIP(hipEventRecord(pend[k].ev, st));
    return MI355_OK;
}

static int sift_run_batch(mi355_ctx* ctx, SiftWork* s) {
    BatchRun b = {};
    b.ctx = ctx; b.s = s;
    b.pend.swap(s->pend);
    const int n = b.n = (int)b.pend.size();
    if (n == 0) return MI355_OK;
    ctx->sift_next = (ctx->sift_next + 1) % SIFT_SLOTS;
    const hipStream_t st = b.st = s->stream;
    MI_HIP(hipEventRecord(ctx->sift_in_ev, ctx->stream));
    MI_HIP(hipStreamWaitEvent(st, ctx->sift_in_ev, 0));
    const bool serial_heavy = ctx->serial_heavy != 0;
    if (serial_heavy && ctx->heavy_ev_valid) MI_HIP(hipStreamWaitEvent(st, ctx->heavy_ev, 0));
    b.cnt = s->b.counters.as<unsigned>();
    MI_HIP(hipMemsetAsync(b.cnt, 0, (size_t)n * CNT_STRIDE * sizeof(unsigned), st));
    MI_HIP(hipMemsetAsync(s->b.ccnt.p, 0, (size_t)n * CCNT_STRIDE * sizeof(unsigned), st));
    for (int k = 0; k < n; k++) {
        Features* f = &ctx->feats[b.pend[k].img_id];
        b.fs.push_back(f);
        b.outs.kp[k] = f->kp.as<mi355_keypoint>(); b.outs.d8[k] = f->d8.as<uint8_t>();
    }
    { const int rc = b.enqueue_pyramid(); if (rc != MI355_OK) return rc; }
    if (serial_heavy) {
        if (!ctx->heavy_ev) MI_HIP(hipEventCreateWithFlags(&ctx->heavy_ev, hipEventDisableTiming));
        MI_HIP(hipEventRecord(ctx->heavy_ev, st)); ctx->heavy_ev_valid = true;
    }
    b.enqueue_keypoints();
    MI_HIP(hipGetLastError());
    return b.publish_batch();
}

int mi_sift_flush_if_parked(mi355_ctx* ctx, hipEvent_t ev) {
    for (SiftWork* s : ctx->sift_slots) {
        if (!s) continue;
        for (const SiftWork::Pend& p : s->pend) if (p.ev == ev) return sift_run_batch(ctx, s);
    }
    return MI355_OK;
}
```

Measured before the change: 4105 image-pairs/s.

## Replace claimed-bitmap dedup with post-select hash dedup and refine-fused key histogram

Removes the per-octave claimed bitmap, along with its atomicOr/atomicAnd in refine and the separate unclaim pass, and deduplicates refined extrema only among the top-response candidates, using an LDS or global open-addressing hash. Refine now builds the 65536-bin response-key histogram with wave-aggregated atomics, so the select kernel skips its two histogram passes and finds the threshold with a single prefix scan. The topk fallback path builds its own deduplicated list for the second orient pass. New nfeatures and select_margin options are added. The risks are extra histogram atomics in refine, hash overflow handling, and a possible change in which keypoints survive if dedup ordering differs.

```diff
diff --git a/imagemosaicing_amd/capi.py b/imagemosaicing_amd/capi.py
--- a/imagemosaicing_amd/capi.py
+++ b/imagemosaicing_amd/capi.py
@@ -286,6 +286,8 @@
 
     def set_option(self, name, value):
         self._chk(self.L.mi355_set_option(self._h, name.encode(), int(value)))
+        if name == "nfeatures":
+            self.params.nfeatures = int(value)
 
     def profile_enable(self, on=True):
         self._chk(self.L.mi355_profile_enable(self._h, int(bool(on))))
diff --git a/imagemosaicing_amd/csrc/api.hip b/imagemosaicing_amd/csrc/api.hip
--- a/imagemosaicing_amd/csrc/api.hip
+++ b/imagemosaicing_amd/csrc/api.hip
@@ -393,6 +393,20 @@
         ctx->keepall_max = value;
         return MI355_OK;
     }
+    if (std::string(name) == "nfeatures") {
+        if (value > 2048) { ctx->set_error("set_option: nfeatures must be in [1, 2048], or <= 0 for keep-all"); return MI355_ERR_ARG; }
+        int rc = mi_resolve_features(ctx);
+        if (rc != MI355_OK) return rc;
+        ctx->p.nfeatures = value;
+        return MI355_OK;
+    }
+    if (std::string(name) == "select_margin") {
+        if (value < 0 || value > 65536) { ctx->set_error("set_option: select_margin must be in [0, 65536]"); return MI355_ERR_ARG; }
+        int rc = mi_resolve_features(ctx);
+        if (rc != MI355_OK) return rc;
+        ctx->select_margin = value;
+        return MI355_OK;
+    }
     if (std::string(name) == "big_subpairs_max") { ctx->big_sub_max = value < 1 ? 1 : value; return MI355_OK; }
     {
         struct { const char* n; int* p; } knobs[] = {{"ransac_split", &ctx->ransac_split}, {"strict_frames", &ctx->strict_frames}};
diff --git a/imagemosaicing_amd/csrc/common.h b/imagemosaicing_amd/csrc/common.h
--- a/imagemosaicing_amd/csrc/common.h
+++ b/imagemosaicing_amd/csrc/common.h
@@ -149,6 +149,7 @@
     SurfState* surf = nullptr;
     int keepall_max = MI355_SIFT_KEEPALL_MAX;
     int big_sub_max = 65536;
+    int select_margin = 256;
     int last_counts[8] = {0};
 
     void set_error(const std::string& s) { err = s; }
diff --git a/imagemosaicing_amd/csrc/sift.hip b/imagemosaicing_amd/csrc/sift.hip
--- a/imagemosaicing_amd/csrc/sift.hip
+++ b/imagemosaicing_amd/csrc/sift.hip
@@ -213,12 +213,12 @@
 
 constexpr int ECAP = 128;
 constexpr int REG_STRIDE = 32;
-struct BatchStride { size_t pyr, claimed, cand, refined, kps, cube, sel, mins; };
+struct BatchStride { size_t pyr, cand, refined, kps, cube, sel, mins; };
 struct FrameOuts { mi355_keypoint* kp[SIFT_BATCH_MAX]; uint8_t* d8[SIFT_BATCH_MAX]; };
 
 struct Refined { int o, layer, r, c; float xi, xr, xc, contr, scl; unsigned start; };
 
-struct PyrDev { OctaveDev oc[MAX_OCT]; unsigned* claimed[MAX_OCT]; unsigned* mins[MAX_OCT]; int n_oct; };
+struct PyrDev { OctaveDev oc[MAX_OCT]; unsigned* mins[MAX_OCT]; int n_oct; };
 
 __device__ __forceinline__ float dogv(const OctaveDev& oc, size_t foff, int lvl, int r, int c) {
     const size_t o = foff + (size_t)r * oc.w + c;
@@ -672,10 +672,11 @@
     }
 }
 
+constexpr unsigned KEY_BINS = 65536;
 __global__ __launch_bounds__(256) void refine_kernel(PyrDev P, const unsigned long long* cand_all, const unsigned* cand_counts, unsigned cand_cap, unsigned* cand_total,
                                                      float contrast_thr, float edge_thr, float sigma,
                                                      Refined* out, unsigned* out_count, unsigned out_cap, unsigned* out_resp, BatchStride bs,
-                                                     const float* cube_all, unsigned cube_cap) {
+                                                     const float* cube_all, unsigned cube_cap, unsigned* khist ) {
     const size_t fr = blockIdx.z, foff = fr * bs.pyr;
     cube_all += fr * bs.cube;
     cand_all += fr * bs.cand; cand_counts += fr * CCNT_STRIDE; cand_total += fr * CNT_STRIDE;
@@ -752,12 +753,6 @@
             if (!alive || it >= MAX_INTERP) continue;
             if (!fit_accept(dv, L, R, C, f, contrast_thr, edge_thr, contr)) continue;
         }
-        const size_t bit = ((size_t)R * oc.w + C) * 4 + (size_t)L;
-        const unsigned mask = 1u << (bit & 31);
-        if (!P.mins[o]) {
-            const unsigned old = atomicOr(&P.claimed[o][fr * bs.claimed + (bit >> 5)], mask);
-            if (old & mask) continue;
-        }
         const unsigned long long act = __ballot(1);
         const int leader = __builtin_ctzll(act), lane_id = (int)(threadIdx.x & 63);
         unsigned slot = 0;
@@ -770,19 +765,18 @@
             rr.start = start;
             out[slot] = rr;
             out_resp[slot] = __float_as_uint(fabsf(contr));
-            if (P.mins[o]) atomicMin(&P.mins[o][fr * bs.mins + bit], start);
-        } else if (!P.mins[o]) atomicAnd(&P.claimed[o][fr * bs.claimed + (bit >> 5)], ~mask);
-    }
-}
-
-__device__ __forceinline__ void unclaim_body(const PyrDev& P, const Refined* ref, const unsigned* ref_count, unsigned ref_cap, const BatchStride& bs, size_t fr, unsigned first, unsigned step) {
-    ref += fr * bs.refined; ref_count += fr * CNT_STRIDE;
-    unsigned n = *ref_count;
-    if (n > ref_cap) n = ref_cap;
-    for (unsigned i = first; i < n; i += step) {
-        const Refined rr = ref[i];
-        const size_t bit = ((size_t)rr.r * P.oc[rr.o].w + rr.c) * 4 + (size_t)rr.layer;
-        atomicAnd(&P.claimed[rr.o][fr * bs.claimed + (bit >> 5)], ~(1u << (bit & 31)));
+            if (khist) {
+                const unsigned key = (__float_as_uint(fabsf(contr)) >> 15) & 0xffffu;
+                unsigned long long peers = __ballot(1);
+#pragma unroll
+                for (int b = 0; b < 16; b++) {
+                    const unsigned long long bm = __ballot((key >> b) & 1u);
+                    peers &= ((key >> b) & 1u) ? bm : ~bm;
+                }
+                if ((peers & ((1ull << lane_id) - 1ull)) == 0ull) atomicAdd(&khist[fr * KEY_BINS + key], (unsigned)__popcll(peers));
+            }
+            if (P.mins[o]) atomicMin(&P.mins[o][fr * bs.mins + ((size_t)R * oc.w + C) * 4 + (size_t)L], start);
+        }
     }
 }
 
@@ -827,77 +821,136 @@
     unsigned start;
 };
 
-constexpr int UNCLAIM_WGS = 32;
-__global__ __launch_bounds__(1024) void select_unclaim_kernel(PyrDev P, const Refined* ref, BatchStride bs,
-                                                              const unsigned* resp , const unsigned* ref_count, unsigned ref_cap,
-                                                              unsigned want, unsigned* ctrl , size_t resp_stride,
-                                                              unsigned* list ) {
-    if (blockIdx.x > 0) { unclaim_body(P, ref, ref_count, ref_cap, bs, blockIdx.y, (blockIdx.x - 1) * 1024 + threadIdx.x, (gridDim.x - 1) * 1024); return; }
+constexpr unsigned UNIQ_LDS = 8192;
+constexpr unsigned long long UNIQ_EMPTY = ~0ull;
+__device__ __forceinline__ unsigned long long loc_key(int o, int layer, int r, int c) {
+    return ((unsigned long long)(unsigned)o << 48) | ((unsigned long long)(unsigned)layer << 44) | ((unsigned long long)(unsigned)r << 22) | (unsigned long long)(unsigned)c;
+}
+__device__ __forceinline__ bool uniq_insert(unsigned long long* tab, unsigned mask, unsigned long long key, int* overflow) {
+    unsigned h = (unsigned)((key * 0x9e3779b97f4a7c15ull) >> 32) & mask;
+    for (unsigned probe = 0; probe <= mask; probe++) {
+        const unsigned long long old = atomicCAS(&tab[h], UNIQ_EMPTY, key);
+        if (old == UNIQ_EMPTY) return true;
+        if (old == key) return false;
+        h = (h + 1u) & mask;
+    }
+    *overflow = 1;
+    return false;
+}
+__device__ __forceinline__ unsigned wave_append(bool take, unsigned value, unsigned* dst, unsigned cap, unsigned* counter) {
+    const int lane = threadIdx.x & 63;
+    const unsigned long long bm = __builtin_amdgcn_ballot_w64(take);
+    if (!bm) return 0xffffffffu;
+    const int first = __builtin_ctzll(bm);
+    unsigned base = 0;
+    if (lane == first) base = atomicAdd(counter, (unsigned)__builtin_popcountll(bm));
+    base = __shfl(base, first) + (unsigned)__builtin_popcountll(bm & ((1ull << lane) - 1ull));
+    if (take && base < cap) dst[base] = value;
+    return take ? base : 0xffffffffu;
+}
+__device__ __forceinline__ unsigned unique_compact_mem(const Refined* ref, const unsigned* resp, unsigned n, unsigned lo, unsigned hi, unsigned m,
+                                                       unsigned long long* g_tab, unsigned g_cap, unsigned* list, unsigned* s_cnt, int* overflow) {
+    const int tid = threadIdx.x;
+    unsigned size = 1024;
+    while (size < 2u * m && size < g_cap) size <<= 1;
+    for (unsigned i = tid; i < size; i += 1024) g_tab[i] = UNIQ_EMPTY;
+    if (tid == 0) *s_cnt = 0;
+    __syncthreads();
+    const unsigned nr = (n + 1023u) & ~1023u;
+    for (unsigned i0 = tid; i0 < nr; i0 += 8 * 1024) {
+        unsigned vv[8];
+#pragma unroll
+        for (int u = 0; u < 8; u++) { const unsigned i = i0 + 1024u * u; vv[u] = i < n ? resp[i] : 0u; }
+#pragma unroll
+        for (int u = 0; u < 8; u++) {
+            const unsigned i = i0 + 1024u * u;
+            bool take = i < n && vv[u] >= lo && vv[u] < hi;
+            if (take) { const Refined& rr = ref[i]; take = uniq_insert(g_tab, size - 1u, loc_key(rr.o, rr.layer, rr.r, rr.c), overflow); }
+            wave_append(take, i, list, n, s_cnt);
+        }
+    }
+    __syncthreads();
+    return *s_cnt;
+}
+__device__ __forceinline__ unsigned unique_compact_lds(const Refined* ref, const unsigned* resp, unsigned n, unsigned lo,
+                                                       unsigned long long* s_tab, unsigned* s_idx, unsigned* list, unsigned* s_cnt , int* overflow) {
+    const int tid = threadIdx.x;
+    for (unsigned i = tid; i < UNIQ_LDS; i += 1024) s_tab[i] = UNIQ_EMPTY;
+    if (tid == 0) { s_cnt[0] = 0; s_cnt[1] = 0; }
+    __syncthreads();
+    const unsigned nr = (n + 1023u) & ~1023u;
+    for (unsigned i0 = tid; i0 < nr; i0 += 8 * 1024) {
+        unsigned vv[8];
+#pragma unroll
+        for (int u = 0; u < 8; u++) { const unsigned i = i0 + 1024u * u; vv[u] = i < n ? resp[i] : 0u; }
+#pragma unroll
+        for (int u = 0; u < 8; u++) { const unsigned i = i0 + 1024u * u; wave_append(i < n && vv[u] >= lo, i, s_idx, UNIQ_LDS / 2, &s_cnt[1]); }
+    }
+    __syncthreads();
+    const unsigned ma = s_cnt[1] < UNIQ_LDS / 2 ? s_cnt[1] : UNIQ_LDS / 2;
+    for (unsigned j0 = 0; j0 < ma; j0 += 1024) {
+        const unsigned j = j0 + tid;
+        bool take = j < ma;
+        unsigned i = 0;
+        if (take) { i = s_idx[j]; const Refined& rr = ref[i]; take = uniq_insert(s_tab, UNIQ_LDS - 1u, loc_key(rr.o, rr.layer, rr.r, rr.c), overflow); }
+        wave_append(take, i, list, n, &s_cnt[0]);
+    }
+    __syncthreads();
+    return s_cnt[0];
+}
+
+__global__ __launch_bounds__(1024) void select_unique_kernel(const Refined* ref, BatchStride bs,
+                                                             const unsigned* resp , const unsigned* ref_count, unsigned ref_cap,
+                                                             unsigned want, unsigned* ctrl , size_t resp_stride,
+                                                             unsigned* list ,
+                                                             unsigned* khist , unsigned long long* g_tab, unsigned g_cap, int* overflow) {
+    ref += (size_t)blockIdx.y * bs.refined; g_tab += (size_t)blockIdx.y * bs.cand; overflow += (size_t)blockIdx.y * CNT_STRIDE; khist += (size_t)blockIdx.y * KEY_BINS;
     resp += (size_t)blockIdx.y * resp_stride; ref_count += (size_t)blockIdx.y * CNT_STRIDE; ctrl += (size_t)blockIdx.y * CNT_STRIDE;
     list += (size_t)blockIdx.y * resp_stride;
-    __shared__ unsigned s_h[16][256];
-    __shared__ unsigned s_sel[2], s_cnt;
-    const int tid = threadIdx.x, wv = tid >> 6;
+    __shared__ unsigned s_idx[UNIQ_LDS / 2], s_wtot[16], s_sel[2], s_cnt[2];
+    __shared__ unsigned long long s_tab[UNIQ_LDS];
+    const int tid = threadIdx.x, wv = tid >> 6, lane = tid & 63;
     unsigned n = *ref_count;
     if (n > ref_cap) n = ref_cap;
+    unsigned hv[64];
+    {
+        uint4* hp = reinterpret_cast<uint4*>(khist) + (size_t)tid * 16;
+#pragma unroll
+        for (int q = 0; q < 16; q++) { const uint4 v = hp[q]; hv[4 * q] = v.x; hv[4 * q + 1] = v.y; hv[4 * q + 2] = v.z; hv[4 * q + 3] = v.w; }
+#pragma unroll
+        for (int q = 0; q < 16; q++) hp[q] = make_uint4(0u, 0u, 0u, 0u);
+    }
     if (n <= want) {
-        if (tid == 0) { ctrl[0] = 0; ctrl[1] = 0; ctrl[2] = n; }
-        for (unsigned i = tid; i < n; i += 1024) list[i] = i;
+        if (n <= UNIQ_LDS / 2) unique_compact_lds(ref, resp, n, 0u, s_tab, s_idx, list, s_cnt, overflow);
+        else unique_compact_mem(ref, resp, n, 0u, 0xffffffffu, n, g_tab, g_cap, list, s_cnt, overflow);
+        if (tid == 0) { ctrl[0] = 0; ctrl[1] = 0; ctrl[2] = s_cnt[0]; }
         return;
     }
-    const unsigned nr = (n + 1023u) & ~1023u;
-    unsigned above = 0, hi_sel = 0;
-    for (int pass = 0; pass < 2; pass++) {
-        for (int i = tid; i < 16 * 256; i += 1024) (&s_h[0][0])[i] = 0;
-        __syncthreads();
-        for (unsigned i0 = tid; i0 < nr; i0 += 8 * 1024) {
-            unsigned vv[8];
-#pragma unroll
-            for (int u = 0; u < 8; u++) { const unsigned i = i0 + 1024u * u; vv[u] = i < n ? resp[i] : 0u; }
-#pragma unroll
-            for (int u = 0; u < 8; u++) {
-                if (i0 + 1024u * u >= n) continue;
-                const unsigned key = (vv[u] >> 15) & 0xffffu;
-                if (pass == 0) atomicAdd(&s_h[wv][key >> 8], 1u);
-                else if ((key >> 8) == hi_sel) atomicAdd(&s_h[wv][key & 255u], 1u);
-            }
-        }
-        __syncthreads();
-        if (tid < 256) { unsigned t = 0; for (int w = 0; w < 16; w++) t += s_h[w][tid]; s_h[0][tid] = t; }
-        __syncthreads();
-        if (tid == 0) {
-            unsigned cum = above; int b = 255;
-            for (; b >= 0; b--) { if (cum + s_h[0][b] >= want) break; cum += s_h[0][b]; }
-            if (b < 0) b = 0;
-            s_sel[0] = (unsigned)b; s_sel[1] = cum;
-        }
-        __syncthreads();
-        if (pass == 0) { hi_sel = s_sel[0]; above = s_sel[1]; }
-        else if (tid == 0) { ctrl[0] = ((hi_sel << 8) | s_sel[0]) << 15; ctrl[1] = 0; s_cnt = 0; }
-        __syncthreads();
-    }
-    const unsigned T = ((hi_sel << 8) | s_sel[0]) << 15;
-    const int lane = tid & 63;
-    for (unsigned i0 = tid; i0 < nr; i0 += 8 * 1024) {
-        unsigned vv[8];
-#pragma unroll
-        for (int u = 0; u < 8; u++) { const unsigned i = i0 + 1024u * u; vv[u] = i < n ? resp[i] : 0u; }
-#pragma unroll
-        for (int u = 0; u < 8; u++) {
-            const unsigned i = i0 + 1024u * u;
-            const bool take = i < n && vv[u] >= T;
-            const unsigned long long m = __builtin_amdgcn_ballot_w64(take);
-            if (m) {
-                const int first = __builtin_ctzll(m);
-                unsigned base = 0;
-                if (lane == first) base = atomicAdd(&s_cnt, (unsigned)__builtin_popcountll(m));
-                base = __shfl(base, first);
-                if (take) list[base + (unsigned)__builtin_popcountll(m & ((1ull << lane) - 1ull))] = i;
-            }
-        }
-    }
+    unsigned own = 0;
+#pragma unroll
+    for (int b = 0; b < 64; b++) own += hv[b];
+    unsigned suf = own;
+#pragma unroll
+    for (int off = 1; off < 64; off <<= 1) { const unsigned v = __shfl_down(suf, off); if (lane + off < 64) suf += v; }
+    if (lane == 0) s_wtot[wv] = suf;
+    if (tid == 0) { s_sel[0] = 0; s_sel[1] = n; }
     __syncthreads();
-    if (tid == 0) ctrl[2] = s_cnt;
+    for (int w = wv + 1; w < 16; w++) suf += s_wtot[w];
+    if (suf >= want && suf - own < want) {
+        unsigned cum = suf - own, key = 0, m = 0;
+        bool found = false;
+#pragma unroll
+        for (int b = 63; b >= 0; b--) {
+            if (!found && cum + hv[b] >= want) { found = true; key = (unsigned)tid * 64u + (unsigned)b; m = cum + hv[b]; }
+            cum += hv[b];
+        }
+        s_sel[0] = key << 15; s_sel[1] = m;
+    }
+    __syncthreads();
+    const unsigned T = s_sel[0], m = s_sel[1] < n ? s_sel[1] : n;
+    if (2u * m <= UNIQ_LDS) unique_compact_lds(ref, resp, n, T, s_tab, s_idx, list, s_cnt, overflow);
+    else unique_compact_mem(ref, resp, n, T, 0xffffffffu, m, g_tab, g_cap, list, s_cnt, overflow);
+    if (tid == 0) { ctrl[0] = T; ctrl[1] = 0; ctrl[2] = s_cnt[0]; }
 }
 
 static_assert(sizeof(lvl_t) == 2, "level_taps forms byte offsets of 2-byte samples in 32 bits");
@@ -930,17 +983,14 @@
     const int tid = threadIdx.x, lane = tid & 63, wv = tid >> 6;
     unsigned n = *ref_count;
     if (n > ref_cap) n = ref_cap;
-    if (pass == 0) n = ctrl[2] < n ? ctrl[2] : n;
+    { const unsigned nl = ctrl[pass == 0 ? 2 : 3]; n = nl < n ? nl : n; }
     if (tid == 0) s_on = 0;
     __syncthreads();
     for (unsigned base = blockIdx.x * 4; base < n; base += gridDim.x * 4) {
         unsigned k = base + wv;
-        bool take = false;
-        if (k < n) {
-            if (pass == 0) { k = list[k]; take = true; }
-            else take = __float_as_uint(fabsf(ref[k].contr)) < Tbits;
-        }
+        const bool take = k < n;
         if (take) {
+            k = list[k];
             const Refined rr = ref[k];
             const OctaveDev& oc = P.oc[__builtin_amdgcn_readfirstlane(rr.o)];
             const lvl_t* img = oc.lv[__builtin_amdgcn_readfirstlane(rr.layer)] + foff;
@@ -1036,8 +1086,11 @@
 }
 
 __global__ __launch_bounds__(1024) void topk_kernel(const KpRec* kps, const unsigned* resp, const unsigned* kp_count, unsigned kp_cap, int nfeatures,
-                                                    FrameOuts outs, SelRec* out_sel, int* out_n, int* overflow, unsigned* ctrl, int pass, BatchStride bs) {
+                                                    FrameOuts outs, SelRec* out_sel, int* out_n, int* overflow, unsigned* ctrl, int pass, BatchStride bs,
+                                                    const Refined* ref, const unsigned* ref_resp, const unsigned* ref_count, unsigned ref_cap,
+                                                    unsigned* list, unsigned long long* g_tab, unsigned g_cap, int* fell_back) {
     const size_t fr = blockIdx.x;
+    ref += fr * bs.refined; ref_resp += fr * bs.refined; ref_count += fr * CNT_STRIDE; list += fr * bs.refined; g_tab += fr * bs.cand; fell_back += fr * CNT_STRIDE;
     kps += fr * bs.kps; resp += fr * bs.kps; kp_count += fr * CNT_STRIDE; out_sel += fr * bs.sel; out_n += fr * CNT_STRIDE; overflow += fr * CNT_STRIDE; ctrl += fr * CNT_STRIDE;
     mi355_keypoint* out_kp = outs.kp[0];
 #pragma unroll
@@ -1147,9 +1200,18 @@
         SelRec sr; sr.ptx = k.ptx; sr.pty = k.pty; sr.scl = k.scl; sr.angle = k.angle; sr.o = k.o; sr.layer = k.layer;
         out_sel[i] = sr;
     }
+    const unsigned Tbits = ctrl[0];
+    const bool fall = pass == 0 && Tbits != 0 && keep < K;
     if (tid == 0) {
         *out_n = (int)keep;
-        if (pass == 0 && ctrl[0] != 0 && keep < K) ctrl[1] = 1;
+        if (fall) { ctrl[1] = 1; *fell_back = 1; }
+    }
+    if (fall) {
+        unsigned nr = *ref_count;
+        if (nr > ref_cap) nr = ref_cap;
+        __syncthreads();
+        const unsigned cnt = unique_compact_mem(ref, ref_resp, nr, 0u, Tbits, nr, g_tab, g_cap, list, &s_misc[2], overflow);
+        if (tid == 0) ctrl[3] = cnt;
     }
 }
 
@@ -1409,8 +1471,8 @@
 
 struct SiftBufs {
     DevBuf pyr;
-    DevBuf claimed;
     DevBuf cand, refined, kps, kresp, sel, counters, rhist, ccnt;
+    DevBuf khist;
     DevBuf olist;
     DevBuf mins;
     DevBuf ksort;
@@ -1418,18 +1480,17 @@
     hipError_t reserve(const Layout& l, int nb, hipStream_t st) {
         const Strides& bs = l.bs;
         const struct { DevBuf* b; size_t bytes; } want[] = {
-            {&pyr, bs.pyr * sizeof(lvl_t)}, {&claimed, bs.claimed * sizeof(unsigned)}, {&cand, bs.cand * sizeof(unsigned long long)},
+            {&pyr, bs.pyr * sizeof(lvl_t)}, {&cand, bs.cand * sizeof(unsigned long long)},
             {&refined, bs.refined * sizeof(Refined)}, {&kps, bs.kps * sizeof(KpRec)}, {&kresp, bs.kps * sizeof(unsigned)}, {&sel, bs.sel * sizeof(SelRec)},
             {&mins, bs.mins * sizeof(unsigned)}, {&ksort, l.ksort_stride * sizeof(unsigned long long)}, {&counters, CNT_STRIDE * sizeof(unsigned)},
-            {&rhist, bs.refined * sizeof(unsigned)}, {&olist, bs.refined * sizeof(unsigned)}, {&ccnt, CCNT_STRIDE * sizeof(unsigned)}, {&cube, bs.cube * sizeof(float)}};
+            {&rhist, bs.refined * sizeof(unsigned)}, {&khist, l.keepall ? 0 : KEY_BINS * sizeof(unsigned)}, {&olist, bs.refined * sizeof(unsigned)}, {&ccnt, CCNT_STRIDE * sizeof(unsigned)}, {&cube, bs.cube * sizeof(float)}};
         for (const auto& w : want) {
             if (!w.bytes) { w.b->release(); continue; }
             if (const hipError_t e = w.b->reserve((size_t)nb * w.bytes); e != hipSuccess) return e;
         }
-        if (const hipError_t e = hipMemsetAsync(claimed.p, 0, (size_t)nb * bs.claimed * sizeof(unsigned), st); e != hipSuccess) return e;
-        return l.keepall ? hipMemsetAsync(mins.p, 0xff, (size_t)nb * bs.mins * sizeof(unsigned), st) : hipSuccess;
-    }
-    void release() { for (DevBuf* b : {&pyr, &claimed, &cand, &refined, &kps, &kresp, &sel, &counters, &rhist, &ccnt, &olist, &mins, &ksort, &cube}) b->release(); }
+        return l.keepall ? hipMemsetAsync(mins.p, 0xff, (size_t)nb * bs.mins * sizeof(unsigned), st) : hipMemsetAsync(khist.p, 0, (size_t)nb * KEY_BINS * sizeof(unsigned), st);
+    }
+    void release() { for (DevBuf* b : {&pyr, &khist, &cand, &refined, &kps, &kresp, &sel, &counters, &rhist, &ccnt, &olist, &mins, &ksort, &cube}) b->release(); }
 };
 
 }
@@ -1544,17 +1605,16 @@
     if (s->lay.same_key(lay) && s->nb == nb) return MI355_OK;
     MI_HIP(hipStreamSynchronize(s->stream));
     MI_HIP(s->b.reserve(lay, nb, s->stream));
-    if ((((uintptr_t)s->b.pyr.p) | ((uintptr_t)s->b.claimed.p)) & 127) { ctx->set_error("sift: work area is not 128-byte aligned"); return MI355_ERR_FAILED; }
+    if (((uintptr_t)s->b.pyr.p) & 127) { ctx->set_error("sift: work area is not 128-byte aligned"); return MI355_ERR_FAILED; }
     memset(&s->P, 0, sizeof(s->P));
     for (int o = 0; o < lay.n_oct; o++) {
         const Octave& oc = lay.oc[o];
         s->P.oc[o].w = oc.w; s->P.oc[o].h = oc.h;
         for (int i = 0; i < N_LEVELS; i++) s->P.oc[o].lv[i] = s->b.pyr.as<lvl_t>() + oc.lv[i];
-        s->P.claimed[o] = s->b.claimed.as<unsigned>() + oc.claimed;
         s->P.mins[o] = lay.keepall ? s->b.mins.as<unsigned>() + oc.mins : nullptr;
     }
     s->P.n_oct = lay.n_oct;
-    s->bs = BatchStride{lay.bs.pyr, lay.bs.claimed, lay.bs.cand, lay.bs.refined, lay.bs.kps, lay.bs.cube, lay.bs.sel, lay.bs.mins};
+    s->bs = BatchStride{lay.bs.pyr, lay.bs.cand, lay.bs.refined, lay.bs.kps, lay.bs.cube, lay.bs.sel, lay.bs.mins};
     s->lay = lay; s->nb = nb;
     return MI355_OK;
 }
@@ -1675,10 +1735,13 @@
     const Layout& lay = s->lay;
     const BatchStride bs = s->bs;
     const unsigned kmax = (unsigned)lay.kmax;
+    unsigned uniq_cap = 1024;
+    while ((size_t)uniq_cap * 2 <= bs.cand && uniq_cap < (1u << 31)) uniq_cap <<= 1;
     {
         ProfScope ps(ctx, "refine", 0.0, st);
         hipLaunchKernelGGL(refine_kernel, dim3(REFINE_GX, NREG, n), dim3(256), 0, st, s->P, d.cand.as<unsigned long long>(), d.ccnt.as<unsigned>(), lay.cand_cap, cnt + 0,
-                           ctx->p.contrast_threshold, ctx->p.edge_threshold, 1.6f, d.refined.as<Refined>(), cnt + 1, lay.ref_cap, d.rhist.as<unsigned>(), bs, d.cube.as<float>(), lay.cube_cap);
+                           ctx->p.contrast_threshold, ctx->p.edge_threshold, 1.6f, d.refined.as<Refined>(), cnt + 1, lay.ref_cap, d.rhist.as<unsigned>(), bs, d.cube.as<float>(), lay.cube_cap,
+                           lay.keepall ? nullptr : d.khist.as<unsigned>());
     }
     {
         ProfScope ps(ctx, "kp_select", 0.0, st);
@@ -1686,8 +1749,9 @@
             hipLaunchKernelGGL(keepall_live_kernel, dim3(256, n), dim3(256), 0, st, s->P, d.refined.as<Refined>(), cnt + 1, lay.ref_cap, cnt + 8, d.olist.as<unsigned>(), bs);
             hipLaunchKernelGGL(keepall_reset_kernel, dim3(256, n), dim3(256), 0, st, s->P, d.refined.as<Refined>(), cnt + 1, lay.ref_cap, bs);
         } else {
-            hipLaunchKernelGGL(select_unclaim_kernel, dim3(1 + UNCLAIM_WGS, n), dim3(1024), 0, st, s->P, d.refined.as<Refined>(), bs, d.rhist.as<unsigned>(), cnt + 1, lay.ref_cap,
-                               (unsigned)ctx->p.nfeatures + 256u, cnt + 8, bs.refined, d.olist.as<unsigned>());
+            hipLaunchKernelGGL(select_unique_kernel, dim3(1, n), dim3(1024), 0, st, d.refined.as<Refined>(), bs, d.rhist.as<unsigned>(), cnt + 1, lay.ref_cap,
+                               (unsigned)ctx->p.nfeatures + (unsigned)ctx->select_margin, cnt + 8, bs.refined, d.olist.as<unsigned>(), d.khist.as<unsigned>(), d.cand.as<unsigned long long>(), uniq_cap,
+                               reinterpret_cast<int*>(cnt + 4));
         }
     }
     for (int pass = 0; pass < (lay.keepall ? 1 : 2); pass++) {
@@ -1704,7 +1768,9 @@
                                d.ksort.as<const unsigned long long>(), lay.ksort_stride, outs, d.sel.as<SelRec>(), reinterpret_cast<int*>(cnt + 3), reinterpret_cast<int*>(cnt + 4), bs);
         } else {
             hipLaunchKernelGGL(topk_kernel, dim3(n), dim3(1024), 0, st, d.kps.as<KpRec>(), d.kresp.as<unsigned>(), cnt + 2, lay.kp_cap, ctx->p.nfeatures,
-                               outs, d.sel.as<SelRec>(), reinterpret_cast<int*>(cnt + 3), reinterpret_cast<int*>(cnt + 4), cnt + 8, pass, bs);
+                               outs, d.sel.as<SelRec>(), reinterpret_cast<int*>(cnt + 3), reinterpret_cast<int*>(cnt + 4), cnt + 8, pass, bs,
+                               d.refined.as<Refined>(), d.rhist.as<unsigned>(), cnt + 1, lay.ref_cap, d.olist.as<unsigned>(), d.cand.as<unsigned long long>(), uniq_cap,
+                               reinterpret_cast<int*>(cnt + 5));
         }
     }
     ProfScope ps(ctx, "describe", 0.0, st);
```

Result: faster. 4166 image-pairs/s, median of 6 (+1.5%).
